# facebookresearch/habitat-lab

Hardware: AMD Instinct MI355X
Metric: env-steps/sec (SPS) PointNav RGB-D 256x256, 64 envs x 128 rollout (higher is better)
Workload: dtype f32; 1 GPU; PointNav SimpleCNN+GRU, 64 envs x 128 steps, 256x256 RGB-D synthetic; envs_per_gpu=64, rollout_steps=128, ppo_epoch=4, num_mini_batch=4, parallelism=dp1

## Files before the change

habitat-lab_amd/csrc/conv2_dgrad_strip.h:

```cpp
#pragma once
#include "igemm_bf3.h"
#include "ops.h"

namespace hab {

struct C2dArgs {
    const float* dy;
    const float* wd;
    const float* mask;
    float* dx;
    int B;
    int strips, items;
    int sign_schedule;
    int H, W, Ho, Wo;
};

template <int R2>
struct C2dCfg {
    static constexpr int H = 63, Ho = 30, Wo = 30, NT = 512, CELLS = 32;
    static constexpr int YRS = R2 + 1, YCOLS = 33, YPIX = YRS * YCOLS;
    static constexpr int YU = YRS * Wo * 16, YPT = (YU + NT - 1) / NT;
    static constexpr int Y_PLANE = YPIX * 64;
    static constexpr int RED_LD = 68;
    static constexpr size_t Y_BYTES = ((size_t)3 * Y_PLANE * 2 + 15) / 16 * 16, RED_BYTES = (size_t)8 * 32 * RED_LD * 4;
    static constexpr size_t LDS_BYTES = Y_BYTES + RED_BYTES;
    static_assert(CELLS % R2 == 0, "");
};

template <int R2, bool RT>
__global__ void __launch_bounds__(512) conv2_dgrad_strip_kernel(const C2dArgs a) {
    using Cfg = C2dCfg<R2>;
    constexpr int NT = Cfg::NT;
    const int H = RT ? a.H : Cfg::H, W = RT ? a.W : Cfg::H, Ho = RT ? a.Ho : Cfg::Ho, Wo = RT ? a.Wo : Cfg::Wo;
    const int YU = Cfg::YRS * Wo * 16;
    extern __shared__ __attribute__((aligned(16))) unsigned short smem16[];
    unsigned short* ys = smem16;
    float* red = reinterpret_cast<float*>(reinterpret_cast<char*>(smem16) + Cfg::Y_BYTES);
    const int t = threadIdx.x, lane = t & 63;
    const int wave = __builtin_amdgcn_readfirstlane(t >> 6);
    const int tap = wave >> 1, ph = wave & 1, ta = tap >> 1, tb = tap & 1;
    const int li = lane & 31, hi = lane >> 5;

    const int xcd = blockIdx.x & 7, jw = blockIdx.x >> 3, wg_per_xcd = gridDim.x >> 3;
    const int per_xcd = (a.items + 7) >> 3, per_wg = (per_xcd + wg_per_xcd - 1) / wg_per_xcd;
    const int xcd_end = min(a.items, (xcd + 1) * per_xcd);
    const int first = min(xcd_end, xcd * per_xcd + jw * per_wg), last = min(xcd_end, first + per_wg);
    if (first >= last) return;

    for (int i = t; i < (int)(Cfg::Y_BYTES / 16); i += NT) reinterpret_cast<u32x4*>(smem16)[i] = u32x4{0u, 0u, 0u, 0u};

    const bool flip = a.sign_schedule && (blockIdx.x & 1);
    const unsigned sgn2 = flip ? 0x80008000u : 0u;

    bf16x8 bw[4][2][3];
#pragma unroll
    for (int j = 0; j < 4; ++j)
#pragma unroll
        for (int pw = 0; pw < 2; ++pw) {
            const int kh = ph + 2 * ta, kw = pw + 2 * tb, co = j * 16 + hi * 8;
            const float* src = a.wd + ((size_t)(li * 4 + kh) * 4 + kw) * 64 + co;
            const f32x4 v0 = *reinterpret_cast<const f32x4*>(src), v1 = *reinterpret_cast<const f32x4*>(src + 4);
            unsigned p[3][4];
            bf3_split2(v0[0], v0[1], p[0][0], p[1][0], p[2][0]);
            bf3_split2(v0[2], v0[3], p[0][1], p[1][1], p[2][1]);
            bf3_split2(v1[0], v1[1], p[0][2], p[1][2], p[2][2]);
            bf3_split2(v1[2], v1[3], p[0][3], p[1][3], p[2][3]);
#pragma unroll
            for (int pl = 0; pl < 3; ++pl)
                bw[j][pw][pl] = __builtin_bit_cast(bf16x8, u32x4{p[pl][0] ^ sgn2, p[pl][1] ^ sgn2, p[pl][2] ^ sgn2, p[pl][3] ^ sgn2});
        }

    f32x4 yr[Cfg::YPT];
    int pf_h20 = 0;
    auto fetch = [&](int item) {
        const int img = item / a.strips, h20 = (item - img * a.strips) * R2;
        pf_h20 = h20;
#pragma unroll
        for (int j = 0; j < Cfg::YPT; ++j) {
            const int u = t + j * NT;
            const int r = u / (Wo * 16), row = h20 - 1 + r;
            const bool ok = (RT ? u < YU : (Cfg::YU % NT == 0 || u < Cfg::YU)) && (unsigned)row < (unsigned)Ho;
            const size_t off = ok ? ((size_t)img * Ho + row) * (size_t)(Wo * 64) + (size_t)(u - r * (Wo * 16)) * 4 : 0;
            yr[j] = *reinterpret_cast<const f32x4*>(a.dy + off);
        }
    };
    auto stage = [&]() {
#pragma unroll
        for (int j = 0; j < Cfg::YPT; ++j) {
            const int u = t + j * NT;
            if (RT ? u >= YU : (Cfg::YU % NT != 0 && u >= Cfg::YU)) continue;
            const int r = u / (Wo * 16), rem = u - r * (Wo * 16), w = rem >> 4, c4 = rem & 15;
            const int pixidx = r * Cfg::YCOLS + w + 1;
            unsigned short* dst = ys + pixidx * 64 + (((c4 >> 1) ^ ((pixidx >> 1) & 7)) << 3) + (c4 & 1) * 4;
            const bool in_image = (unsigned)(pf_h20 - 1 + r) < (unsigned)Ho;
            bf3_store4(in_image ? yr[j] : f32x4{0.f, 0.f, 0.f, 0.f}, dst, dst + Cfg::Y_PLANE, dst + 2 * Cfg::Y_PLANE);
        }
    };

    __syncthreads();
    fetch(first);
    for (int item = first; item < last; ++item) {
        stage();
        __syncthreads();
        if (item + 1 < last) fetch(item + 1);
        const int img = item / a.strips, h20 = (item - img * a.strips) * R2;
#pragma unroll 1
        for (int tr = 0; tr < R2; ++tr) {
            const int pixidx = (tr + 1 - ta) * Cfg::YCOLS + li + 1 - tb;
            const int swz = (pixidx >> 1) & 7;
            f32x4 mk[2];
            if (a.mask) {
#pragma unroll
                for (int q = 0; q < 2; ++q) {
                    const int idx = t + q * NT, rph = idx >> 9, cell = (idx >> 4) & 31, cq = idx & 15;
                    const int h = 2 * (h20 + tr) + rph, w = 2 * cell + (cq >> 3);
                    const bool ok = h < H && w < W;
                    mk[q] = *reinterpret_cast<const f32x4*>(a.mask + (ok ? (((size_t)img * H + h) * W + w) * 32 + (cq & 7) * 4 : (size_t)0));
                }
            }
            f32x16 acc[2];
#pragma unroll
            for (int pw = 0; pw < 2; ++pw)
#pragma unroll
                for (int v = 0; v < 16; ++v) acc[pw][v] = 0.f;
#pragma unroll
            for (int j = 0; j < 4; ++j) {
                const unsigned short* src = ys + pixidx * 64 + (((2 * j + hi) ^ swz) << 3);
                bf16x8 yf[3];
#pragma unroll
                for (int pl = 0; pl < 3; ++pl) yf[pl] = *reinterpret_cast<const bf16x8*>(src + pl * Cfg::Y_PLANE);
                constexpr int PA[6] = {2, 0, 1, 1, 0, 0}, PB[6] = {0, 2, 1, 0, 1, 0};
#pragma unroll
                for (int q = 0; q < 6; ++q)
#pragma unroll
                    for (int pw = 0; pw < 2; ++pw)
                        acc[pw] = __builtin_amdgcn_mfma_f32_32x32x16_bf16(bw[j][pw][PB[q]], yf[PA[q]], acc[pw], 0, 0, 0);
            }
            if (tr > 0) __syncthreads();
            float* mine = red + (size_t)(wave * 32 + li) * Cfg::RED_LD;
#pragma unroll
            for (int pw = 0; pw < 2; ++pw)
#pragma unroll
                for (int g = 0; g < 4; ++g)
                    *reinterpret_cast<f32x4*>(mine + pw * 32 + 8 * g + 4 * hi) =
                        f32x4{acc[pw][4 * g], acc[pw][4 * g + 1], acc[pw][4 * g + 2], acc[pw][4 * g + 3]};
            __syncthreads();
            const int h2 = h20 + tr;
#pragma unroll
            for (int q = 0; q < 2; ++q) {
                const int idx = t + q * NT, rph = idx >> 9, cell = (idx >> 4) & 31, cq = idx & 15;
                f32x4 s = *reinterpret_cast<const f32x4*>(red + (size_t)(rph * 32 + cell) * Cfg::RED_LD + cq * 4);
#pragma unroll
                for (int t4 = 1; t4 < 4; ++t4)
                    s += *reinterpret_cast<const f32x4*>(red + (size_t)((2 * t4 + rph) * 32 + cell) * Cfg::RED_LD + cq * 4);
                if (flip) s = -s;
                const int h = 2 * h2 + rph, w = 2 * cell + (cq >> 3);
                if (h < H && w < W) {
                    const size_t off = (((size_t)img * H + h) * W + w) * 32 + (cq & 7) * 4;
                    if (a.mask) {
                        const f32x4 m = mk[q];
#pragma unroll
                        for (int e = 0; e < 4; ++e) s[e] = m[e] > 0.f ? s[e] : 0.f;
                    }
                    *reinterpret_cast<f32x4*>(a.dx + off) = s;
                }
            }
        }
        __syncthreads();
    }
}

inline bool conv2_dgrad_strip_covers(const ConvDesc& d) {
    return d.KH == 4 && d.KW == 4 && d.stride == 2 && d.pad == 0 && d.C == 32 && d.Cout == 64 && d.H >= 4 && d.W >= 4 && d.H <= 63 && d.W <= 63;
}

inline int conv2_dgrad_strip(const ConvDesc& d, const float* dy, const float* wd, const float* mask, const float* add, float* dx,
                             hipStream_t stream) {
    if (!conv2_dgrad_strip_covers(d)) return 1;
    if (add || d.B < 16 || !dy || !wd || !dx) return 1;
    if ((reinterpret_cast<uintptr_t>(dy) | reinterpret_cast<uintptr_t>(wd) | reinterpret_cast<uintptr_t>(dx) | reinterpret_cast<uintptr_t>(mask)) & 15) return 1;
    constexpr int R2 = 2;
    using Cfg = C2dCfg<R2>;
    C2dArgs a;
    a.dy = dy; a.wd = wd; a.mask = mask; a.dx = dx; a.B = d.B;
    a.H = d.H; a.W = d.W; a.Ho = (d.H - 4) / 2 + 1; a.Wo = (d.W - 4) / 2 + 1;
    a.strips = ((d.H + 1) / 2 + R2 - 1) / R2;
    if ((long long)d.B * a.strips > 0x7fffffffLL) return 1;
    a.items = d.B * a.strips;
    static const int sign_schedule = !hab_env_flag("HAB_BF3_NOSIGN");
    a.sign_schedule = sign_schedule;
    static const hipError_t attr_err = [] {
        const hipError_t e0 = hipFuncSetAttribute(reinterpret_cast<const void*>(conv2_dgrad_strip_kernel<R2, false>),
                                                  hipFuncAttributeMaxDynamicSharedMemorySize, (int)Cfg::LDS_BYTES);
        const hipError_t e1 = hipFuncSetAttribute(reinterpret_cast<const void*>(conv2_dgrad_strip_kernel<R2, true>),
                                                  hipFuncAttributeMaxDynamicSharedMemorySize, (int)Cfg::LDS_BYTES);
        return e0 != hipSuccess ? e0 : e1;
    }();
    if (attr_err != hipSuccess) return (int)attr_err;
    int grid = 256;
    while (grid > 8 && grid > a.items) grid -= 8;
    if (d.H == 63 && d.W == 63) conv2_dgrad_strip_kernel<R2, false><<<grid, Cfg::NT, Cfg::LDS_BYTES, stream>>>(a);
    else conv2_dgrad_strip_kernel<R2, true><<<grid, Cfg::NT, Cfg::LDS_BYTES, stream>>>(a);
    HAB_LAUNCH_CHECK();
    return HAB_OK;
}

}
```

habitat-lab_amd/csrc/conv2_fwd_strip.h:

```cpp
#pragma once
#include "igemm_bf3.h"

namespace hab {

struct C2fArgs {
    const float* x;
    const float* wf;
    const float* bias;
    float* y;
    int B;
    int strips, items;
    int relu, sign_schedule;
    int H, W, Ho, Wo;
};

template <int R>
struct C2fCfg {
    static constexpr int W = 63, C = 32, N = 64, Wo = 30, Ho = 30, NT = 512;
    static constexpr int XRS = 2 * (R - 1) + 4, XROWS = XRS * W, NPIX = R * Wo, NPT = (NPIX + 31) / 32;
    static constexpr int XU = XRS * W * C / 4, XPT = (XU + NT - 1) / NT;
    static constexpr int WH = (W + 1) / 2;
    static constexpr int X_PLANE = XROWS * 32;
    static constexpr int RED_LD = N + 4;
    static constexpr size_t X_BYTES = (size_t)3 * X_PLANE * 2, RED_BYTES = (size_t)8 * 32 * RED_LD * 4;
    static constexpr size_t LDS_BYTES = X_BYTES + RED_BYTES;
    static_assert(X_BYTES % 16 == 0 && Ho % R == 0, "");
    __host__ __device__ static constexpr int xcol(int w) { return (w & 1) * WH + (w >> 1); }
};

template <int R, bool RT>
__global__ void __launch_bounds__(512) conv2_fwd_strip_kernel(const C2fArgs a) {
    using Cfg = C2fCfg<R>;
    constexpr int NT = Cfg::NT;
    const int W = RT ? a.W : Cfg::W, H = RT ? a.H : Cfg::W, Wo = RT ? a.Wo : Cfg::Wo, Ho = RT ? a.Ho : Cfg::Ho;
    const int WH = (W + 1) / 2, X_PLANE = Cfg::XRS * W * 32, XU = Cfg::XRS * W * 8, NPIX = R * Wo, NPT = (NPIX + 31) / 32;
    auto xcol = [&](int w) { return (w & 1) * WH + (w >> 1); };
    extern __shared__ __attribute__((aligned(16))) unsigned short smem16[];
    unsigned short* xs = smem16;
    float* red = reinterpret_cast<float*>(reinterpret_cast<char*>(smem16) + (size_t)3 * X_PLANE * 2);
    const int t = threadIdx.x, lane = t & 63;
    const int wave = __builtin_amdgcn_readfirstlane(t >> 6);
    const int kh = wave >> 1, kwp = wave & 1;
    const int li = lane & 31, hi = lane >> 5;

    const int xcd = blockIdx.x & 7, jw = blockIdx.x >> 3, wg_per_xcd = gridDim.x >> 3;
    const int per_xcd = (a.items + 7) >> 3, per_wg = (per_xcd + wg_per_xcd - 1) / wg_per_xcd;
    const int xcd_end = min(a.items, (xcd + 1) * per_xcd);
    const int first = min(xcd_end, xcd * per_xcd + jw * per_wg), last = min(xcd_end, first + per_wg);
    if (first >= last) return;

    const bool flip = a.sign_schedule && (blockIdx.x & 1);
    const unsigned sgn2 = flip ? 0x80008000u : 0u;

    bf16x8 bw[4][2][3];
#pragma unroll
    for (int j = 0; j < 4; ++j)
#pragma unroll
        for (int ct = 0; ct < 2; ++ct) {
            const int co = ct * 32 + li, kw = 2 * kwp + (j >> 1), ci = (j & 1) * 16 + hi * 8;
            const float* src = a.wf + ((size_t)(co * 4 + kh) * 4 + kw) * 32 + ci;
            const f32x4 v0 = *reinterpret_cast<const f32x4*>(src), v1 = *reinterpret_cast<const f32x4*>(src + 4);
            unsigned p[3][4];
            bf3_split2(v0[0], v0[1], p[0][0], p[1][0], p[2][0]);
            bf3_split2(v0[2], v0[3], p[0][1], p[1][1], p[2][1]);
            bf3_split2(v1[0], v1[1], p[0][2], p[1][2], p[2][2]);
            bf3_split2(v1[2], v1[3], p[0][3], p[1][3], p[2][3]);
#pragma unroll
            for (int pl = 0; pl < 3; ++pl)
                bw[j][ct][pl] = __builtin_bit_cast(bf16x8, u32x4{p[pl][0] ^ sgn2, p[pl][1] ^ sgn2, p[pl][2] ^ sgn2, p[pl][3] ^ sgn2});
        }

    f32x4 xr[Cfg::XPT];
    int pf_units = XU;
    auto fetch = [&](int item) {
        const int img = item / a.strips, ho0 = (item - img * a.strips) * R;
        const float* xb = a.x + ((size_t)img * H + ho0 * 2) * (size_t)(W * 32);
        if (RT) pf_units = min(Cfg::XRS, H - 2 * ho0) * W * 8;
#pragma unroll
        for (int j = 0; j < Cfg::XPT; ++j) {
            const int u = t + j * NT;
            const bool in = RT ? u < pf_units : (Cfg::XU % NT == 0 || u < Cfg::XU);
            xr[j] = *reinterpret_cast<const f32x4*>(xb + (in ? (size_t)u * 4 : 0));
        }
    };
    auto stage = [&]() {
#pragma unroll
        for (int j = 0; j < Cfg::XPT; ++j) {
            const int u = t + j * NT;
            if (RT ? u >= XU : (Cfg::XU % NT != 0 && u >= Cfg::XU)) continue;
            const int c4 = u & 7, pix = u >> 3, w = pix % W, hh = pix / W;
            const int row = hh * W + xcol(w);
            unsigned short* dst = xs + row * 32 + (((c4 >> 1) ^ ((row >> 2) & 3)) << 3) + (c4 & 1) * 4;
            bf3_store4((!RT || u < pf_units) ? xr[j] : f32x4{0.f, 0.f, 0.f, 0.f}, dst, dst + X_PLANE, dst + 2 * X_PLANE);
        }
    };

    const int rpix = t >> 4, rco = (t & 15) * 4;
    f32x4 bias4 = {0.f, 0.f, 0.f, 0.f};
    if (a.bias) bias4 = *reinterpret_cast<const f32x4*>(a.bias + rco);

    fetch(first);
    for (int item = first; item < last; ++item) {
        stage();
        __syncthreads();
        if (item + 1 < last) fetch(item + 1);
        const int img = item / a.strips, ho0 = (item - img * a.strips) * R;
        float* yb = a.y + ((size_t)img * Ho + ho0) * (size_t)(Wo * 64);
        const int npix_here = RT ? min(R, Ho - ho0) * Wo : NPIX;
#pragma unroll 1
        for (int pt = 0; pt < NPT; ++pt) {
            const int p = pt * 32 + li;
            const int pc = (!RT && Cfg::NPIX % 32 == 0) || p < NPIX ? p : 0;
            const int hol = pc / Wo, wo = pc - hol * Wo;
            const int row0 = (hol * 2 + kh) * W + wo;
            f32x16 acc[2];
#pragma unroll
            for (int ct = 0; ct < 2; ++ct)
#pragma unroll
                for (int v = 0; v < 16; ++v) acc[ct][v] = 0.f;
#pragma unroll
            for (int j = 0; j < 4; ++j) {
                const int kw = 2 * kwp + (j >> 1);
                const int row = row0 + (kw & 1) * WH + (kw >> 1);
                const int chunk = (j & 1) * 2 + hi;
                const unsigned short* src = xs + row * 32 + ((chunk ^ ((row >> 2) & 3)) << 3);
                bf16x8 af[3];
#pragma unroll
                for (int pl = 0; pl < 3; ++pl) af[pl] = *reinterpret_cast<const bf16x8*>(src + pl * X_PLANE);
                constexpr int PA[6] = {2, 0, 1, 1, 0, 0}, PB[6] = {0, 2, 1, 0, 1, 0};
#pragma unroll
                for (int q = 0; q < 6; ++q)
#pragma unroll
                    for (int ct = 0; ct < 2; ++ct)
                        acc[ct] = __builtin_amdgcn_mfma_f32_32x32x16_bf16(bw[j][ct][PB[q]], af[PA[q]], acc[ct], 0, 0, 0);
            }
            if (pt > 0) __syncthreads();
            float* mine = red + (size_t)(wave * 32 + li) * Cfg::RED_LD;
#pragma unroll
            for (int ct = 0; ct < 2; ++ct)
#pragma unroll
                for (int g = 0; g < 4; ++g)
                    *reinterpret_cast<f32x4*>(mine + ct * 32 + 8 * g + 4 * hi) =
                        f32x4{acc[ct][4 * g], acc[ct][4 * g + 1], acc[ct][4 * g + 2], acc[ct][4 * g + 3]};
            __syncthreads();
            f32x4 s = *reinterpret_cast<const f32x4*>(red + (size_t)rpix * Cfg::RED_LD + rco);
#pragma unroll
            for (int w8 = 1; w8 < 8; ++w8) s += *reinterpret_cast<const f32x4*>(red + (size_t)(w8 * 32 + rpix) * Cfg::RED_LD + rco);
            if (flip) s = -s;
            s += bias4;
            if (a.relu) {
#pragma unroll
                for (int e = 0; e < 4; ++e) s[e] = s[e] > 0.f ? s[e] : 0.f;
            }
            const int op = pt * 32 + rpix;
            if (RT ? op < npix_here : (Cfg::NPIX % 32 == 0 || op < Cfg::NPIX)) *reinterpret_cast<f32x4*>(yb + (size_t)op * 64 + rco) = s;
        }
        __syncthreads();
    }
}

inline bool conv2_fwd_strip_covers(const ConvGeom& g) {
    return g.KH == 4 && g.KW == 4 && g.stride == 2 && g.pad == 0 && g.C == 32 && g.Cout == 64 && g.H >= 4 && g.W >= 4 && g.W <= 63;
}

inline int conv2_fwd_strip(const ConvFwdProb& p, float* , size_t , hipStream_t stream) {
    const ConvGeom& g = p.g;
    if (!conv2_fwd_strip_covers(g)) return 1;
    if ((p.ldy != 0 && p.ldy != 64) || g.B < 16) return 1;
    if ((reinterpret_cast<uintptr_t>(p.x) | reinterpret_cast<uintptr_t>(p.w) | reinterpret_cast<uintptr_t>(p.y) | reinterpret_cast<uintptr_t>(p.bias)) & 15) return 1;
    constexpr int R = 2;
    using Cfg = C2fCfg<R>;
    C2fArgs a;
    a.x = p.x; a.wf = p.w; a.bias = p.bias; a.y = p.y; a.B = g.B;
    a.H = g.H; a.W = g.W; a.Ho = (g.H - 4) / 2 + 1; a.Wo = (g.W - 4) / 2 + 1;
    a.strips = (a.Ho + R - 1) / R;
    if ((long long)g.B * a.strips > 0x7fffffffLL) return 1;
    a.items = g.B * a.strips;
    a.relu = p.relu;
    static const int sign_schedule = !hab_env_flag("HAB_BF3_NOSIGN");
    a.sign_schedule = sign_schedule;
    const bool bench_geom = g.H == 63 && g.W == 63;
    static const hipError_t attr_err = [] {
        const hipError_t e0 = hipFuncSetAttribute(reinterpret_cast<const void*>(conv2_fwd_strip_kernel<R, false>),
                                                  hipFuncAttributeMaxDynamicSharedMemorySize, (int)Cfg::LDS_BYTES);
        const hipError_t e1 = hipFuncSetAttribute(reinterpret_cast<const void*>(conv2_fwd_strip_kernel<R, true>),
                                                  hipFuncAttributeMaxDynamicSharedMemorySize, (int)Cfg::LDS_BYTES);
        return e0 != hipSuccess ? e0 : e1;
    }();
    if (attr_err != hipSuccess) return (int)attr_err;
    int grid = 256;
    while (grid > 8 && grid > a.items) grid -= 8;
    if (bench_geom) conv2_fwd_strip_kernel<R, false><<<grid, Cfg::NT, Cfg::LDS_BYTES, stream>>>(a);
    else conv2_fwd_strip_kernel<R, true><<<grid, Cfg::NT, (size_t)3 * Cfg::XRS * g.W * 32 * 2 + Cfg::RED_BYTES, stream>>>(a);
    HAB_LAUNCH_CHECK();
    return HAB_OK;
}

}
```

habitat-lab_amd/csrc/engine.h:

```cpp
#pragma once
#include <string.h>

#include <algorithm>
#include <string>
#include <vector>

#include "heads.h"
#include "ops.h"
#include "problems.h"
#include "resnet_ops.h"
#include "../../include/habitat_amd.h"

struct ParamSpec {
    std::string name;
    int64_t shape[4];
    int ndim;
    int64_t offset;
    int64_t numel;
    int is_buffer = 0;
};

struct Arena {
    int64_t used = 0;
    int64_t take(int64_t n) {
        const int64_t o = used;
        used += (n + 63) & ~(int64_t)63;
        return o;
    }
};

struct RnnForm {
    int chunks = 0;
    bool wave = false;
};

struct hab_policy {
    hab_policy_desc d;
    std::vector<ParamSpec> params;
    int64_t param_floats = 0, packed_floats = 0, work_floats = 0;
    float *P = nullptr, *G = nullptr, *PK = nullptr, *WK = nullptr;
    int64_t work_bound = 0;
    int Cin = 0;
    hab::ConvDesc c1, c2, c3;
    int fc_in = 0, rnn_in = 0, rnn_ld = 0, G_ = 3, L = 1;
    int i_c1w = -1, i_c1b = -1, i_c2w = -1, i_c2b = -1, i_c3w = -1, i_c3b = -1, i_fcw = -1, i_fcb = -1, i_aw = -1, i_ab = -1, i_cw = -1, i_cb = -1;
    int i_astd = -1;
    int head_K = 0;
    int64_t w_gsaved = -1;
    std::vector<int> i_wih, i_whh, i_bih, i_bhh;
    int64_t pk_c1f = -1, pk_c2f = -1, pk_c2d = -1, pk_c3f = -1, pk_c3d = -1, pk_fc = -1;
    int64_t pk_c1img = -1;
    std::vector<int64_t> pk_whht;
    std::vector<int64_t> pk_wiht;
    int64_t pk_wih0 = -1;
    int64_t w_a1 = -1, w_a2 = -1, w_a3 = -1, w_da1 = -1, w_da2 = -1, w_da3 = -1;
    int64_t w_rnnin = -1, w_drnnin = -1, w_hinit = -1, w_cinit = -1, w_probs = -1, w_logitsn = -1, w_dzv = -1, w_dv = -1, w_dfeat = -1,
            w_scratch = -1, w_value = -1, w_logp = -1, w_ent = -1, w_hmask = -1, w_gistep = -1, w_step_h = -1, w_ws = -1;
    std::vector<int64_t> w_gi, w_gates, w_hn, w_hprev, w_cprev, w_c, w_out, w_dgi, w_dgh, w_dlayer;
    int64_t ws_floats = 0;
    int last_B = 0, last_n = 0;
    const uint8_t* last_masks = nullptr;
    hipStream_t s2 = nullptr;
    std::vector<hipEvent_t> evs;
    int64_t w_ws2 = -1, ws2_floats = 0, w_fmask = -1, w_iota = -1;
    RnnForm form;
    struct ResNetPlan* rn = nullptr;
    int save_acts = 1;
    int training = 1;
    hab_allreduce_fn allreduce_cb = nullptr;
    void* allreduce_ctx = nullptr;
    int world_size = 1;
    hab_grad_ready_fn grad_ready_cb = nullptr;
    void* grad_ready_ctx = nullptr;
    struct hab_comm* comm = nullptr;
    const float* xg_feat = nullptr; const float* xg_perc = nullptr;
    int comm_err = 0;
    int64_t comm_first = -1;
    hipStream_t cur_stream = nullptr;
    uint64_t probe_mask = 0;
    struct ProbeEv { int tag; hipEvent_t first, second; };
    std::vector<ProbeEv> probe_events;
    size_t probe_used = 0;
    double probe_flops[64] = {0}, probe_bytes[64] = {0};

    float* p(int i) const { return P + params[i].offset; }
    float* g(int i) const { return G + params[i].offset; }
};

inline int add_param(hab_policy* e, const std::string& name, std::initializer_list<int64_t> shape) {
    ParamSpec s;
    s.name = name;
    s.ndim = (int)shape.size();
    s.numel = 1;
    int k = 0;
    for (auto v : shape) { s.shape[k++] = v; s.numel *= v; }
    for (; k < 4; ++k) s.shape[k] = 1;
    s.offset = e->param_floats;
    e->param_floats += (s.numel + 3) & ~(int64_t)3;
    e->params.push_back(s);
    return (int)e->params.size() - 1;
}
inline int conv_out(int x, int k, int s, int p) { return (x + 2 * p - k) / s + 1; }

void add_tail_params(hab_policy* e);
void pack_tail(hab_policy* e, Arena& pk);
void plan_tail_workspace(hab_policy* e, Arena& wk, int64_t ws_floats);
int repack_tail(hab_policy* e, hipStream_t s);
int build_resnet(hab_policy* e);
void destroy_resnet(hab_policy* e);
int resnet_repack(hab_policy* e, hipStream_t s);
void grad_tail_ready(hab_policy* e, int first_param);
int comm_exchange_async(struct hab_comm* c, float* buf, int64_t first, int64_t count, hipStream_t compute);
extern "C" int hab_comm_allreduce_sum(struct hab_comm* c, float* buf, int64_t count, hipStream_t stream);
int resnet_feature_shape(const hab_policy* e, int* c, int* hf, int* wf);
int resnet_encode(hab_policy* e, const hab_obs* obs, int n, float* out, hipStream_t s);
int resnet_encoder_forward(hab_policy* e, const hab_obs* obs, const uint8_t* masks, const int* rows, int B, hipStream_t s, int f0 = 0, int nB = -1);
int resnet_encoder_backward(hab_policy* e, const hab_obs* obs, const uint8_t* masks, const int* rows, int B, hipStream_t s);
int resnet_tap(hab_policy* e, int which, const float** ptr, int64_t* floats);

struct Probe {
    hab_policy* e; hipStream_t s; bool on;
    Probe(hab_policy* e_, int tag, hipStream_t s_, double flops = 0.0, double bytes = 0.0) : e(e_), s(s_), on((e_->probe_mask >> tag) & 1) {
        if (!on) return;
        e->probe_flops[tag] += flops; e->probe_bytes[tag] += bytes;
        if (e->probe_used == e->probe_events.size()) {
            hipEvent_t a, b;
            (void)hipEventCreate(&a); (void)hipEventCreate(&b);
            e->probe_events.push_back({tag, a, b});
        }
        e->probe_events[e->probe_used].tag = tag;
        (void)hipEventRecord(e->probe_events[e->probe_used].first, s);
    }
    ~Probe() {
        if (!on) return;
        (void)hipEventRecord(e->probe_events[e->probe_used].second, s);
        e->probe_used++;
    }
};
// ... 2 lines not shown
```

habitat-lab_amd/csrc/engine.hip:

```cpp
#include <string.h>

#include <algorithm>

#include <string>
#include <vector>

#include "engine.h"

using namespace hab;

static void plan_tm_workspace(hab_policy* e, Arena& wk);
void add_tail_params(hab_policy* e) {
    const hab_policy_desc& d = e->d;
    const int H = d.hidden;
    const std::string rn = "net.state_encoder.rnn.";
    for (int l = 0; l < d.rnn_layers; ++l) {
        const int in = l == 0 ? e->rnn_in : H;
        const std::string sfx = "_l" + std::to_string(l);
        e->i_wih.push_back(add_param(e, rn + "weight_ih" + sfx, {e->G_ * H, in}));
        e->i_whh.push_back(add_param(e, rn + "weight_hh" + sfx, {e->G_ * H, H}));
        e->i_bih.push_back(add_param(e, rn + "bias_ih" + sfx, {e->G_ * H}));
        e->i_bhh.push_back(add_param(e, rn + "bias_hh" + sfx, {e->G_ * H}));
    }
    if (d.action_dist == HAB_DIST_GAUSSIAN) {
// ... 11 lines not shown
void pack_tail(hab_policy* e, Arena& pk) {
    const int64_t GH = (int64_t)e->G_ * e->d.hidden;
    for (int l = 0; l < e->L; ++l) e->pk_whht.push_back(pk.take(GH * e->d.hidden));
    for (int l = 0; l < e->L; ++l) e->pk_wiht.push_back(l == 0 ? -1 : pk.take(GH * e->d.hidden));
    e->pk_wih0 = pk.take(GH * e->rnn_ld);
}
int repack_tail(hab_policy* e, hipStream_t s) {
    const int H = e->d.hidden;
    for (int l = 0; l < e->L; ++l) HAB_TRY(transpose2d(e->p(e->i_whh[l]), e->PK + e->pk_whht[l], e->G_ * H, H, s));
    for (int l = 1; l < e->L; ++l) HAB_TRY(transpose2d(e->p(e->i_wih[l]), e->PK + e->pk_wiht[l], e->G_ * H, H, s));
    return pad_rows(e->p(e->i_wih[0]), e->PK + e->pk_wih0, e->G_ * H, e->rnn_in, e->rnn_ld, s);
}
void plan_tail_workspace(hab_policy* e, Arena& wk, int64_t ws_floats) {
    const hab_policy_desc& d = e->d;
    const int64_t B = d.max_frames, F = d.max_frames;
    const int64_t H = d.hidden, GH = e->G_ * H;
    e->w_rnnin = wk.take(B * e->rnn_ld); e->w_drnnin = wk.take(B * e->rnn_ld);
    e->w_hinit = wk.take(e->L * F * H); e->w_cinit = wk.take(e->L * F * H);
    for (int l = 0; l < e->L; ++l) {
        e->w_gi.push_back(wk.take(B * GH)); e->w_gates.push_back(wk.take(B * GH));
        e->w_hn.push_back(wk.take(B * H)); e->w_hprev.push_back(wk.take(B * H));
        e->w_cprev.push_back(wk.take(B * H)); e->w_c.push_back(wk.take(B * H)); e->w_out.push_back(wk.take(B * H));
        e->w_dgi.push_back(wk.take(B * GH)); e->w_dgh.push_back(wk.take(B * GH));
        e->w_dlayer.push_back(wk.take(B * H));
    }
    e->w_probs = wk.take(B * 8); e->w_logitsn = wk.take(B * 8); e->w_dzv = wk.take(B * 8); e->w_dv = wk.take(B);
    e->w_dfeat = wk.take(B * H); e->w_scratch = wk.take((int64_t)std::max(3, 2 * e->L) * F * H);
    e->w_value = wk.take(B); e->w_logp = wk.take(B); e->w_ent = wk.take(B);
    if (d.action_dist == HAB_DIST_GAUSSIAN) e->w_gsaved = wk.take(B * 16);
    e->w_hmask = wk.take(2 * H * e->L * d.max_envs);
    e->w_gistep = wk.take(d.max_envs * GH);
    e->w_step_h = wk.take(d.max_envs * H * 2);
    e->ws_floats = ws_floats;
    e->w_ws = wk.take(ws_floats);
    plan_tm_workspace(e, wk);
}

static int build_baseline(hab_policy* e) {
    const hab_policy_desc& d = e->d;
    e->Cin = (d.has_rgb ? 3 : 0) + (d.has_depth ? 1 : 0);
    const bool blind = e->Cin == 0;
    if (blind && d.goal_dim <= 0) return HAB_ERR_ARG;
    if (d.rnn_type != HAB_RNN_GRU && d.rnn_type != HAB_RNN_LSTM) return HAB_ERR_ARG;
    const int H = d.hidden;
    e->G_ = d.rnn_type == HAB_RNN_GRU ? 3 : 4;
    e->L = d.rnn_layers;
    e->c1 = ConvDesc{0, d.H, d.W, blind ? 4 : e->Cin, 32, 8, 8, 4, 0};
    e->c2 = ConvDesc{0, conv_out(d.H, 8, 4, 0), conv_out(d.W, 8, 4, 0), 32, 64, 4, 4, 2, 0};
    e->c3 = ConvDesc{0, e->c2.Ho(), e->c2.Wo(), 64, 32, 3, 3, 1, 0};
    const int h3 = e->c3.Ho(), w3 = e->c3.Wo();
    if (!blind && (h3 <= 0 || w3 <= 0)) return HAB_ERR_ARG;
    e->fc_in = blind ? 0 : 32 * h3 * w3;
    e->rnn_in = (blind ? 0 : H) + d.goal_dim;
    e->rnn_ld = (e->rnn_in + 15) & ~15;
    const std::string ve = "net.visual_encoder.cnn.";
    if (!blind) {
        e->i_c1w = add_param(e, ve + "0.weight", {32, e->Cin, 8, 8});
        e->i_c1b = add_param(e, ve + "0.bias", {32});
        e->i_c2w = add_param(e, ve + "2.weight", {64, 32, 4, 4});
        e->i_c2b = add_param(e, ve + "2.bias", {64});
        e->i_c3w = add_param(e, ve + "4.weight", {32, 64, 3, 3});
        e->i_c3b = add_param(e, ve + "4.bias", {32});
        e->i_fcw = add_param(e, ve + "6.weight", {H, e->fc_in});
        e->i_fcb = add_param(e, ve + "6.bias", {H});
    }
    add_tail_params(e);

    Arena pk;
    e->pk_c1f = pk.take(32 * 64 * (blind ? 4 : e->Cin));
    e->pk_c1img = (!blind && e->Cin == 4) ? pk.take(obs_conv_weight_image_floats()) : -1;
    e->pk_c2f = pk.take(64 * 16 * 32);
    e->pk_c2d = pk.take(64 * 16 * 32);
    e->pk_c3f = pk.take(32 * 9 * 64);
    e->pk_c3d = pk.take(32 * 9 * 64);
    e->pk_fc = pk.take((int64_t)H * std::max(e->fc_in, 4));
    pack_tail(e, pk);
    e->packed_floats = pk.used;

    Arena wk;
    const int64_t B = d.max_frames;
    const int64_t m1 = blind ? 0 : (int64_t)e->c1.Ho() * e->c1.Wo() * 32, m2 = blind ? 0 : (int64_t)e->c2.Ho() * e->c2.Wo() * 64, m3 = e->fc_in;
    e->w_a1 = wk.take(B * m1); e->w_a2 = wk.take(B * m2); e->w_a3 = wk.take(B * m3);
    e->w_da1 = wk.take(B * m1); e->w_da2 = wk.take(B * m2); e->w_da3 = wk.take(B * m3);
    plan_tail_workspace(e, wk, std::max<int64_t>((int64_t)16 << 20, (int64_t)8 * H * e->fc_in / 4));
    e->work_floats = wk.used;
    return HAB_OK;
}

extern "C" int hab_policy_create(const hab_policy_desc* desc, hab_policy** out) {
    if (!desc || !out) return HAB_ERR_ARG;
    if (desc->hidden <= 0 || desc->hidden % 64 || desc->num_actions <= 0 || desc->num_actions > 8 || desc->max_frames <= 0 ||
        desc->max_envs <= 0 || desc->rnn_layers <= 0 || desc->goal_dim < 0 ||
        ((desc->has_rgb || desc->has_depth || desc->has_semantic || desc->num_visual > 0) && (desc->H <= 0 || desc->W <= 0)))
        return HAB_ERR_ARG;
    if (desc->arch != HAB_ARCH_RESNET && (desc->num_visual != 0 || desc->num_fused != 0)) return HAB_ERR_UNSUPPORTED;
    if (desc->action_dist != HAB_DIST_CATEGORICAL && (desc->action_dist != HAB_DIST_GAUSSIAN || desc->arch != HAB_ARCH_RESNET))
        return HAB_ERR_UNSUPPORTED;
    if (desc->action_dist == HAB_DIST_GAUSSIAN && desc->num_actions > 4) return HAB_ERR_UNSUPPORTED;
    hab_policy* e = new hab_policy();
    e->d = *desc;
    int rc = HAB_ERR_UNSUPPORTED;
    if (desc->arch == HAB_ARCH_SIMPLE_CNN) rc = build_baseline(e);
    else if (desc->arch == HAB_ARCH_RESNET) rc = build_resnet(e);
    if (rc != HAB_OK) { destroy_resnet(e); delete e; return rc; }
    *out = e;
    return HAB_OK;
}
extern "C" void hab_policy_destroy(hab_policy* e) {
    if (!e) return;
    for (auto& ev : e->probe_events) { (void)hipEventDestroy(ev.first); (void)hipEventDestroy(ev.second); }
    for (auto& ev : e->evs) (void)hipEventDestroy(ev);
    if (e->s2) (void)hipStreamDestroy(e->s2);
    destroy_resnet(e);
    delete e;
}
extern "C" int hab_policy_num_params(const hab_policy* e) { return e ? (int)e->params.size() : HAB_ERR_ARG; }
extern "C" int hab_policy_param_info(const hab_policy* e, int i, char* name, int name_cap, int64_t* shape4, int* ndim,
                                     int64_t* offset_floats) {
    if (!e || i < 0 || i >= (int)e->params.size() || !name || name_cap <= 0) return HAB_ERR_ARG;
    const ParamSpec& s = e->params[i];
    strncpy(name, s.name.c_str(), name_cap - 1);
    name[name_cap - 1] = 0;
    if (shape4) for (int k = 0; k < 4; ++k) shape4[k] = s.shape[k];
    if (ndim) *ndim = s.ndim;
    if (offset_floats) *offset_floats = s.offset;
    return HAB_OK;
}
extern "C" int hab_policy_param_is_buffer(const hab_policy* e, int i) {
    if (!e || i < 0 || i >= (int)e->params.size()) return HAB_ERR_ARG;
    return e->params[i].is_buffer;
}
extern "C" int hab_policy_set_training(hab_policy* e, int training) {
    if (!e) return HAB_ERR_ARG;
    e->training = training ? 1 : 0;
    return HAB_OK;
}
extern "C" int hab_policy_set_grad_ready(hab_policy* e, hab_grad_ready_fn fn, void* ctx) {
    if (!e) return HAB_ERR_ARG;
    e->grad_ready_cb = fn; e->grad_ready_ctx = ctx;
    return HAB_OK;
}
void grad_tail_ready(hab_policy* e, int first_param) {
    if (e->comm) {
        static const bool no_overlap = hab_env_flag("HAB_NO_GRAD_OVERLAP");
        if (no_overlap || e->comm_err != HAB_OK) return;
        const int64_t first = e->g(first_param) - e->G;
        const int64_t end = e->comm_first < 0 ? (int64_t)e->param_floats : e->comm_first;
        if (first >= end) return;
        const int rc = comm_exchange_async(e->comm, e->G, first, end - first, e->cur_stream);
        if (rc == HAB_OK) e->comm_first = first;
        else e->comm_err = rc;
        return;
    }
    if (!e->grad_ready_cb) return;
    const int64_t first = e->g(first_param) - e->G;
    e->grad_ready_cb(first, (int64_t)e->param_floats - first, e->grad_ready_ctx);
}
extern "C" int hab_policy_set_allreduce(hab_policy* e, hab_allreduce_fn fn, void* ctx, int world_size) {
    if (!e || world_size < 1) return HAB_ERR_ARG;
    e->allreduce_cb = fn; e->allreduce_ctx = ctx; e->world_size = world_size;
    return HAB_OK;
}
extern "C" int64_t hab_policy_param_floats(const hab_policy* e) { return e ? e->param_floats : -1; }
extern "C" int64_t hab_policy_packed_floats(const hab_policy* e) { return e ? e->packed_floats : -1; }
extern "C" int64_t hab_policy_work_floats(const hab_policy* e) { return e ? e->work_floats : -1; }

// ... 8 lines not shown
extern "C" int hab_policy_repack(hab_policy* e, hipStream_t stream) {
    if (!e || !e->P) return HAB_ERR_ARG;
    if (e->rn) return resnet_repack(e, stream);
    if (e->Cin == 0) return repack_tail(e, stream);
    HAB_TRY(repack_conv(e->p(e->i_c1w), e->PK + e->pk_c1f, nullptr, 32, e->Cin, 8, 8, e->Cin, stream));
    if (e->pk_c1img >= 0) {
        const int rc = obs_conv_weight_image(e->PK + e->pk_c1f, 32, 8, 8, e->Cin, e->PK + e->pk_c1img, stream);
        if (rc != HAB_OK) return rc == 1 ? HAB_ERR_UNSUPPORTED : rc;
    }
    HAB_TRY(repack_conv(e->p(e->i_c2w), e->PK + e->pk_c2f, e->PK + e->pk_c2d, 64, 32, 4, 4, 32, stream));
    HAB_TRY(repack_conv(e->p(e->i_c3w), e->PK + e->pk_c3f, e->PK + e->pk_c3d, 32, 64, 3, 3, 64, stream));
    HAB_TRY(repack_flatten(e->p(e->i_fcw), e->PK + e->pk_fc, e->d.hidden, 32, e->fc_in / 32, stream));
    return repack_tail(e, stream);
}

extern "C" int hab_policy_probe_enable(hab_policy* e, int tag) {
    if (!e || tag >= 64) return HAB_ERR_ARG;
    e->probe_mask = tag < 0 ? 0 : (uint64_t)1 << tag;
    e->probe_used = 0;
    for (int i = 0; i < 64; ++i) { e->probe_flops[i] = 0.0; e->probe_bytes[i] = 0.0; }
    return HAB_OK;
}
extern "C" int hab_policy_probe_enable_mask(hab_policy* e, uint64_t mask) {
    if (!e) return HAB_ERR_ARG;
    e->probe_mask = mask;
    e->probe_used = 0;
    for (int i = 0; i < 64; ++i) { e->probe_flops[i] = 0.0; e->probe_bytes[i] = 0.0; }
    return HAB_OK;
}
static int probe_sum(hab_policy* e, int tag, double* total_ms, int* count) {
    double t = 0;
    int n = 0;
    for (size_t i = 0; i < e->probe_used; ++i) {
        if (tag >= 0 && e->probe_events[i].tag != tag) continue;
        hipError_t err = hipEventSynchronize(e->probe_events[i].second);
        if (err != hipSuccess) return (int)err;
        float ms = 0;
        err = hipEventElapsedTime(&ms, e->probe_events[i].first, e->probe_events[i].second);
        if (err != hipSuccess) return (int)err;
        t += ms;
        ++n;
    }
    *total_ms = t;
    *count = n;
    return HAB_OK;
}
extern "C" int hab_policy_probe_work(hab_policy* e, int tag, double* flops, double* bytes) {
    if (!e || tag < 0 || tag >= 64 || !flops || !bytes) return HAB_ERR_ARG;
    *flops = e->probe_flops[tag]; *bytes = e->probe_bytes[tag];
    return HAB_OK;
}
extern "C" int hab_policy_probe_read(hab_policy* e, double* total_ms, int* count) {
    if (!e || !total_ms || !count) return HAB_ERR_ARG;
    HAB_TRY(probe_sum(e, -1, total_ms, count));
    e->probe_used = 0;
    return HAB_OK;
}
extern "C" int hab_policy_probe_read_tag(hab_policy* e, int tag, double* total_ms, int* count) {
    if (!e || !total_ms || !count || tag < 0 || tag >= 64) return HAB_ERR_ARG;
    return probe_sum(e, tag, total_ms, count);
}


static int encoder_forward(hab_policy* e, const hab_obs* obs, const uint8_t* masks, const int* rows, int B, hipStream_t s, int f0 = 0, int nB = -1) {
    if (e->rn) { Probe pr(e, HAB_PROBE_ENC_FWD, s); return resnet_encoder_forward(e, obs, masks, rows, B, s, f0, nB); }
    if (nB < 0) nB = B;
    float* W = e->WK;
    float* ws = W + e->w_ws;
    const int H = e->d.hidden;
    if (e->Cin == 0) {
        if (!rows && f0) return HAB_ERR_ARG;
        return gather_cols(obs->goal, e->d.goal_dim, rows ? rows + f0 : nullptr, W + e->w_rnnin + (int64_t)f0 * e->rnn_ld, e->rnn_ld, 0, e->d.goal_dim,
                           e->rnn_ld - e->rnn_in, nB, s);
    }
    const int64_t m1 = (int64_t)e->c1.Ho() * e->c1.Wo() * 32, m2 = (int64_t)e->c2.Ho() * e->c2.Wo() * 64, m3 = e->fc_in;
    float *a1 = W + e->w_a1 + f0 * m1, *a2 = W + e->w_a2 + f0 * m2, *a3 = W + e->w_a3 + f0 * m3, *rin = W + e->w_rnnin + (int64_t)f0 * e->rnn_ld;
    const int* rws = rows ? rows + f0 : nullptr;
    if (!rows && f0) return HAB_ERR_ARG;
    ObsView ov;
    ov.rgb = e->d.has_rgb ? obs->rgb : nullptr; ov.depth = e->d.has_depth ? obs->depth : nullptr; ov.rows = rws;
    ov.H = e->d.H; ov.W = e->d.W; ov.C = e->Cin;
    ConvDesc c1 = e->c1, c2 = e->c2, c3 = e->c3;
    c1.B = c2.B = c3.B = nB;
    { Probe pr(e, HAB_PROBE_CONV1_FWD, s);
      HAB_TRY(obs_conv_fwd(c1, ov, e->PK + e->pk_c1f, e->p(e->i_c1b), a1, 1, ws, e->ws_floats, s, e->pk_c1img >= 0 ? e->PK + e->pk_c1img : nullptr)); }
    { Probe pr(e, HAB_PROBE_CONV2_FWD, s);
      HAB_TRY(conv_fwd(c2, a1, e->PK + e->pk_c2f, e->p(e->i_c2b), a2, 1, ws, e->ws_floats, s)); }
    { Probe pr(e, HAB_PROBE_CONV3_FWD, s);
      HAB_TRY(conv_fwd(c3, a2, e->PK + e->pk_c3f, e->p(e->i_c3b), a3, 0, ws, e->ws_floats, s)); }
    { Probe pr(e, HAB_PROBE_FC_FWD, s);
      HAB_TRY(linear_fwd(a3, e->fc_in, e->PK + e->pk_fc, e->fc_in, e->p(e->i_fcb), rin, e->rnn_ld, nB, H, e->fc_in, 1, 0, ws, e->ws_floats, s)); }
    if (e->d.goal_dim > 0)
        HAB_TRY(gather_cols(obs->goal, e->d.goal_dim, rws, rin, e->rnn_ld, H, e->d.goal_dim, e->rnn_ld - e->rnn_in, nB, s));
    return HAB_OK;
}

static RnnForm rnn_form_cfg(const hab_policy* e, int frames, int n, bool tm_shape) {
    static const int chunks = hab_env_int("HAB_RNN_CHUNKS", 4), chunks_resnet = hab_env_int("HAB_RNN_CHUNKS_RESNET", -1);
    static const int wave = hab_env_int("HAB_RNN_WAVE", 1);
    RnnForm f;
    if (tm_shape) {
        int nc = chunks;
        if (e->rn && chunks > 1) nc = chunks_resnet >= 0 ? chunks_resnet : frames >= 4096 ? 2 : 0;
        f.chunks = std::max(0, std::min(nc, frames / n));
    }
    if (f.chunks == 0) f.wave = wave && e->L >= 2 && e->L <= 4;
    return f;
}
static RnnForm rnn_form(const hab_policy* e, const int* rows, const hab_pack_info* pack, int B, int n) {
    const bool tm_shape = e->Cin > 0 && rows && !pack->env_first_frame && (B % n) == 0 && B / n >= 2 && e->w_ws2 >= 0 &&
                          (int64_t)e->L * 2 * n <= 3 * (int64_t)e->d.max_frames;
    return rnn_form_cfg(e, B, n, tm_shape);
}
static void plan_tm_workspace(hab_policy* e, Arena& wk) {
    const int64_t B = e->d.max_frames;
    if (rnn_form_cfg(e, (int)B, 1, true).chunks == 0) return;
    e->ws2_floats = e->ws_floats;
    e->w_ws2 = wk.take(e->ws2_floats);
    e->w_fmask = wk.take((B + 3) / 4 + 64);
    e->w_iota = wk.take(B + 64);
}
static int tm_setup(hab_policy* e, int nev) {
    if (!e->s2) {
        int lo = 0, hi = 0;
        (void)hipDeviceGetStreamPriorityRange(&lo, &hi);
        hipError_t err = hipStreamCreateWithPriority(&e->s2, hipStreamNonBlocking, hi);
        if (err != hipSuccess) return (int)err;
    }
    while ((int)e->evs.size() < nev) {
        hipEvent_t ev;
        hipError_t err = hipEventCreateWithFlags(&ev, hipEventDisableTiming);
        if (err != hipSuccess) return (int)err;
        e->evs.push_back(ev);
    }
    return HAB_OK;
}
static int tm_order(hab_policy* e, int ev, hipStream_t from, hipStream_t to) {
    hipError_t err = hipEventRecord(e->evs[ev], from);
    if (err != hipSuccess) return (int)err;
    err = hipStreamWaitEvent(to, e->evs[ev], 0);
    return err == hipSuccess ? HAB_OK : (int)err;
}

static RnnLayerParams layer_params(hab_policy* e, int l) {
    RnnLayerParams lp;
    lp.w_ih = e->p(e->i_wih[l]); lp.w_hh = e->p(e->i_whh[l]); lp.b_ih = e->p(e->i_bih[l]); lp.b_hh = e->p(e->i_bhh[l]);
    lp.w_hh_t = e->PK + e->pk_whht[l];
    if (e->G) { lp.dw_ih = e->g(e->i_wih[l]); lp.dw_hh = e->g(e->i_whh[l]); lp.db_ih = e->g(e->i_bih[l]); lp.db_hh = e->g(e->i_bhh[l]); }
    else { lp.dw_ih = lp.dw_hh = lp.db_ih = lp.db_hh = nullptr; }
    lp.in_dim = l == 0 ? e->rnn_in : e->d.hidden;
    if (l == 0 && e->pk_wih0 >= 0) { lp.w_ih_pad = e->PK + e->pk_wih0; lp.w_ih_ld = e->rnn_ld; }
    else if (l > 0 && (e->d.hidden & 15) == 0) { lp.w_ih_pad = lp.w_ih; lp.w_ih_ld = e->d.hidden; }
    return lp;
}
static RnnWork layer_work(hab_policy* e, int l) {
    float* W = e->WK;
    RnnWork wk;
    wk.gi = W + e->w_gi[l]; wk.gates = W + e->w_gates[l]; wk.hn = W + e->w_hn[l]; wk.hprev = W + e->w_hprev[l];
    wk.cprev = W + e->w_cprev[l]; wk.c = W + e->w_c[l]; wk.out = W + e->w_out[l]; wk.dgi = W + e->w_dgi[l];
    wk.dgh = W + e->w_dgh[l];
    return wk;
}
static const float* layer_x(const hab_policy* e, int l) { return e->WK + (l == 0 ? e->w_rnnin : e->w_out[l - 1]); }
static int layer_ld(const hab_policy* e, int l) { return l == 0 ? e->rnn_ld : e->d.hidden; }
static float* layer_dx(const hab_policy* e, int l) { return e->WK + (l == 0 ? e->w_drnnin : e->w_dlayer[l]); }
static const float* layer_dout(const hab_policy* e, int l) { return l == e->L - 1 ? e->WK + e->w_dfeat : layer_dx(e, l + 1); }
static PackInfo pack_info(const hab_pack_info* pack, int n) {
    PackInfo pk;
    pk.select_inds = pack->select_inds; pk.step_offsets = pack->step_offsets_host; pk.num_seqs_at_step = pack->num_seqs_at_step_host;
    pk.frag_env = pack->frag_env; pk.frag_start = pack->frag_start; pk.P = pack->P; pk.F = pack->F; pk.max_len = pack->max_len;
// ... 64 lines not shown
    ha.mode = actions ? (deterministic ? 2 : 1) : 2;
    ha.feats = x; ha.feats_ld = ldx; ha.w_actor = e->p(e->i_aw); ha.b_actor = e->p(e->i_ab); ha.w_critic = e->p(e->i_cw); ha.b_critic = e->p(e->i_cb);
    ha.actions_in = nullptr; ha.rows = nullptr; ha.noise = exp_noise;
    ha.actions_out = actions ? actions : reinterpret_cast<int64_t*>(W + e->w_dzv);
    ha.value = values; ha.logp = action_log_probs ? action_log_probs : W + e->w_logp; ha.entropy = nullptr;
    ha.probs = probs_out ? W + e->w_probs : nullptr; ha.logits_n = W + e->w_logitsn;
    if (ha.mode == 1 && !exp_noise) return HAB_ERR_ARG;
    HAB_TRY(heads_forward(ha, stream));
    if (probs_out) HAB_TRY(copy_rows(W + e->w_probs, nullptr, 8, probs_out, 8, n, 8, stream));
    return HAB_OK;
}

static int rnn_state_init(hab_policy* e, const float* hidden0, int hidden_env_stride, const int* rows, const uint8_t* masks,
                          const int* frag_env, const int* frag_start, int F, const int* env_first_frame, hipStream_t s) {
    const int H = e->d.hidden, L = e->L;
    for (int l = 0; l < L; ++l) {
        HAB_TRY(rnn_frag_init(hidden0 + (size_t)l * H, rows, hidden_env_stride, masks, rows, frag_env, frag_start, F, H,
                              e->WK + e->w_hinit + (size_t)l * F * H, s, env_first_frame));
        if (e->d.rnn_type == HAB_RNN_LSTM)
            HAB_TRY(rnn_frag_init(hidden0 + (size_t)(L + l) * H, rows, hidden_env_stride, masks, rows, frag_env, frag_start, F, H,
                                  e->WK + e->w_cinit + (size_t)l * F * H, s, env_first_frame));
    }
    return HAB_OK;
}
static int rnn_tm_forward(hab_policy* e, const hab_obs* obs, const int* rows, const float* hidden0, int hidden_env_stride,
                          const uint8_t* masks, int B, int n, hipStream_t stream) {
    float* W = e->WK;
    const int H = e->d.hidden, L = e->L, NC = e->form.chunks, T = B / n, Tc = (T + NC - 1) / NC;
    HAB_TRY(tm_setup(e, 2 * NC + 4));
    hipStream_t sB = e->s2;
    uint8_t* fmask = reinterpret_cast<uint8_t*>(W + e->w_fmask);
    HAB_TRY(rnn_tm_prepare(masks, rows, B, fmask, reinterpret_cast<int*>(W + e->w_iota), stream));
    HAB_TRY(rnn_state_init(e, hidden0, hidden_env_stride, rows, masks, nullptr, nullptr, n, nullptr, stream));
    for (int c = 0; c < NC; ++c) {
        const int t0 = c * Tc, t1 = std::min(T, t0 + Tc);
        if (t0 >= t1) break;
        HAB_TRY(encoder_forward(e, obs, masks, rows, B, stream, t0 * n, (t1 - t0) * n));
        HAB_TRY(tm_order(e, c, stream, sB));
        for (int l = 0; l < L; ++l) {
            Probe pr(e, HAB_PROBE_RNN_FWD, sB);
            HAB_TRY(rnn_tm_layer_forward(e->d.rnn_type, H, layer_params(e, l), layer_work(e, l), layer_x(e, l), layer_ld(e, l),
                                         W + e->w_hinit + (size_t)l * n * H, W + e->w_cinit + (size_t)l * n * H, fmask, n, T, t0, t1,
                                         W + e->w_ws2, e->ws2_floats, sB));
        }
    }
    return tm_order(e, NC, sB, stream);
}
static int rnn_packed_forward(hab_policy* e, const int* rows, const float* hidden0, int hidden_env_stride, const uint8_t* masks,
                              const hab_pack_info* pack, int n, hipStream_t stream) {
    float* W = e->WK;
    const int H = e->d.hidden, L = e->L;
    const PackInfo pk = pack_info(pack, n);
    HAB_TRY(rnn_state_init(e, hidden0, hidden_env_stride, rows, masks, pk.frag_env, pk.frag_start, pk.F, pack->env_first_frame, stream));
    if (e->form.wave) {
        RnnLayerParams lps[4]; RnnWork wks[4]; const float* hin[4]; const float* cin[4];
        for (int l = 0; l < L; ++l) {
            lps[l] = layer_params(e, l); wks[l] = layer_work(e, l);
            hin[l] = W + e->w_hinit + (size_t)l * pk.F * H; cin[l] = W + e->w_cinit + (size_t)l * pk.F * H;
        }
        Probe pr(e, HAB_PROBE_RNN_FWD, stream);
        const int rc = rnn_seq_wave_forward(e->d.rnn_type, H, L, lps, wks, layer_x(e, 0), layer_ld(e, 0), hin, cin, pk, W + e->w_ws,
                                            e->ws_floats, stream);
        return rc == 1 ? HAB_ERR_UNSUPPORTED : rc;
    }
    for (int l = 0; l < L; ++l) {
        Probe pr(e, HAB_PROBE_RNN_FWD, stream);
        HAB_TRY(rnn_seq_layer_forward(e->d.rnn_type, H, layer_params(e, l), layer_work(e, l), layer_x(e, l), layer_ld(e, l),
                                      W + e->w_hinit + (size_t)l * pk.F * H, W + e->w_cinit + (size_t)l * pk.F * H, pk, W + e->w_ws,
                                      e->ws_floats, stream));
    }
    return HAB_OK;
}

extern "C" int hab_policy_evaluate(hab_policy* e, const hab_obs* obs, const int* rows, const float* hidden0,
                                   int hidden_env_stride, const uint8_t* masks, const int64_t* actions,
                                   const hab_pack_info* pack, int B, int n, float* value, float* log_prob, float* entropy,
                                   hipStream_t stream) {
    if (!e || !e->P || !obs || !hidden0 || !masks || !actions || !pack || B <= 0 || n <= 0 || B > e->d.max_frames) return HAB_ERR_ARG;
    if (!pack->env_first_frame && (B % n)) return HAB_ERR_ARG;
    if (pack->P != B || pack->F <= 0 || pack->F > B || pack->max_len <= 0) return HAB_ERR_ARG;
    float* W = e->WK;
    const int H = e->d.hidden, L = e->L;
    e->form = rnn_form(e, rows, pack, B, n);
    if (e->form.chunks > 0) {
        HAB_TRY(rnn_tm_forward(e, obs, rows, hidden0, hidden_env_stride, masks, B, n, stream));
    } else {
        HAB_TRY(encoder_forward(e, obs, masks, rows, B, stream));
        HAB_TRY(rnn_packed_forward(e, rows, hidden0, hidden_env_stride, masks, pack, n, stream));
    }
    const float* feats = W + e->w_out[L - 1];
    if (e->d.action_dist == HAB_DIST_GAUSSIAN) {
        GaussHeadsArgs ga;
        ga.B = B; ga.H = H; ga.A = e->d.num_actions; ga.K = e->head_K; ga.flags = e->d.gauss_flags; ga.mode = 0;
        ga.min_std = e->d.gauss_min_std; ga.max_std = e->d.gauss_max_std;
        ga.feats = feats; ga.feats_ld = H; ga.w = e->p(e->i_aw); ga.b = e->p(e->i_ab);
        ga.std_param = e->i_astd >= 0 ? e->p(e->i_astd) : nullptr; ga.w_critic = e->p(e->i_cw); ga.b_critic = e->p(e->i_cb);
        ga.actions_in = reinterpret_cast<const float*>(actions); ga.rows = rows; ga.noise = nullptr; ga.actions_out = nullptr;
        ga.value = value ? value : W + e->w_value; ga.logp = log_prob ? log_prob : W + e->w_logp;
        ga.entropy = entropy ? entropy : W + e->w_ent; ga.saved = W + e->w_gsaved;
        HAB_TRY(gauss_heads_forward(ga, stream));
    } else {
    HeadsArgs ha;
        ha.B = B; ha.H = H; ha.A = e->d.num_actions; ha.mode = 0;
        ha.feats = feats; ha.feats_ld = H; ha.w_actor = e->p(e->i_aw); ha.b_actor = e->p(e->i_ab); ha.w_critic = e->p(e->i_cw); ha.b_critic = e->p(e->i_cb);
        ha.actions_in = actions; ha.rows = rows; ha.noise = nullptr; ha.actions_out = nullptr;
        ha.value = value ? value : W + e->w_value; ha.logp = log_prob ? log_prob : W + e->w_logp;
        ha.entropy = entropy ? entropy : W + e->w_ent;
        ha.probs = W + e->w_probs; ha.logits_n = W + e->w_logitsn;
        HAB_TRY(heads_forward(ha, stream));
    }
    e->last_B = B;
    e->last_n = pack->env_first_frame ? 0 : n;
    e->last_masks = masks;
    return HAB_OK;
}

extern "C" int hab_policy_final_hidden(hab_policy* e, float* hidden_out, hipStream_t stream) {
    if (!e || !hidden_out || e->last_B <= 0 || e->last_n <= 0) return HAB_ERR_ARG;
    const int H = e->d.hidden, L = e->L, n = e->last_n, B = e->last_B;
    const int Lh = e->d.rnn_type == HAB_RNN_LSTM ? 2 * L : L;
    for (int l = 0; l < L; ++l) {
        HAB_TRY(copy_rows(e->WK + e->w_out[l] + (size_t)(B - n) * H, nullptr, H, hidden_out + (size_t)l * H, Lh * H, n, H, stream));
        if (e->d.rnn_type == HAB_RNN_LSTM)
            HAB_TRY(copy_rows(e->WK + e->w_c[l] + (size_t)(B - n) * H, nullptr, H, hidden_out + (size_t)(L + l) * H, Lh * H, n, H, stream));
    }
    return HAB_OK;
}

__global__ void add_rows_kernel(float* __restrict__ dst, const float* __restrict__ src, long long n) {
    for (long long i = (long long)blockIdx.x * blockDim.x + threadIdx.x; i < n; i += (long long)gridDim.x * blockDim.x) dst[i] += src[i];
}
__global__ void add_masked_cols_kernel(float* __restrict__ dst, int ldd, const float* __restrict__ src, const float* __restrict__ x, int ldx,
                                       int B, int H) {
    const long long n = (long long)B * H;
    for (long long i = (long long)blockIdx.x * blockDim.x + threadIdx.x; i < n; i += (long long)gridDim.x * blockDim.x) {
        const int f = (int)(i / H), c = (int)(i % H);
        if (x[(size_t)f * ldx + c] > 0.f) dst[(size_t)f * ldd + c] += src[i];
    }
}
extern "C" int hab_policy_set_extra_grads(hab_policy* e, const float* d_rnn_output, const float* d_perception_embed) {
    if (!e) return HAB_ERR_ARG;
    if (d_perception_embed && e->Cin == 0) return HAB_ERR_ARG;
    e->xg_feat = d_rnn_output; e->xg_perc = d_perception_embed;
    return HAB_OK;
}

static int cnn_dgrad(hab_policy* e, int64_t f0, int nB, hipStream_t s) {
    float* W = e->WK;
    float* ws = W + e->w_ws;
    const int64_t m1 = (int64_t)e->c1.Ho() * e->c1.Wo() * 32, m2 = (int64_t)e->c2.Ho() * e->c2.Wo() * 64, m3 = e->fc_in;
    ConvDesc c2 = e->c2, c3 = e->c3;
    c2.B = c3.B = nB;
    { Probe pr(e, HAB_PROBE_FC_DGRAD, s);
      HAB_TRY(linear_dgrad(W + e->w_drnnin + f0 * e->rnn_ld, e->rnn_ld, e->PK + e->pk_fc, e->fc_in, nullptr, 0, 0, W + e->w_da3 + f0 * m3,
                           e->fc_in, nB, e->fc_in, e->d.hidden, 0, ws, e->ws_floats, s)); }
    { Probe pr(e, HAB_PROBE_CONV3_DGRAD, s);
      HAB_TRY(conv_dgrad(c3, W + e->w_da3 + f0 * m3, e->PK + e->pk_c3d, W + e->w_a2 + f0 * m2, nullptr, W + e->w_da2 + f0 * m2, ws,
                         e->ws_floats, s)); }
    { Probe pr(e, HAB_PROBE_CONV2_DGRAD, s);
      HAB_TRY(conv_dgrad(c2, W + e->w_da2 + f0 * m2, e->PK + e->pk_c2d, W + e->w_a1 + f0 * m1, nullptr, W + e->w_da1 + f0 * m1, ws,
                         e->ws_floats, s)); }
    return HAB_OK;
}
static int rnn_tm_backward(hab_policy* e, int B, hipStream_t stream) {
    float* W = e->WK;
    const int H = e->d.hidden, L = e->L, n = e->last_n, T = B / n, NC = e->form.chunks, Tc = (T + NC - 1) / NC;
    hipStream_t sB = e->s2;
    const uint8_t* fmask = reinterpret_cast<const uint8_t*>(W + e->w_fmask);
    const int* iota = reinterpret_cast<const int*>(W + e->w_iota);
    HAB_TRY(tm_order(e, NC + 1, stream, sB));
    for (int c = NC - 1; c >= 0; --c) {
        const int t0 = c * Tc, t1 = std::min(T, t0 + Tc);
        if (t0 >= t1) continue;
        for (int l = L - 1; l >= 0; --l) {
            Probe pr(e, HAB_PROBE_RNN_BWD, sB);
            HAB_TRY(rnn_tm_layer_backward(e->d.rnn_type, H, layer_params(e, l), layer_work(e, l), layer_dout(e, l), layer_dx(e, l), layer_ld(e, l),
                                          l == 0 ? layer_x(e, 0) : nullptr, layer_ld(e, l), H, fmask, iota, n, T, t0, t1,
                                          W + e->w_scratch + (size_t)l * 2 * n * H, W + e->w_ws2, e->ws2_floats, sB));
        }
        if (!e->rn) {
            HAB_TRY(tm_order(e, NC + 2 + c, sB, stream));
            HAB_TRY(cnn_dgrad(e, (int64_t)t0 * n, (t1 - t0) * n, stream));
        }
    }
    for (int l = L - 1; l >= 0; --l)
        HAB_TRY(rnn_tm_layer_param_grads(e->d.rnn_type, H, layer_params(e, l), layer_work(e, l), layer_x(e, l), layer_ld(e, l), B, W + e->w_ws2,
                                         e->ws2_floats, sB));
    return HAB_OK;
}
static int rnn_packed_backward(hab_policy* e, const hab_pack_info* pack, hipStream_t stream) {
    float* W = e->WK;
    const int H = e->d.hidden, L = e->L;
    const PackInfo pk = pack_info(pack, e->last_n);
    const bool blind0 = !e->rn && e->Cin == 0, nofc = e->Cin == 0;
    const float* x0 = layer_x(e, 0);
    if (e->form.wave) {
        RnnLayerParams lps[4]; RnnWork wks[4]; const float* wiht[4];
        for (int l = 0; l < L; ++l) { lps[l] = layer_params(e, l); wks[l] = layer_work(e, l); wiht[l] = l ? e->PK + e->pk_wiht[l] : nullptr; }
        Probe pr(e, HAB_PROBE_RNN_BWD, stream);
        const int rc = rnn_seq_wave_backward(e->d.rnn_type, H, L, lps, wiht, wks, x0, e->rnn_ld, layer_dout(e, L - 1), blind0 ? nullptr : layer_dx(e, 0),
                                             e->rnn_ld, nofc ? nullptr : x0, e->rnn_ld, nofc ? 0 : H, pk, W + e->w_scratch, W + e->w_ws, e->ws_floats,
                                             stream);
        return rc == 1 ? HAB_ERR_UNSUPPORTED : rc;
    }
    for (int l = L - 1; l >= 0; --l) {
        Probe pr(e, HAB_PROBE_RNN_BWD, stream);
        HAB_TRY(rnn_seq_layer_backward(e->d.rnn_type, H, layer_params(e, l), layer_work(e, l), layer_x(e, l), layer_ld(e, l), layer_dout(e, l),
                                       (blind0 && l == 0) ? nullptr : layer_dx(e, l), layer_ld(e, l), (l == 0 && !nofc) ? x0 : nullptr,
                                       layer_ld(e, l), nofc ? 0 : H, pk, W + e->w_scratch, W + e->w_ws, e->ws_floats, stream));
    }
    return HAB_OK;
}

static int policy_backward_impl(hab_policy* e, const hab_obs* obs, const int* rows, const int64_t* actions,
                                const hab_pack_info* pack, const float* d_value, const float* d_log_prob,
                                const float* d_entropy, hipStream_t stream) {
    if (!e || !e->P || !e->G || !obs || !actions || !pack || !d_value || !d_log_prob || !d_entropy || e->last_B <= 0)
        return HAB_ERR_ARG;
    e->comm_err = HAB_OK;
    float* W = e->WK;
    float* ws = W + e->w_ws;
    const int H = e->d.hidden, L = e->L, B = e->last_B, A = e->d.num_actions;
    e->cur_stream = stream;
    e->comm_first = -1;
    const float* feats = W + e->w_out[L - 1];
    if (e->d.action_dist == HAB_DIST_GAUSSIAN) {
        const int K = e->head_K;
        GaussHeadsBwdArgs gb;
        gb.B = B; gb.H = H; gb.A = A; gb.K = K; gb.d_value = d_value; gb.d_logp = d_log_prob; gb.d_entropy = d_entropy;
        gb.actions = reinterpret_cast<const float*>(actions); gb.rows = rows; gb.saved = W + e->w_gsaved;
        gb.w = e->p(e->i_aw); gb.w_critic = e->p(e->i_cw); gb.dfeat = W + e->w_dfeat; gb.dz = W + e->w_dzv; gb.dv_out = W + e->w_dv;
        HAB_TRY(gauss_heads_backward(gb, stream));
        HAB_TRY(linear_wgrad(W + e->w_dzv, 8, feats, H, e->g(e->i_aw), H, B, K, H, 0, 0, 0, ws, e->ws_floats, stream));
        HAB_TRY(colsum(W + e->w_dzv, 8, B, K, e->g(e->i_ab), 0, ws, e->ws_floats, stream));
        if (e->i_astd >= 0) HAB_TRY(colsum(W + e->w_dzv + A, 8, B, A, e->g(e->i_astd), 0, ws, e->ws_floats, stream));
        HAB_TRY(linear_wgrad(W + e->w_dv, 1, feats, H, e->g(e->i_cw), H, B, 1, H, 0, 0, 0, ws, e->ws_floats, stream));
        HAB_TRY(colsum(W + e->w_dv, 1, B, 1, e->g(e->i_cb), 0, ws, e->ws_floats, stream));
    } else {
    HeadsBwdArgs hb;
        hb.B = B; hb.H = H; hb.A = A; hb.d_value = d_value; hb.d_logp = d_log_prob; hb.d_entropy = d_entropy;
        hb.actions = actions; hb.rows = rows; hb.probs = W + e->w_probs; hb.logits_n = W + e->w_logitsn;
        hb.w_actor = e->p(e->i_aw); hb.w_critic = e->p(e->i_cw); hb.dfeat = W + e->w_dfeat; hb.dzv = W + e->w_dzv; hb.dv_out = W + e->w_dv;
        HAB_TRY(heads_backward(hb, stream));
        HAB_TRY(linear_wgrad(W + e->w_dzv, 8, feats, H, e->g(e->i_aw), H, B, A, H, 0, 0, 0, ws, e->ws_floats, stream));
        HAB_TRY(linear_wgrad(W + e->w_dv, 1, feats, H, e->g(e->i_cw), H, B, 1, H, 0, 0, 0, ws, e->ws_floats, stream));
        HAB_TRY(colsum(W + e->w_dzv, 8, B, A, e->g(e->i_ab), 0, ws, e->ws_floats, stream));
        HAB_TRY(colsum(W + e->w_dv, 1, B, 1, e->g(e->i_cb), 0, ws, e->ws_floats, stream));
    }
    const int NC = e->form.chunks;
    if (e->xg_feat || e->xg_perc) {
        if (NC > 0) return HAB_ERR_UNSUPPORTED;
        if (e->xg_feat) {
            add_rows_kernel<<<(int)std::min<long long>(1024, cdivl((long long)B * H, 256)), 256, 0, stream>>>(W + e->w_dfeat, e->xg_feat, (long long)B * H);
            HAB_LAUNCH_CHECK();
        }
    }
    if (NC > 0) {
        HAB_TRY(rnn_tm_backward(e, B, stream));
    } else {
        HAB_TRY(rnn_packed_backward(e, pack, stream));
        if (e->xg_perc) {
            add_masked_cols_kernel<<<(int)std::min<long long>(1024, cdivl((long long)B * H, 256)), 256, 0, stream>>>(
                W + e->w_drnnin, e->rnn_ld, e->xg_perc, W + e->w_rnnin, e->rnn_ld, B, H);
            HAB_LAUNCH_CHECK();
        }
        if (!e->rn && e->Cin == 0) {
            grad_tail_ready(e, e->i_wih[0]);
            return HAB_OK;
        }
    }
    if (e->rn) {
        if (NC > 0) HAB_TRY(tm_order(e, 2 * NC + 3, e->s2, stream));
        Probe pr(e, HAB_PROBE_ENC_BWD, stream);
        return resnet_encoder_backward(e, obs, e->last_masks, rows, B, stream);
    }
    const float* dfc = W + e->w_drnnin;
    { Probe pr(e, HAB_PROBE_FC_WGRAD, stream);
      HAB_TRY(linear_wgrad(dfc, e->rnn_ld, W + e->w_a3, e->fc_in, e->g(e->i_fcw), e->fc_in, B, H, e->fc_in, 32, e->fc_in / 32, 0,
                           ws, e->ws_floats, stream)); }
    HAB_TRY(colsum(dfc, e->rnn_ld, B, H, e->g(e->i_fcb), 0, ws, e->ws_floats, stream));
    if (NC > 0) HAB_TRY(tm_order(e, 2 * NC + 3, e->s2, stream));
    grad_tail_ready(e, e->i_fcw);
    if (NC == 0) HAB_TRY(cnn_dgrad(e, 0, B, stream));
    ConvDesc c1 = e->c1, c2 = e->c2, c3 = e->c3;
    c1.B = c2.B = c3.B = B;
    { Probe pr(e, HAB_PROBE_CONV3_WGRAD, stream);
      HAB_TRY(conv_wgrad(c3, W + e->w_a2, W + e->w_da3, e->g(e->i_c3w), e->g(e->i_c3b), ws, e->ws_floats, stream)); }
    { Probe pr(e, HAB_PROBE_CONV2_WGRAD, stream);
      HAB_TRY(conv_wgrad(c2, W + e->w_a1, W + e->w_da2, e->g(e->i_c2w), e->g(e->i_c2b), ws, e->ws_floats, stream)); }
    ObsView ov;
    ov.rgb = e->d.has_rgb ? obs->rgb : nullptr; ov.depth = e->d.has_depth ? obs->depth : nullptr; ov.rows = rows;
    ov.H = e->d.H; ov.W = e->d.W; ov.C = e->Cin;
    { Probe pr(e, HAB_PROBE_CONV1_WGRAD, stream);
      HAB_TRY(obs_conv_wgrad(c1, ov, W + e->w_da1, e->g(e->i_c1w), e->g(e->i_c1b), ws, e->ws_floats, stream)); }
    return HAB_OK;
}
extern "C" int hab_policy_backward(hab_policy* e, const hab_obs* obs, const int* rows, const int64_t* actions,
                                   const hab_pack_info* pack, const float* d_value, const float* d_log_prob,
                                   const float* d_entropy, hipStream_t stream) {
    const int rc = policy_backward_impl(e, obs, rows, actions, pack, d_value, d_log_prob, d_entropy, stream);
    if (e) e->xg_feat = e->xg_perc = nullptr;
    return (rc == HAB_OK && e && e->comm_err != HAB_OK) ? e->comm_err : rc;
}

extern "C" int hab_policy_tap(hab_policy* e, int which, const float** ptr, int64_t* floats) {
    if (!e || !ptr || !floats || e->last_B <= 0) return HAB_ERR_ARG;
    const int64_t B = e->last_B;
    float* W = e->WK;
    if (e->rn && which != HAB_TAP_RNN_IN && which != HAB_TAP_RNN_OUT) return resnet_tap(e, which, ptr, floats);
    if (!e->rn && e->Cin == 0 && (which == HAB_TAP_CONV1 || which == HAB_TAP_CONV2 || which == HAB_TAP_CONV3)) return HAB_ERR_ARG;
    switch (which) {
        case HAB_TAP_CONV1: *ptr = W + e->w_a1; *floats = B * e->c1.Ho() * e->c1.Wo() * 32; break;
        case HAB_TAP_CONV2: *ptr = W + e->w_a2; *floats = B * e->c2.Ho() * e->c2.Wo() * 64; break;
        case HAB_TAP_CONV3: *ptr = W + e->w_a3; *floats = B * e->fc_in; break;
        case HAB_TAP_RNN_IN: *ptr = W + e->w_rnnin; *floats = B * e->rnn_ld; break;
        case HAB_TAP_RNN_OUT: *ptr = W + e->w_out[e->L - 1]; *floats = B * e->d.hidden; break;
        default: return HAB_ERR_ARG;
    }
    return HAB_OK;
}
```

habitat-lab_amd/csrc/gemm_ops.hip:

```cpp
#include "igemm.h"
#include "igemm_dma.h"
#include "igemm_dma_wgrad.h"
#include "igemm_bf3.h"
#include "igemm_bf3_ws.h"
#include "dense_bf3.h"
#include "obs_conv_bf3.h"
#include "obs_conv_bf3_ws.h"
#include "obs_conv_patch.h"
#include "wgrad3x3_bf3.h"
#include "conv2_fwd_strip.h"
#include "conv2_dgrad_strip.h"
#include "obs_wgrad_bf3.h"
#include "conv_patch_bf3.h"
#include "wgrad3x3_patch.h"
#include "prob_build.h"
#include <stdlib.h>

#include <atomic>

#include "../../include/habitat_amd.h"

namespace hab {

static bool no_dma() { static const bool v = hab_env_flag("HAB_NO_DMA"); return v; }
static bool no_merged_dgrad() { static const bool v = hab_env_flag("HAB_NO_MERGED_DGRAD"); return v; }
static bool no_patch() { static const bool v = hab_env_flag("HAB_NO_PATCH"); return v; }
static std::atomic<int> g_bf3_mode{-1};
static int bf3_mode() {
    int m = g_bf3_mode.load(std::memory_order_relaxed);
    if (m < 0) {
        static const int from_env = hab_env_int("HAB_BF3", 2047);
        int expected = -1;
        g_bf3_mode.compare_exchange_strong(expected, from_env, std::memory_order_relaxed);
        m = g_bf3_mode.load(std::memory_order_relaxed);
    }
    return m;
}
int matrix_path_bits() { return bf3_mode(); }
extern "C" int hab_set_matrix_path(int mode) {
    const int prev = bf3_mode();
    if (mode >= 0) g_bf3_mode.store(mode, std::memory_order_relaxed);
    return prev;
}


template <class P, int TM, int TN, int WM, int WN>
static int bf3_launch(const P& p, float* ws, size_t ws_floats, int target_blocks, hipStream_t stream) {
    constexpr bool WS_SHAPE = P::A_RC && P::B_RC && TM == 2 && TN == 2 && WM == 2 && WN == 2;
    if constexpr (WS_SHAPE) {
        constexpr int ws_min_k = 2048;
        if ((bf3_mode() & 32) && p.K >= ws_min_k) return igemm_bf3_ws_launch<P, TM, TN, WM, WN, 4>(p, ws, ws_floats, target_blocks, stream);
    }
    return igemm_bf3_launch<P, TM, TN, WM, WN>(p, ws, ws_floats, target_blocks, stream);
}

template <class P>
static int run_igemm(const P& p, float* ws, size_t ws_floats, hipStream_t stream, int target_blocks = 1024) {
    if (P::A_RC || P::B_RC) target_blocks = 256;
    constexpr bool WG = !P::A_RC && !P::B_RC && AKv<P>::value == 4;
    if constexpr (P::A_RC && P::B_RC) {
        if ((bf3_mode() & 1) && p.M > 64) {
            if (p.N <= 32) return bf3_launch<P, 2, 1, 4, 1>(p, ws, ws_floats, target_blocks, stream);
            if (p.N <= 64) {
                if (p.M >= 256 * 512 && p.K >= 576) return bf3_launch<P, 2, 2, 4, 1>(p, ws, ws_floats, target_blocks, stream);
                return bf3_launch<P, 1, 2, 4, 1>(p, ws, ws_floats, target_blocks, stream);
            }
            return bf3_launch<P, 2, 2, 2, 2>(p, ws, ws_floats, target_blocks, stream);
        }
    } else if constexpr (AKv<P>::value == 4) {
        if ((bf3_mode() & 4) && p.M > 64) {
            if (p.N <= 32) {
                if constexpr (WG) {
                    if (p.M % 96 == 0 || cdiv(p.M, 96) * 96 < cdiv(p.M, 256) * 256)
                        return bf3_launch<P, 1, 1, 3, 1>(p, ws, ws_floats, target_blocks, stream);
                }
                return bf3_launch<P, 2, 1, 4, 1>(p, ws, ws_floats, target_blocks, stream);
            }
            if (p.N <= 64) {
                if constexpr (WG) {
                    if (p.M % 96 == 0 || cdiv(p.M, 96) * 96 < cdiv(p.M, 128) * 128)
                        return bf3_launch<P, 1, 2, 3, 1>(p, ws, ws_floats, target_blocks, stream);
                }
                return bf3_launch<P, 1, 2, 4, 1>(p, ws, ws_floats, target_blocks, stream);
            }
            return bf3_launch<P, 2, 2, 2, 2>(p, ws, ws_floats, target_blocks, stream);
        }
    }
    if constexpr (std::is_same_v<P, ConvFwdProb> || std::is_same_v<P, ConvDgradProb>) {
        if (p.dma_ok() && p.M > 64 && !no_dma()) {
            if (p.N <= 32) return igemm_dma_launch<P, 2, 1, 4, 1, false>(p, ws, ws_floats, target_blocks, stream);
            if (p.N <= 64) return igemm_dma_launch<P, 1, 2, 4, 1, false>(p, ws, ws_floats, target_blocks, stream);
            if (p.N <= 128) return igemm_dma_launch<P, 2, 2, 2, 2, true>(p, ws, ws_floats, target_blocks, stream);
        }
    }
    if (p.N <= 32) {
        if (p.M <= 64) return igemm_launch<P, 1, 1, 2, 1>(p, ws, ws_floats, target_blocks, stream);
        if constexpr (WG) {
            if (p.M % 96 == 0 || cdiv(p.M, 96) * 96 < cdiv(p.M, 256) * 256)
                return igemm_launch<P, 1, 1, 3, 1>(p, ws, ws_floats, target_blocks, stream);
        }
        return igemm_launch<P, 2, 1, 4, 1>(p, ws, ws_floats, target_blocks, stream);
    } else if (p.N <= 64) {
        if (p.M <= 64) return igemm_launch<P, 1, 1, 2, 2>(p, ws, ws_floats, target_blocks, stream);
        if constexpr (WG) {
            if (p.M % 96 == 0 || cdiv(p.M, 96) * 96 < cdiv(p.M, 128) * 128)
                return igemm_launch<P, 1, 2, 3, 1>(p, ws, ws_floats, target_blocks, stream);
        }
        return igemm_launch<P, 1, 2, 4, 1>(p, ws, ws_floats, target_blocks, stream);
    } else {
        if (p.M <= 64) return igemm_launch<P, 1, 2, 2, 2>(p, ws, ws_floats, target_blocks, stream);
        return igemm_launch<P, 2, 2, 2, 2>(p, ws, ws_floats, target_blocks, stream);
    }
}

int conv_fwd(const ConvDesc& d, const float* x, const float* wf, const float* bias, float* y, int relu, float* ws,
             size_t ws_floats, hipStream_t stream) {
    ConvFwdProb p;
    HAB_TRY(build(p, d, x, wf, bias, y, relu));
    if ((bf3_mode() & 256) && (bf3_mode() & 1)) {
        const int rc = conv2_fwd_strip(p, ws, ws_floats, stream);
        if (rc != 1) return rc;
    }
    if ((bf3_mode() & 16) && d.stride == 1 && d.KH == 3 && d.KW == 3 && p.M > 64) {
        PatchGeom gq{};
        gq.in = x; gq.Hi = d.H; gq.Wi = d.W; gq.Ci = d.C; gq.Ho = p.g.Ho; gq.Wo = p.g.Wo; gq.KH = 3; gq.KW = 3;
        gq.off_h = -d.pad; gq.off_w = -d.pad; gq.flip = 0;
        const int rc = conv_patch_bf3_dispatch(p, gq, ws, ws_floats, stream);
        if (rc != 1) return rc;
    }
    return run_igemm(p, ws, ws_floats, stream);
}
int64_t obs_conv_weight_image_floats() { return ((int64_t)OCP_W_ELEMS + 1) / 2 + 4; }
int obs_conv_weight_image(const float* wf, int Cout, int KH, int KW, int C, void* img, hipStream_t stream) {
    return obs_conv_patch_weight_image(wf, Cout, KH, KW, C, reinterpret_cast<unsigned short*>(img), stream);
}
int obs_conv_fwd(const ConvDesc& d, const ObsView& obs, const float* wf, const float* bias, float* y, int relu, float* ws,
                 size_t ws_floats, hipStream_t stream, const void* wimg) {
    ObsConvFwdProb p;
    HAB_TRY(build(p, d, obs, wf, bias, y, relu));
    if ((bf3_mode() & 64) && (bf3_mode() & 2) && p.quad) {
        const int rc = obs_conv_patch_launch(p, ws, ws_floats, stream, reinterpret_cast<const unsigned short*>(wimg));
        if (rc != 1) return rc;
    }
    if ((bf3_mode() & 32) && (bf3_mode() & 2) && p.quad && p.M > 64) {
        const int rc = obs_conv_bf3_ws_launch(p, ws, ws_floats, stream);
        if (rc != 1) return rc;
    }
    if ((bf3_mode() & 2) && p.quad && p.M > 64) {
        const int rc = obs_conv_bf3_launch<2>(p, ws, ws_floats, stream);
        if (rc != 1) return rc;
    }
    return run_igemm(p, ws, ws_floats, stream);
}
__global__ void dgrad_empty_class_kernel(ConvDgradProb p) {
    const long long total = (long long)p.g.B * p.Hc * p.Wc * p.N;
    for (long long e = (long long)blockIdx.x * blockDim.x + threadIdx.x; e < total; e += (long long)gridDim.x * blockDim.x)
        p.store((int)(e / p.N), (int)(e % p.N), 0.f);
}

int conv_dgrad(const ConvDesc& d, const float* dy, const float* wd, const float* mask, const float* add, float* dx,
               float* ws, size_t ws_floats, hipStream_t stream) {
    if ((bf3_mode() & 512) && (bf3_mode() & 1)) {
        const int rc = conv2_dgrad_strip(d, dy, wd, mask, add, dx, stream);
        if (rc != 1) return rc;
    }
    if (d.stride > 1 && !no_dma() && !no_merged_dgrad()) {
        ConvDgradMergedProb q;
        HAB_TRY(check_conv(d));
        q.g = make_geom(d);
        if (ConvDgradMergedProb::applicable(q.g)) {
            q.dy = dy; q.w = wd; q.mask = mask; q.add = add; q.dx = dx;
            q.finish();
            if ((bf3_mode() & 1) && q.M > 64) {
                if (q.N <= 32) return bf3_launch<ConvDgradMergedProb, 2, 1, 4, 1>(q, ws, ws_floats, 256, stream);
                if (q.N <= 64) return bf3_launch<ConvDgradMergedProb, 1, 2, 4, 1>(q, ws, ws_floats, 256, stream);
                return bf3_launch<ConvDgradMergedProb, 2, 2, 2, 2>(q, ws, ws_floats, 256, stream);
            }
            if (q.dma_ok()) {
                if (q.N <= 32) return igemm_dma_launch<ConvDgradMergedProb, 2, 1, 4, 1, false>(q, ws, ws_floats, 1024, stream);
                if (q.N <= 64) return igemm_dma_launch<ConvDgradMergedProb, 1, 2, 4, 1, false>(q, ws, ws_floats, 1024, stream);
                return igemm_dma_launch<ConvDgradMergedProb, 2, 2, 2, 2, false>(q, ws, ws_floats, 1024, stream);
            }
        }
    }
    for (int ph = 0; ph < d.stride; ++ph)
        for (int pw = 0; pw < d.stride; ++pw) {
            ConvDgradProb p;
            HAB_TRY(build(p, d, dy, wd, mask, add, dx, ph, pw));
            if (p.Hc <= 0 || p.Wc <= 0) continue;
            if ((bf3_mode() & 16) && d.stride == 1 && d.KH == 3 && d.KW == 3 && p.M > 64 && p.K > 0) {
                PatchGeom gq{};
                gq.in = dy; gq.Hi = p.g.Ho; gq.Wi = p.g.Wo; gq.Ci = d.Cout; gq.Ho = d.H; gq.Wo = d.W; gq.KH = 3; gq.KW = 3;
                gq.off_h = d.pad - 2; gq.off_w = d.pad - 2; gq.flip = 1;
                const int rc = conv_patch_bf3_dispatch(p, gq, ws, ws_floats, stream);
                if (rc == HAB_OK) continue;
                if (rc != 1) return rc;
            }
            if (p.K <= 0) {
                p.M = d.B * p.Hc * p.Wc;
                dgrad_empty_class_kernel<<<1024, 256, 0, stream>>>(p);
                HAB_LAUNCH_CHECK();
                continue;
            }
            HAB_TRY(run_igemm(p, ws, ws_floats, stream));
        }
    return HAB_OK;
}
int conv_wgrad(const ConvDesc& d, const float* x, const float* dy, float* dw_oihw, float* dbias, float* ws, size_t ws_floats,
               hipStream_t stream) {
    ConvWgradProb p;
    HAB_TRY(build(p, d, x, dy, dw_oihw, dbias));
    if (ws && (bf3_mode() & 8) && (bf3_mode() & 128) && wgrad3x3_bf3_shape(p)) {
        const int rc = wgrad3x3_bf3(p, ws, ws_floats, stream);
        if (rc != 1) return rc;
    }
    if (ws && wgrad3x3_patch_ok(p) && !no_patch() && !(bf3_mode() & 8)) {
        ConvWgradProb q = p;
        q.colsum = nullptr;
        if (dbias) HAB_TRY(colsum(dy, p.N, p.K, p.N, dbias, 0, ws, ws_floats, stream));
        return wgrad3x3_patch(q, ws, ws_floats, stream);
    }
    if (ws && d.pad == 0 && p.N <= 32 && !no_dma() && !(bf3_mode() & 8)) {
        ConvWgradProb q = p;
        q.colsum = nullptr;
        if (wgrad_dma_ok(q)) {
            if (dbias) HAB_TRY(colsum(dy, p.N, p.K, p.N, dbias, 0, ws, ws_floats, stream));
            if ((q.M % 288 == 0) || (cdiv(q.M, 288) * 288 < cdiv(q.M, 256) * 256)) return igemm_dma_wgrad_launch<3, 3, 1>(q, ws, ws_floats, 1024, stream);
            return igemm_dma_wgrad_launch<2, 4, 1>(q, ws, ws_floats, 1024, stream);
        }
    }
    return run_igemm(p, ws, ws_floats, stream);
}
int obs_conv_wgrad(const ConvDesc& d, const ObsView& obs, const float* dy, float* dw_oihw, float* dbias, float* ws,
                   size_t ws_floats, hipStream_t stream) {
    ObsConvWgradProb p;
    HAB_TRY(build(p, d, obs, dy, dw_oihw, dbias));
    if ((bf3_mode() & 2) && p.quad && p.K > 4096) {
        const int rc = obs_wgrad_bf3_launch(p, ws, ws_floats, stream);
        if (rc != 1) return rc;
    }
    return run_igemm(p, ws, ws_floats, stream);
}
static bool dense_on() { return (bf3_mode() & 1024) && (bf3_mode() & 1); }
static bool dense_worth(long long M, long long N, long long K) {
    if (bf3_mode() & 2048) return true;
    static const long long min_flop = (long long)hab_env_int("HAB_DENSE_MIN_MFLOP", 4000) * 1000000LL;
    return 2 * M * N * K >= min_flop;
}
int linear_fwd(const float* x, int ldx, const float* w, int ldw, const float* bias, float* y, int ldy, int M, int N, int K,
               int relu, int accumulate, float* ws, size_t ws_floats, hipStream_t stream) {
    LinearFwdProb p;
    HAB_TRY(build(p, x, ldx, w, ldw, bias, y, ldy, M, N, K, relu, accumulate));
    if (dense_on() && dense_worth(M, N, K)) {
        DenseArgs g{};
        g.M = M; g.N = N; g.K = K; g.a = x; g.lda = ldx; g.b = w; g.ldb = ldw; g.c = y; g.ldc = ldy; g.bias = bias; g.relu = relu;
        g.accumulate = accumulate; g.partial = ws;
        g.a_bytes = ((long long)(M - 1) * ldx + K) * 4; g.b_bytes = ((long long)(N - 1) * ldw + K) * 4;
        if (dense_bf3_ok(g, false, false)) {
            g.nsplit = ws ? dense_bf3_splits(g, ws_floats) : 1;
            HAB_TRY((dense_bf3_launch<0, 0>(g, stream)));
            if (g.nsplit > 1) {
                igemm_splitk_reduce<LinearFwdProb>(p, ws, g.nsplit, stream);
                HAB_LAUNCH_CHECK();
            }
            return HAB_OK;
        }
    }
    return run_igemm(p, ws, ws_floats, stream);
}
int linear_dgrad(const float* dy, int lddy, const float* w, int ldw, const float* mask, int ldmask, int mask_cols, float* dx,
                 int lddx, int M, int Nin, int Kout, int accumulate, float* ws, size_t ws_floats, hipStream_t stream) {
// ... 136 lines not shown
        const size_t t = e / C;
        const int hw = (int)(t % HW);
        const size_t n = t / HW;
        wp[e] = w[(n * C + c) * HW + hw];
    }
}
int repack_flatten(const float* w, float* wp, int N, int C, int HW, hipStream_t stream) {
    if (!w || !wp || N <= 0 || C <= 0 || HW <= 0) return HAB_ERR_ARG;
    const size_t total = (size_t)N * C * HW;
    repack_flatten_kernel<<<(int)fmin(4096.0, (double)cdivl((long long)total, 256)), 256, 0, stream>>>(w, wp, N, C, HW);
    HAB_LAUNCH_CHECK();
    return HAB_OK;
}

__global__ void transpose_kernel(const float* __restrict__ w, float* __restrict__ wt, int R, int C) {
    __shared__ float tile[32][33];
    const int bx = blockIdx.x * 32, by = blockIdx.y * 32;
    for (int j = threadIdx.y; j < 32; j += blockDim.y) {
        const int r = by + j, c = bx + threadIdx.x;
        tile[j][threadIdx.x] = (r < R && c < C) ? w[(size_t)r * C + c] : 0.f;
    }
    __syncthreads();
    for (int j = threadIdx.y; j < 32; j += blockDim.y) {
        const int c = bx + j, r = by + threadIdx.x;
        if (c < C && r < R) wt[(size_t)c * R + r] = tile[threadIdx.x][j];
    }
}
__global__ void pad_rows_kernel(const float* __restrict__ w, float* __restrict__ wp, int R, int C, int ld) {
    const long long total = (long long)R * ld;
    for (long long e = (long long)blockIdx.x * blockDim.x + threadIdx.x; e < total; e += (long long)gridDim.x * blockDim.x) {
        const int c = (int)(e % ld);
        const long long r = e / ld;
        wp[e] = c < C ? w[r * C + c] : 0.f;
    }
}
int pad_rows(const float* w, float* wp, int R, int C, int ld, hipStream_t stream) {
    if (!w || !wp || R <= 0 || C <= 0 || ld < C) return HAB_ERR_ARG;
    const long long total = (long long)R * ld;
    pad_rows_kernel<<<(int)fmin(2048.0, (double)cdivl(total, 256)), 256, 0, stream>>>(w, wp, R, C, ld);
    HAB_LAUNCH_CHECK();
    return HAB_OK;
}
int transpose2d(const float* w, float* wt, int R, int C, hipStream_t stream) {
    if (!w || !wt || R <= 0 || C <= 0) return HAB_ERR_ARG;
    transpose_kernel<<<dim3(cdiv(C, 32), cdiv(R, 32)), dim3(32, 8), 0, stream>>>(w, wt, R, C);
    HAB_LAUNCH_CHECK();
    return HAB_OK;
}

}

using namespace hab;

static ConvDesc mk(int B, int H, int W, int C, int Cout, int KH, int KW, int stride, int pad) {
    ConvDesc d;
    d.B = B; d.H = H; d.W = W; d.C = C; d.Cout = Cout; d.KH = KH; d.KW = KW; d.stride = stride; d.pad = pad;
    return d;
}
static ObsView mkobs(const uint8_t* rgb, const float* depth, const int* rows, int H, int W) {
    ObsView o;
    o.rgb = rgb; o.depth = depth; o.rows = rows; o.H = H; o.W = W; o.C = (rgb ? 3 : 0) + (depth ? 1 : 0);
    return o;
}

extern "C" int hab_conv2d_fwd(const float* x, const float* w_fwd, const float* bias, float* y, int B, int H, int W, int C,
                              int Cout, int KH, int KW, int stride, int pad, int relu, float* ws, size_t ws_floats,
                              hipStream_t stream) {
    if (!x || !w_fwd || !y) return HAB_ERR_ARG;
    return conv_fwd(mk(B, H, W, C, Cout, KH, KW, stride, pad), x, w_fwd, bias, y, relu, ws, ws_floats, stream);
}
extern "C" int hab_obs_conv2d_fwd(const uint8_t* rgb, const float* depth, const int* rows, const float* w_fwd,
                                  const float* bias, float* y, int B, int H, int W, int Cout, int KH, int KW, int stride,
                                  int pad, int relu, float* ws, size_t ws_floats, hipStream_t stream) {
    if ((!rgb && !depth) || !w_fwd || !y) return HAB_ERR_ARG;
    ObsView o = mkobs(rgb, depth, rows, H, W);
    return obs_conv_fwd(mk(B, H, W, o.C, Cout, KH, KW, stride, pad), o, w_fwd, bias, y, relu, ws, ws_floats, stream);
}
extern "C" int hab_conv2d_dgrad(const float* dy, const float* w_dgrad, const float* relu_mask, const float* add, float* dx,
                                int B, int H, int W, int C, int Cout, int KH, int KW, int stride, int pad, float* ws,
                                size_t ws_floats, hipStream_t stream) {
    if (!dy || !w_dgrad || !dx) return HAB_ERR_ARG;
    return conv_dgrad(mk(B, H, W, C, Cout, KH, KW, stride, pad), dy, w_dgrad, relu_mask, add, dx, ws, ws_floats, stream);
}
extern "C" int hab_conv2d_wgrad(const float* x, const float* dy, float* dw_oihw, float* dbias, int B, int H, int W, int C, int Cout,
                                int KH, int KW, int stride, int pad, float* ws, size_t ws_floats, hipStream_t stream) {
    if (!x || !dy || !dw_oihw) return HAB_ERR_ARG;
    return conv_wgrad(mk(B, H, W, C, Cout, KH, KW, stride, pad), x, dy, dw_oihw, dbias, ws, ws_floats, stream);
}
extern "C" int hab_obs_conv2d_wgrad(const uint8_t* rgb, const float* depth, const int* rows, const float* dy, float* dw_oihw,
                                    float* dbias, int B, int H, int W, int Cout, int KH, int KW, int stride, int pad, float* ws,
                                    size_t ws_floats, hipStream_t stream) {
    if ((!rgb && !depth) || !dy || !dw_oihw) return HAB_ERR_ARG;
    ObsView o = mkobs(rgb, depth, rows, H, W);
    return obs_conv_wgrad(mk(B, H, W, o.C, Cout, KH, KW, stride, pad), o, dy, dw_oihw, dbias, ws, ws_floats, stream);
}
extern "C" int hab_linear_fwd(const float* x, int ldx, const float* w, int ldw, const float* bias, float* y, int ldy, int M,
                              int N, int K, int relu, int accumulate, float* ws, size_t ws_floats, hipStream_t stream) {
    return linear_fwd(x, ldx, w, ldw, bias, y, ldy, M, N, K, relu, accumulate, ws, ws_floats, stream);
}
extern "C" int hab_linear_dgrad(const float* dy, int lddy, const float* w, int ldw, const float* relu_mask, int ldmask,
                                float* dx, int lddx, int M, int n_in, int n_out, int accumulate, float* ws, size_t ws_floats,
                                hipStream_t stream) {
    return linear_dgrad(dy, lddy, w, ldw, relu_mask, ldmask, n_in, dx, lddx, M, n_in, n_out, accumulate, ws, ws_floats, stream);
}
extern "C" int hab_linear_wgrad(const float* dy, int lddy, const float* x, int ldx, float* dw, int lddw, int M, int n_out,
                                int n_in, int perm_c, int perm_hw, int accumulate, float* ws, size_t ws_floats,
                                hipStream_t stream) {
    return linear_wgrad(dy, lddy, x, ldx, dw, lddw, M, n_out, n_in, perm_c, perm_hw, accumulate, ws, ws_floats, stream);
}
extern "C" int hab_debug_dense_trace(long long* out320) {
    return (int)hipMemcpyFromSymbol(out320, HIP_SYMBOL(hab::dn_trace), sizeof(long long) * 8 * 8 * 5);
}
extern "C" int hab_colsum(const float* a, int lda, int M, int N, float* out, int accumulate, float* ws, size_t ws_floats,
                          hipStream_t stream) {
    return colsum(a, lda, M, N, out, accumulate, ws, ws_floats, stream);
}
extern "C" int hab_repack_conv_weight(const float* w_oihw, float* w_fwd, float* w_dgrad, int Cout, int Cin, int KH, int KW,
                                      int cin_padded, hipStream_t stream) {
    return repack_conv(w_oihw, w_fwd, w_dgrad, Cout, Cin, KH, KW, cin_padded, stream);
}
extern "C" int hab_repack_flatten_weight(const float* w, float* w_packed, int N, int C, int HW, hipStream_t stream) {
    return repack_flatten(w, w_packed, N, C, HW, stream);
}
extern "C" int hab_transpose2d(const float* w, float* wt, int R, int C, hipStream_t stream) {
    return transpose2d(w, wt, R, C, stream);
}
```

habitat-lab_amd/csrc/obs_conv_patch.h:

```cpp
#pragma once
#include <utility>

#include "igemm_bf3.h"

namespace hab {

constexpr int OCP_TH = 4;
constexpr int OCP_R = 4 * OCP_TH + 4;
constexpr int OCP_KP = 256 + 8;
constexpr int OCP_DP = 64 + 8;

constexpr int OCP_W_ELEMS = 3 * 32 * OCP_KP + 2 * 32 * OCP_DP;
__global__ void obs_patch_split_weights(const float* __restrict__ w, int N, unsigned short* __restrict__ img) {
    const int e = blockIdx.x * blockDim.x + threadIdx.x;
    if (e >= 32 * 256) return;
    const int n = e >> 8, k = e & 255, c = k & 3;
    float v = n < N ? w[(size_t)n * 256 + k] : 0.f;
    if (c < 3) v *= HAB_RCP255;
    unsigned h1, h2, h3;
    bf3_split(v, h1, h2, h3);
    img[(0 * 32 + n) * OCP_KP + k] = (unsigned short)h1;
    img[(1 * 32 + n) * OCP_KP + k] = (unsigned short)h2;
    img[(2 * 32 + n) * OCP_KP + k] = (unsigned short)h3;
    if (c == 3) {
        unsigned short* d = img + 3 * 32 * OCP_KP;
        const int kd = k >> 2;
        d[(0 * 32 + n) * OCP_DP + kd] = (unsigned short)h1;
        d[(1 * 32 + n) * OCP_DP + kd] = (unsigned short)h2;
    }
    if (k < 8) {
        img[(0 * 32 + n) * OCP_KP + 256 + k] = 0; img[(1 * 32 + n) * OCP_KP + 256 + k] = 0; img[(2 * 32 + n) * OCP_KP + 256 + k] = 0;
        unsigned short* d = img + 3 * 32 * OCP_KP;
        d[(0 * 32 + n) * OCP_DP + 64 + k] = 0; d[(1 * 32 + n) * OCP_DP + 64 + k] = 0;
    }
}

template <class F, int... Is>
__device__ __forceinline__ void ocp_static_for_impl(F& f, std::integer_sequence<int, Is...>) { (f(std::integral_constant<int, Is>()), ...); }
template <int N, class F>
__device__ __forceinline__ void ocp_static_for(F& f) { ocp_static_for_impl(f, std::make_integer_sequence<int, N>()); }

struct ObsPatchGeom {
    int W, H, Ho, Wo, tiles_per_img, ntiles;
    int units;
    int patch_elems;
};

template <int UPT>
__global__ void __launch_bounds__(512) obs_conv_patch_kernel(const ObsConvFwdProb p, const ObsPatchGeom gq, const unsigned short* __restrict__ wimg,
                                                              const int sign_schedule, const int ablate) {
    using P = ObsConvFwdProb;
    static_assert(EpiV4<P>::value, "transposed-accumulator epilogue");
    extern __shared__ __attribute__((aligned(16))) unsigned short smem16[];
    const int W = gq.W;
    const int t = threadIdx.x;
    const int lane = t & 63, wave = __builtin_amdgcn_readfirstlane(t >> 6), group = wave >> 2, gw = wave & 3, tg = t & 255;
    const int li = lane & 31, hi = lane >> 5;
    unsigned short* W12 = smem16;
    unsigned short* WD1 = W12 + 2 * 32 * OCP_KP;
    float* biasL = reinterpret_cast<float*>(WD1 + 32 * OCP_DP);
    unsigned short* P0 = WD1 + 32 * OCP_DP + 64 + group * gq.patch_elems;
    unsigned short* P1 = P0 + OCP_R * W * 4;
    unsigned short* P2 = P1 + OCP_R * W;

    for (int i = t; i < 2 * 32 * OCP_KP / 8; i += 512) reinterpret_cast<u32x4*>(W12)[i] = reinterpret_cast<const u32x4*>(wimg)[i];
    for (int i = t; i < 32 * OCP_DP / 8; i += 512) reinterpret_cast<u32x4*>(WD1)[i] = reinterpret_cast<const u32x4*>(wimg + 3 * 32 * OCP_KP)[i];
    if (t < 32) biasL[t] = (p.bias && t < p.N) ? p.bias[t] : 0.f;
    bf16x8 w3f[8][2], wd2f[4];
    {
        const unsigned short* w3 = wimg + 2 * 32 * OCP_KP + li * OCP_KP + hi * 8;
        const unsigned short* wd = wimg + 3 * 32 * OCP_KP + li * OCP_DP + hi * 8;
#pragma unroll
        for (int kh = 0; kh < 8; ++kh)
#pragma unroll
            for (int s = 0; s < 2; ++s) w3f[kh][s] = *reinterpret_cast<const bf16x8*>(w3 + kh * 32 + s * 16);
#pragma unroll
        for (int j = 0; j < 4; ++j) wd2f[j] = *reinterpret_cast<const bf16x8*>(wd + 32 * OCP_DP + j * 16);
    }

    auto tile_of = [&](int vb) {
        const int q = gq.ntiles >> 3, r = gq.ntiles & 7, xcd = vb & 7, idx = vb >> 3;
        return (xcd < r ? xcd * (q + 1) : r * (q + 1) + (xcd - r) * q) + idx;
    };

    struct Rgb12 { uint32_t d0, d1, d2; };
    Rgb12 rg[UPT];
    f32x4 dp[UPT];
    const int qpr = W >> 2;
    auto tile_base = [&](int tile, int& y0) {
        const int img = tile / gq.tiles_per_img;
        y0 = 4 * (tile - img * gq.tiles_per_img) * OCP_TH;
        return (size_t)p.obs.srow(img) * gq.H;
    };
    auto unit_pix = [&](size_t frame, int y0, int j, bool& ok) {
        const int u = tg + 256 * j;
        const int r = u / qpr, x4 = u - r * qpr;
        const int y = y0 + r;
        ok = (u < gq.units) & (y < gq.H);
        return (frame + (ok ? y : 0)) * W + 4 * (ok ? x4 : 0);
    };
    auto fetch_depth = [&](int tile) {
        if (ablate & 1) return;
        int y0;
        const size_t frame = tile_base(tile, y0);
#pragma unroll
        for (int j = 0; j < UPT; ++j) {
            bool ok;
            const size_t pix = unit_pix(frame, y0, j, ok);
            dp[j] = ld4(p.obs.depth + pix);
            if (!ok) dp[j] = zero4();
        }
    };
    auto fetch_rgb = [&](int tile) {
        if (ablate & 1) return;
        int y0;
        const size_t frame = tile_base(tile, y0);
#pragma unroll
        for (int j = 0; j < UPT; ++j) {
            bool ok;
            const size_t pix = unit_pix(frame, y0, j, ok);
            rg[j] = *reinterpret_cast<const Rgb12*>(p.obs.rgb + pix * 3);
            if (!ok) { rg[j].d0 = 0; rg[j].d1 = 0; rg[j].d2 = 0; }
        }
    };
    auto stage = [&]() {
        if (ablate & 8) return;
#pragma unroll
        for (int j = 0; j < UPT; ++j) {
            const int u = tg + 256 * j;
            if (u >= gq.units) continue;
            const unsigned d[3] = {rg[j].d0, rg[j].d1, rg[j].d2};
            unsigned f[12];
#pragma unroll
// ... 14 lines not shown
            *reinterpret_cast<u32x2*>(P1 + (size_t)u * 4) = r1;
            *reinterpret_cast<u32x2*>(P2 + (size_t)u * 4) = r2;
        }
    };

    const int a_px0 = (4 * gw) * W + 4 * li;
    f32x16 acc[2];
    bf16x8 fr[2][5];
    auto load_step = [&](auto stc) {
        constexpr int st = decltype(stc)::value, set = st & 1;
        if constexpr (st < 4) {
#pragma unroll
            for (int i = 0; i < 2; ++i) {
                const int px = a_px0 + (2 * st + hi) * W + 128 * i;
                u32x4 v1, v2;
                const u32x2 l1 = *reinterpret_cast<const u32x2*>(P1 + px), h1 = *reinterpret_cast<const u32x2*>(P1 + px + 4);
                const u32x2 l2 = *reinterpret_cast<const u32x2*>(P2 + px), h2 = *reinterpret_cast<const u32x2*>(P2 + px + 4);
                v1[0] = l1[0]; v1[1] = l1[1]; v1[2] = h1[0]; v1[3] = h1[1];
                v2[0] = l2[0]; v2[1] = l2[1]; v2[2] = h2[0]; v2[3] = h2[1];
                fr[set][i] = __builtin_bit_cast(bf16x8, v1);
                fr[set][2 + i] = __builtin_bit_cast(bf16x8, v2);
            }
            fr[set][4] = *reinterpret_cast<const bf16x8*>(WD1 + li * OCP_DP + (2 * st + hi) * 8);
        } else {
            constexpr int kh = (st - 4) >> 1, s_ = (st - 4) & 1;
#pragma unroll
            for (int i = 0; i < 2; ++i)
                fr[set][i] = *reinterpret_cast<const bf16x8*>(P0 + (size_t)(a_px0 + kh * W + 128 * i) * 4 + (2 * s_ + hi) * 8);
#pragma unroll
            for (int pl = 0; pl < 2; ++pl)
                fr[set][2 + pl] = *reinterpret_cast<const bf16x8*>(W12 + (pl * 32 + li) * OCP_KP + kh * 32 + s_ * 16 + hi * 8);
        }
    };
    auto flip = [&](bf16x8 f, const unsigned sgn) {
        u32x4 v = __builtin_bit_cast(u32x4, f);
        v[0] ^= sgn; v[1] ^= sgn; v[2] ^= sgn; v[3] ^= sgn;
        return __builtin_bit_cast(bf16x8, v);
    };
    auto mma_step = [&](auto stc, const unsigned sgn) {
        constexpr int st = decltype(stc)::value, set = st & 1;
        if constexpr (st < 4) {
            const bf16x8 a1[2] = {flip(fr[set][0], sgn), flip(fr[set][1], sgn)}, a2[2] = {flip(fr[set][2], sgn), flip(fr[set][3], sgn)};
            const bf16x8 wd1 = fr[set][4];
#pragma unroll
            for (int i = 0; i < 2; ++i) acc[i] = __builtin_amdgcn_mfma_f32_32x32x16_bf16(wd1, a2[i], acc[i], 0, 0, 0);
#pragma unroll
            for (int i = 0; i < 2; ++i) acc[i] = __builtin_amdgcn_mfma_f32_32x32x16_bf16(wd2f[st], a1[i], acc[i], 0, 0, 0);
#pragma unroll
            for (int i = 0; i < 2; ++i) acc[i] = __builtin_amdgcn_mfma_f32_32x32x16_bf16(wd1, a1[i], acc[i], 0, 0, 0);
        } else {
            constexpr int kh = (st - 4) >> 1, s_ = (st - 4) & 1;
            const bf16x8 a[2] = {flip(fr[set][0], sgn), flip(fr[set][1], sgn)};
#pragma unroll
            for (int i = 0; i < 2; ++i) acc[i] = __builtin_amdgcn_mfma_f32_32x32x16_bf16(w3f[kh][s_], a[i], acc[i], 0, 0, 0);
#pragma unroll
            for (int i = 0; i < 2; ++i) acc[i] = __builtin_amdgcn_mfma_f32_32x32x16_bf16(fr[set][3], a[i], acc[i], 0, 0, 0);
#pragma unroll
            for (int i = 0; i < 2; ++i) acc[i] = __builtin_amdgcn_mfma_f32_32x32x16_bf16(fr[set][2], a[i], acc[i], 0, 0, 0);
        }
    };
    auto matrix_phase = [&](const unsigned sgn) {
#pragma unroll
        for (int i = 0; i < 2; ++i)
#pragma unroll
            for (int v = 0; v < 16; ++v) acc[i][v] = 0.0f;
        if (ablate & 2) return;
        load_step(std::integral_constant<int, 0>());
        auto body = [&](auto stc) {
            constexpr int st = decltype(stc)::value;
            if constexpr (st + 1 < 20) load_step(std::integral_constant<int, st + 1>());
            mma_step(stc, sgn);
        };
        ocp_static_for<20>(body);
    };
    auto store_tile = [&](int tile, bool neg) {
        if ((ablate & 4) && acc[0][0] != 12345.f) return;
        const int img = tile / gq.tiles_per_img, ho = (tile - img * gq.tiles_per_img) * OCP_TH + gw;
        if (ho >= gq.Ho) return;
#pragma unroll
        for (int i = 0; i < 2; ++i) {
            const int wo = 32 * i + li;
            if (wo >= gq.Wo) continue;
            const size_t base = ((size_t)(img * gq.Ho + ho) * gq.Wo + wo) * p.N;
#pragma unroll
            for (int g = 0; g < 4; ++g) {
                const int n = 8 * g + 4 * hi;
                if (n + 3 >= p.N) continue;
                f32x4 v;
                v[0] = acc[i][4 * g]; v[1] = acc[i][4 * g + 1]; v[2] = acc[i][4 * g + 2]; v[3] = acc[i][4 * g + 3];
                if (neg) { v[0] = -v[0]; v[1] = -v[1]; v[2] = -v[2]; v[3] = -v[3]; }
                v += *reinterpret_cast<const f32x4*>(biasL + n);
                if (p.relu) { v[0] = fmaxf(v[0], 0.f); v[1] = fmaxf(v[1], 0.f); v[2] = fmaxf(v[2], 0.f); v[3] = fmaxf(v[3], 0.f); }
                if (p.y) *reinterpret_cast<f32x4*>(p.y + base + n) = v;
            }
        }
    };

    const int vstep = 2 * gridDim.x;
    const int vb0 = blockIdx.x + group * gridDim.x;
    const int n_mine = vb0 < gq.ntiles ? (gq.ntiles - vb0 + vstep - 1) / vstep : 0;
    const int n_first = (int)blockIdx.x < gq.ntiles ? (gq.ntiles - (int)blockIdx.x + vstep - 1) / vstep : 0;
    if (n_first == 0) return;
    if (n_mine > 0) { fetch_depth(tile_of(vb0)); if (group == 0) fetch_rgb(tile_of(vb0)); }
    if (group == 0) stage();
    __syncthreads();
    for (int pI = 0; pI <= 2 * n_first; ++pI) {
        if ((pI & 1) == group) {
            const int k = pI >> 1;
            if (k < n_mine) {
                if (k + 1 < n_mine) fetch_depth(tile_of(vb0 + (k + 1) * vstep));
                const int tile = tile_of(vb0 + k * vstep);
                matrix_phase((sign_schedule && (tile & 1)) ? 0x80008000u : 0u);
            }
        } else {
            const int kd = (pI - 1 - group) / 2;
            const int ks = (pI + 1 - group) / 2;
            if (ks < n_mine) {
                fetch_rgb(tile_of(vb0 + ks * vstep));
                stage();
            }
            if (pI >= 1 + group && kd < n_mine) {
                const int tile_d = tile_of(vb0 + kd * vstep);
                store_tile(tile_d, sign_schedule && (tile_d & 1));
            }
        }
        __syncthreads();
    }
}

inline int obs_conv_patch_weight_image(const float* w_packed, int N, int KH, int KW, int C, unsigned short* img, hipStream_t stream) {
    if (KH != 8 || KW != 8 || C != 4 || N > 32 || (N & 3) || !w_packed || !img || (reinterpret_cast<uintptr_t>(img) & 15)) return 1;
    obs_patch_split_weights<<<32, 256, 0, stream>>>(w_packed, N, img);
    HAB_LAUNCH_CHECK();
    return HAB_OK;
}

inline int obs_conv_patch_launch(const ObsConvFwdProb& p, float* ws, size_t ws_floats, hipStream_t stream, const unsigned short* wimg_cached = nullptr) {
    const ConvGeom& g = p.g;
    if (!p.quad || g.KH != 8 || g.KW != 8 || g.stride != 4 || g.pad != 0 || p.N > 32 || (p.N & 3) || p.K != 256 || g.W > 256 || (g.W & 3) || g.Wo > 64 ||
        g.Wo < 1 || p.M <= 0)
        return 1;
    if (!wimg_cached && (!ws || ws_floats * 4 < (size_t)OCP_W_ELEMS * 2 || (reinterpret_cast<uintptr_t>(ws) & 15))) return 1;
    if (reinterpret_cast<uintptr_t>(wimg_cached) & 15) return 1;
    ObsPatchGeom gq;
    gq.W = g.W; gq.H = g.H; gq.Ho = g.Ho; gq.Wo = g.Wo;
    gq.tiles_per_img = cdiv(g.Ho, OCP_TH);
    gq.ntiles = g.B * gq.tiles_per_img;
    gq.units = OCP_R * (g.W >> 2);
    if (cdiv(gq.units, 256) > 5) return 1;
    gq.patch_elems = OCP_R * g.W * 6 + 64;
    const size_t lds = ((size_t)2 * 32 * OCP_KP + 32 * OCP_DP + 64 + (size_t)2 * gq.patch_elems) * 2;
    if (lds > 160 * 1024) return 1;
    const unsigned short* wimg = wimg_cached;
    if (!wimg) {
        unsigned short* built = reinterpret_cast<unsigned short*>(ws);
        obs_patch_split_weights<<<32, 256, 0, stream>>>(p.w, p.N, built);
        HAB_LAUNCH_CHECK();
        wimg = built;
    }
    auto kern = obs_conv_patch_kernel<5>;
    static const hipError_t attr_err = hipFuncSetAttribute(reinterpret_cast<const void*>(kern), hipFuncAttributeMaxDynamicSharedMemorySize, 160 * 1024);
    if (attr_err != hipSuccess) return (int)attr_err;
    static const int sign_schedule = !hab_env_flag("HAB_BF3_NOSIGN");
    static const int ablate = hab_env_int("HAB_OCP_ABLATE", 0);
    const int pairs = (gq.ntiles + 1) / 2;
    const int grid = pairs < 256 ? (pairs + 7) / 8 * 8 : 256;
    kern<<<grid, 512, lds, stream>>>(p, gq, wimg, sign_schedule, ablate);
    HAB_LAUNCH_CHECK();
    return HAB_OK;
}

}
```

habitat-lab_amd/csrc/ops.h:

```cpp
#pragma once
#include "hab_common.h"

namespace hab {

struct ConvDesc {
    int B, H, W, C, Cout, KH, KW, stride, pad;
    int Creal = 0;
    int Ho() const { return (H + 2 * pad - KH) / stride + 1; }
    int Wo() const { return (W + 2 * pad - KW) / stride + 1; }
};
struct ObsView;

int conv_fwd(const ConvDesc& d, const float* x, const float* wf, const float* bias, float* y, int relu, float* ws,
             size_t ws_floats, hipStream_t stream);
int obs_conv_fwd(const ConvDesc& d, const ObsView& obs, const float* wf, const float* bias, float* y, int relu, float* ws,
                 size_t ws_floats, hipStream_t stream, const void* wimg = nullptr);
int64_t obs_conv_weight_image_floats();
int obs_conv_weight_image(const float* wf, int Cout, int KH, int KW, int C, void* img, hipStream_t stream);
int conv_dgrad(const ConvDesc& d, const float* dy, const float* wd, const float* mask, const float* add, float* dx,
               float* ws, size_t ws_floats, hipStream_t stream);
int conv_wgrad(const ConvDesc& d, const float* x, const float* dy, float* dw_oihw, float* dbias, float* ws, size_t ws_floats,
               hipStream_t stream);
int obs_conv_wgrad(const ConvDesc& d, const ObsView& obs, const float* dy, float* dw_oihw, float* dbias, float* ws,
                   size_t ws_floats, hipStream_t stream);
int linear_fwd(const float* x, int ldx, const float* w, int ldw, const float* bias, float* y, int ldy, int M, int N, int K,
               int relu, int accumulate, float* ws, size_t ws_floats, hipStream_t stream);
int linear_dgrad(const float* dy, int lddy, const float* w, int ldw, const float* mask, int ldmask, int mask_cols, float* dx,
                 int lddx, int M, int Nin, int Kout, int accumulate, float* ws, size_t ws_floats, hipStream_t stream);
int linear_wgrad(const float* dy, int lddy, const float* x, int ldx, float* dw, int lddw, int Mrows, int Nout, int Kin,
                 int perm_c, int perm_hw, int accumulate, float* ws, size_t ws_floats, hipStream_t stream);
int colsum(const float* a, int lda, int M, int N, float* out, int accumulate, float* ws, size_t ws_floats, hipStream_t stream);
int repack_conv(const float* w_oihw, float* wf, float* wd, int Cout, int Cin, int KH, int KW, int cpad, hipStream_t stream);
int repack_flatten(const float* w, float* wp, int N, int C, int HW, hipStream_t stream);
int transpose2d(const float* w, float* wt, int R, int C, hipStream_t stream);
int pad_rows(const float* w, float* wp, int R, int C, int ld, hipStream_t stream);

struct PackInfo {
    const int* select_inds;
    const int* step_offsets;
    const int* num_seqs_at_step;
    const int* frag_env;
    const int* frag_start;
    int P, F, max_len, n_envs;
};

struct RnnLayerParams {
    const float* w_ih; const float* w_hh; const float* b_ih; const float* b_hh;
    const float* w_hh_t;
    float* dw_ih; float* dw_hh; float* db_ih; float* db_hh;
    int in_dim;
    const float* w_ih_pad = nullptr;
    int w_ih_ld = 0;
};

struct RnnWork {
    float* gi;
    float* gates;
    float* hn;
    float* hprev;
    float* cprev;
    float* c;
    float* out;
    float* dgi;
    float* dgh;
};

int rnn_frag_init(const float* h0, const int* env_rows, int env_stride, const uint8_t* masks, const int* mask_rows,
                  const int* frag_env, const int* frag_start, int F, int H, float* hinit, hipStream_t stream,
                  const int* env_first = nullptr);
int rnn_seq_layer_forward(int rnn_type, int H, const RnnLayerParams& lp, const RnnWork& wk, const float* x, int ldx,
                          const float* hinit, const float* cinit, const PackInfo& pk, float* ws, size_t ws_floats,
                          hipStream_t stream);
int rnn_seq_wave_forward(int rnn_type, int H, int L, const RnnLayerParams* lp, const RnnWork* wk, const float* x, int ldx,
                         const float* const* hinit, const float* const* cinit, const PackInfo& pk, float* ws, size_t ws_floats,
                         hipStream_t stream);
int rnn_seq_wave_backward(int rnn_type, int H, int L, const RnnLayerParams* lp, const float* const* w_ih_t, const RnnWork* wk, const float* x0,
                          int ldx0, const float* dout, float* dx0, int lddx0, const float* dx_mask, int ldmask, int mask_cols,
                          const PackInfo& pk, float* scratch , float* ws, size_t ws_floats, hipStream_t stream);
int rnn_step_layer_forward(int rnn_type, int H, const RnnLayerParams& lp, const float* x, int ldx, const float* h_in, int h_in_stride,
                           const float* c_in, int c_in_stride, const uint8_t* masks, int n, float* gi_scratch, float* h_out,
                           int h_out_stride, float* c_out, int c_out_stride, float* ws, size_t ws_floats, hipStream_t stream);
int rnn_seq_layer_backward(int rnn_type, int H, const RnnLayerParams& lp, const RnnWork& wk, const float* x, int ldx,
                           const float* dout, float* dx, int lddx, const float* dx_mask, int ldmask, int mask_cols,
                           const PackInfo& pk, float* scratch , float* ws, size_t ws_floats,
                           hipStream_t stream);
int matrix_path_bits();
int rnn_tm_prepare(const uint8_t* masks, const int* rows, int B, uint8_t* frame_mask, int* iota, hipStream_t stream);
int rnn_tm_layer_forward(int rnn_type, int H, const RnnLayerParams& lp, const RnnWork& wk, const float* x, int ldx, const float* hinit,
                         const float* cinit, const uint8_t* frame_mask, int n, int T_total, int t0, int t1, float* ws, size_t ws_floats,
                         hipStream_t stream);
int rnn_tm_layer_backward(int rnn_type, int H, const RnnLayerParams& lp, const RnnWork& wk, const float* dout, float* dx, int lddx,
                          const float* dx_mask, int ldmask, int mask_cols, const uint8_t* frame_mask, const int* iota, int n, int T, int t0,
                          int t1, float* scratch, float* ws, size_t ws_floats, hipStream_t stream);
int rnn_tm_layer_param_grads(int rnn_type, int H, const RnnLayerParams& lp, const RnnWork& wk, const float* x, int ldx, int P, float* ws,
                             size_t ws_floats, hipStream_t stream);

}
```

habitat-lab_amd/csrc/problems.h:

```cpp
#pragma once
#include <math.h>

#include "hab_common.h"
#include "bf3_split.h"

namespace hab {

#define HAB_HD __host__ __device__ inline

HAB_HD f32x4 zero4() {
    f32x4 z;
    z[0] = 0.f; z[1] = 0.f; z[2] = 0.f; z[3] = 0.f;
    return z;
}
HAB_HD f32x4 ld4(const float* p) { return *reinterpret_cast<const f32x4*>(p); }

struct Raw4 { f32x4 v; int ok; };
struct KKey { int k, ok; };
HAB_HD KKey kkey(int k, int k_end) { KKey q; q.k = k; q.ok = k < k_end; return q; }
HAB_HD f32x4 sel4(const Raw4& r) { return r.ok ? r.v : zero4(); }
struct NoCtx {};
struct NoAux {};

constexpr int HAB_FAR = -(1 << 28);
// ... 265 lines not shown
    }
    HAB_HD AKey a_key(const KCtx&, int k, int k_end) const {
        AKey q;
        g.dKW.divmod(k >> 2, q.kh, q.kw);
        q.ok = k < k_end;
        return q;
    }
    HAB_HD ARaw a_fetch(const ACtx& c, const KCtx&, const AKey& q) const {
        if (quad) {
            const int h = c.h0 + q.kh, w_ = c.w0 + q.kw;
            const int ok = q.ok & ((unsigned)h < (unsigned)g.H) & ((unsigned)w_ < (unsigned)g.W);
            return obs_quad_fetch(obs, c.srow, h, w_, ok);
        }
        ARaw r;
        r.d0 = r.d1 = r.d2 = 0; r.dep = zero4(); r.ok = -1;
        return r;
    }
    HAB_HD void a_cvt(const ACtx& c, const ARaw& r, int k, int k_end, f32x4* out) const {
        if (r.ok >= 0) { obs_quad_cvt_raw(r, out); return; }
        for (int e = 0; e < 16; ++e) {
            const int kk = k + e;
            float v = 0.f;
            if (kk < k_end && c.h0 != HAB_FAR) {
                int tap, ci, kh, kw;
                g.dC.divmod(kk, tap, ci);
                g.dKW.divmod(tap, kh, kw);
                const int h = c.h0 + kh, w_ = c.w0 + kw;
                if ((unsigned)h < (unsigned)g.H && (unsigned)w_ < (unsigned)g.W) v = obs.get(c.srow, h, w_, ci);
            }
            out[e >> 2][e & 3] = v;
        }
    }
    HAB_HD BCtx b_ctx(int n) const { BCtx c; c.ok = n < N; c.row = c.ok ? w + (size_t)n * K : w; return c; }
    HAB_HD BKey b_key(const KCtx&, int k, int k_end) const { return kkey(k, k_end); }
    HAB_HD BRaw b_fetch(const BCtx& c, const KCtx&, const BKey& q) const {
        BRaw r;
        if ((K & 3) == 0) {
            r.ok = c.ok & q.ok;
            r.v = ld4(c.row + (q.k & -r.ok));
        } else {
            r.ok = 1;
            r.v = zero4();
            for (int e = 0; e < 4; ++e)
                if (c.ok && q.ok && q.k + e < K) r.v[e] = c.row[q.k + e];
        }
        return r;
    }
    HAB_HD f32x4 b_cvt(const BRaw& r) const {
        f32x4 v = sel4(r);
        if (quad) { v[0] *= HAB_RCP255; v[1] *= HAB_RCP255; v[2] *= HAB_RCP255; }
        return v;
    }
    using EpiCol = ColN;
    using EpiRow = RowBase;
    using EpiAux = NoAux;
    HAB_HD EpiCol epi_col(int n) const { EpiCol c; c.n = n; c.ok = n < N; c.bias = (bias && c.ok) ? bias[n] : 0.f; return c; }
    HAB_HD EpiRow epi_row(int m) const { EpiRow r; r.ok = m < M; r.base = (size_t)m * N; return r; }
    HAB_HD EpiAux epi_fetch(const EpiRow&, const EpiCol&) const { return EpiAux(); }
    HAB_HD void epi_store(const EpiRow& r, const EpiCol& c, const EpiAux&, float v) const {
        if (!(r.ok & c.ok)) return;
        v += c.bias;
        if (relu) v = v > 0.f ? v : 0.f;
        if (y) y[r.base + c.n] = v;
    }
    HAB_BIAS_RELU_VEC4
    HAB_GENERIC_STORE
};

struct ConvDgradProb {
    static constexpr bool A_RC = true, B_RC = true;
    int M, N, K;
    ConvGeom g;
    int ph, pw;
    int h_first, w_first;
    int Hc, Wc;
    int KHs, KWs;
    int Kfull;
    FastDiv dHcWc, dWc, dKWs;
    const float* dy;
    const float* w;
    const float* mask;
    const float* add;
    float* dx;
    HAB_HD const float* dma_a_origin() const { return dy; }
    HAB_HD const float* dma_b_origin() const { return w; }
    void set_class(int ph_, int pw_) {
        const int s = g.stride;
        ph = ph_; pw = pw_;
        h_first = ((ph - g.pad) % s + s) % s;
        w_first = ((pw - g.pad) % s + s) % s;
        Hc = h_first < g.H ? (g.H - h_first + s - 1) / s : 0;
        Wc = w_first < g.W ? (g.W - w_first + s - 1) / s : 0;
        KHs = ph < g.KH ? (g.KH - ph + s - 1) / s : 0;
        KWs = pw < g.KW ? (g.KW - pw + s - 1) / s : 0;
        Kfull = g.KH * g.KW * g.Cout;
        M = g.B * Hc * Wc; N = g.C; K = KHs * KWs * g.Cout;
        dHcWc = FastDiv(Hc * Wc > 0 ? Hc * Wc : 1); dWc = FastDiv(Wc > 0 ? Wc : 1); dKWs = FastDiv(KWs > 0 ? KWs : 1);
    }
    HAB_NO_KCTX
    struct ACtx { const float* base; int hq, wq, off0; };
    struct AKey { int a, b, koff, ok; };
    using BCtx = WRowCtx;
    struct BKey { int off, ok; };
    using ARaw = Raw4;
    using BRaw = Raw4;
    HAB_HD ACtx a_ctx(int m) const {
        ACtx c;
        if (m >= M) { c.base = dy; c.hq = HAB_FAR; c.wq = 0; c.off0 = 0; return c; }
        int img, rem, hc, wc;
        dHcWc.divmod(m, img, rem);
        dWc.divmod(rem, hc, wc);
        c.base = dy + (size_t)img * g.Ho * g.Wo * g.Cout;
        c.hq = (h_first + hc * g.stride + g.pad - ph) / g.stride;
        c.wq = (w_first + wc * g.stride + g.pad - pw) / g.stride;
        c.off0 = (c.hq * g.Wo + c.wq) * g.Cout;
        return c;
    }
    HAB_HD AKey a_key(const KCtx&, int k, int k_end) const {
        AKey q;
        int tap, co;
        g.dCout.divmod(k, tap, co);
        dKWs.divmod(tap, q.a, q.b);
        q.koff = co - (q.a * g.Wo + q.b) * g.Cout;
        q.ok = k < k_end;
        return q;
    }
    HAB_HD ARaw a_fetch(const ACtx& c, const KCtx&, const AKey& q) const {
        const int hs = c.hq - q.a, ws = c.wq - q.b;
        ARaw r;
        r.ok = q.ok & ((unsigned)hs < (unsigned)g.Ho) & ((unsigned)ws < (unsigned)g.Wo);
        r.v = ld4(c.base + ((c.off0 + q.koff) & -r.ok));
        return r;
    }
    HAB_HD BCtx b_ctx(int n) const { BCtx c; c.ok = n < N; c.row = c.ok ? w + (size_t)n * Kfull : w; return c; }
    HAB_HD BKey b_key(const KCtx&, int k, int k_end) const {
        BKey q;
        int tap, co, a, b;
        g.dCout.divmod(k, tap, co);
        dKWs.divmod(tap, a, b);
        q.off = ((ph + g.stride * a) * g.KW + (pw + g.stride * b)) * g.Cout + co;
        q.ok = k < k_end;
        return q;
    }
    HAB_HD BRaw b_fetch(const BCtx& c, const KCtx&, const BKey& q) const {
        BRaw r;
        r.ok = c.ok & q.ok;
        r.v = ld4(c.row + (q.off & -r.ok));
        return r;
    }
    HAB_HD bool dma_ok() const {
        return (g.Cout % 32 == 0) && (KHs * KWs <= 32) && (KWs < 32) && (K % 32 == 0) && ((size_t)g.Ho * g.Wo * g.Cout * 4 * 64 < 0x7fffffffull);
    }
    HAB_HD DmaTile dma_a_tile(int m0) const {
        DmaTile t;
        t.origin = dHcWc.div(m0 < M ? m0 : M - 1);
        const size_t shift = (size_t)((KHs - 1) * g.Wo + (KWs - 1)) * g.Cout;
        t.base = dy + (size_t)t.origin * g.Ho * g.Wo * g.Cout - shift;
        t.records = dma_records(((size_t)(g.B - t.origin) * g.Ho * g.Wo * g.Cout + shift) * 4);
        return t;
    }
    HAB_HD uint32_t dma_a_row(const DmaTile& t, int m, uint32_t& mask) const {
        mask = 0;
        if (m >= M) return 0;
        int img, rem, hc, wc;
        dHcWc.divmod(m, img, rem);
        dWc.divmod(rem, hc, wc);
        const int hq = (h_first + hc * g.stride + g.pad - ph) / g.stride, wq = (w_first + wc * g.stride + g.pad - pw) / g.stride;
        mask = tap_rect_mask(hq - g.Ho + 1 > 0 ? hq - g.Ho + 1 : 0, hq + 1 < KHs ? hq + 1 : KHs,
                             wq - g.Wo + 1 > 0 ? wq - g.Wo + 1 : 0, wq + 1 < KWs ? wq + 1 : KWs, KWs);
        return (uint32_t)((((img - t.origin) * g.Ho + hq) * g.Wo + wq) * g.Cout) * 4u;
    }
    HAB_HD void dma_tap(int k0, int& tap, uint32_t& sa, uint32_t& sb) const {
        int co0, a, b;
        g.dCout.divmod(k0, tap, co0);
        dKWs.divmod(tap, a, b);
        sa = (uint32_t)(((KHs - 1 - a) * g.Wo + (KWs - 1 - b)) * g.Cout + co0) * 4u;
        sb = (uint32_t)(((ph + g.stride * a) * g.KW + (pw + g.stride * b)) * g.Cout + co0) * 4u;
    }
    HAB_HD DmaTile dma_b_tile(int n0) const {
        DmaTile t;
        t.origin = n0;
        t.base = w + (size_t)n0 * Kfull;
        t.records = dma_records((size_t)(N - n0) * Kfull * 4);
        return t;
    }
    HAB_HD uint32_t dma_b_row(const DmaTile& t, int n, uint32_t& ok) const { ok = n < N; return (uint32_t)(n - t.origin) * (uint32_t)Kfull * 4u; }
    HAB_PLAIN_CVT
    struct EpiCol { int n, ok; };
    using EpiRow = RowBase;
    struct EpiAux { float add, mask; };
    HAB_HD EpiCol epi_col(int n) const { EpiCol c; c.n = n; c.ok = n < N; return c; }
    HAB_HD EpiRow epi_row(int m) const {
        EpiRow r;
        r.ok = m < M;
        int img, rem, hc, wc;
        dHcWc.divmod(r.ok ? m : 0, img, rem);
        dWc.divmod(rem, hc, wc);
        r.base = ((((size_t)img * g.H) + h_first + hc * g.stride) * g.W + w_first + wc * g.stride) * N;
        return r;
    }
    HAB_HD EpiAux epi_fetch(const EpiRow& r, const EpiCol& c) const {
        EpiAux a;
        const size_t i = (r.ok & c.ok) ? r.base + c.n : 0;
        a.add = add ? add[i] : 0.f;
        a.mask = mask ? mask[i] : 1.f;
        return a;
    }
    HAB_HD void epi_store(const EpiRow& r, const EpiCol& c, const EpiAux& a, float v) const {
        if (!(r.ok & c.ok)) return;
        v += a.add;
        if (!(a.mask > 0.f)) v = 0.f;
        if (dx) dx[r.base + c.n] = v;
    }
    static constexpr bool EPI_VEC4 = true;
    struct EpiCol4 { int n, ok, tail; };
    using EpiAux4 = AddMask4;
    HAB_HD EpiCol4 epi_col4(int n) const { EpiCol4 c; c.n = n; c.ok = ((N & 3) == 0) & (n + 3 < N); c.tail = (n < N) & !c.ok; return c; }
    HAB_HD EpiAux4 epi_fetch4(const EpiRow& r, const EpiCol4& c) const {
        EpiAux4 a;
        const size_t i = (r.ok & c.ok) ? r.base + c.n : 0;
        a.add = add ? ld4(add + i) : zero4();
        a.mask = mask ? ld4(mask + i) : splat4(1.f);
        return a;
    }
    HAB_HD void epi_store4(const EpiRow& r, const EpiCol4& c, const EpiAux4& a, f32x4 v) const {
        if (!r.ok) return;
        if (c.ok) {
            v += a.add;
#pragma unroll
            for (int e = 0; e < 4; ++e)
                if (!(a.mask[e] > 0.f)) v[e] = 0.f;
            if (dx) *reinterpret_cast<f32x4*>(dx + r.base + c.n) = v;
        } else if (c.tail) {
            for (int e = 0; e < 4; ++e) {
                const EpiCol ce = epi_col(c.n + e);
                epi_store(r, ce, epi_fetch(r, ce), v[e]);
            }
        }
    }
    HAB_GENERIC_STORE
};

struct ConvDgradMergedProb {
    int M, N, K;
    ConvGeom g;
    int Hq, Wq, KHs, KWs, Kfull;
    FastDiv dHqWq, dWq, dKWs;
    const float* dy;
    const float* w;
    const float* mask;
    const float* add;
    float* dx;
    HAB_HD const float* dma_a_origin() const { return dy; }
    HAB_HD const float* dma_b_origin() const { return w; }
    static bool applicable(const ConvGeom& g) {
        return g.stride > 1 && g.KH % g.stride == 0 && g.KW % g.stride == 0 && g.Cout % 32 == 0 && g.C % 8 == 0 &&
               g.stride * g.stride * g.C <= 128;
    }
    void finish() {
        const int s = g.stride;
        Hq = (g.H - 1 + g.pad) / s + 1; Wq = (g.W - 1 + g.pad) / s + 1;
        KHs = g.KH / s; KWs = g.KW / s;
        Kfull = g.KH * g.KW * g.Cout;
        M = g.B * Hq * Wq; N = s * s * g.C; K = KHs * KWs * g.Cout;
        dHqWq = FastDiv(Hq * Wq); dWq = FastDiv(Wq); dKWs = FastDiv(KWs);
    }
    static constexpr bool A_RC = true, B_RC = true;
    HAB_NO_KCTX
    struct ACtx { const float* base; int hq, wq; };
    struct AKey { int a, b, co, ok; };
    using BCtx = WRowCtx;
    struct BKey { int koff, ok; };
    using ARaw = Raw4;
    using BRaw = Raw4;
    HAB_HD ACtx a_ctx(int m) const {
        ACtx c;
        if (m >= M) { c.base = dy; c.hq = HAB_FAR; c.wq = 0; return c; }
        int img, rem;
        dHqWq.divmod(m, img, rem);
        dWq.divmod(rem, c.hq, c.wq);
        c.base = dy + (size_t)img * g.Ho * g.Wo * g.Cout;
        return c;
    }
    HAB_HD AKey a_key(const KCtx&, int k, int k_end) const {
        AKey q;
        int tap;
        g.dCout.divmod(k, tap, q.co);
        dKWs.divmod(tap, q.a, q.b);
        q.ok = k < k_end;
        return q;
    }
    HAB_HD ARaw a_fetch(const ACtx& c, const KCtx&, const AKey& q) const {
        const int h = c.hq - q.a, w_ = c.wq - q.b;
        ARaw r;
        r.ok = q.ok & ((unsigned)h < (unsigned)g.Ho) & ((unsigned)w_ < (unsigned)g.Wo);
        r.v = ld4(c.base + (((h * g.Wo + w_) * g.Cout + q.co) & -r.ok));
        return r;
    }
    HAB_HD BCtx b_ctx(int n) const {
        BCtx c;
        c.ok = n < N;
        int pp, ci;
        g.dC.divmod(c.ok ? n : 0, pp, ci);
        const int ph = pp / g.stride, pw = pp - ph * g.stride;
        c.row = w + (size_t)ci * Kfull + (ph * g.KW + pw) * g.Cout;
// ... 477 lines not shown
```

habitat-lab_amd/habitat_amd/_lib.py:

```python
from __future__ import annotations

import ctypes as C
import os
from ctypes import POINTER, c_char_p, c_double, c_float, c_int, c_int32, c_int64, c_size_t, c_uint8, c_uint32, c_void_p

_HERE = os.path.dirname(os.path.abspath(__file__))
LIB_PATH = os.path.join(_HERE, "libhabitat_amd.so")

vp = c_void_p
ALLREDUCE_FN = C.CFUNCTYPE(None, c_void_p, c_int, c_float, c_void_p)
GRAD_READY_FN = C.CFUNCTYPE(None, c_int64, c_int64, c_void_p)


class HabError(RuntimeError):
    pass


class PolicyDesc(C.Structure):
    _fields_ = [(n, c_int32) for n in (
        "arch", "backbone", "baseplanes", "normalize_visual_inputs", "rnn_type", "rnn_layers", "hidden", "num_actions",
        "H", "W", "has_rgb", "has_depth", "goal_dim", "max_frames", "max_envs", "visual_order", "has_semantic",
        "num_object_categories", "has_compass", "has_gps", "action_dist", "gauss_flags")] + [("gauss_min_std", c_float),
                                                                                                ("gauss_max_std", c_float),
                                                                                                ("pointgoal_dim", c_int32),
                                                                                                ("proximity_dim", c_int32),
                                                                                                ("num_visual", c_int32),
                                                                                                ("visual_dtype", c_int32 * 4),
                                                                                                ("visual_channels", c_int32 * 4),
                                                                                                ("visual_scale", c_float * 4),
                                                                                                ("num_fused", c_int32),
                                                                                                ("fused_width", c_int32 * 8)]


MAX_VISUAL, MAX_FUSED = 4, 8
DTYPE_U8, DTYPE_F32, DTYPE_I32 = 0, 1, 2


GAUSS_TANH_MU, GAUSS_USE_LOG_STD, GAUSS_USE_SOFTPLUS, GAUSS_USE_STD_PARAM, GAUSS_CLAMP_STD = 1, 2, 4, 8, 16


class Obs(C.Structure):
    _fields_ = [("rgb", vp), ("depth", vp), ("goal", vp), ("prev_actions", vp), ("semantic", vp), ("objectgoal", vp), ("compass", vp),
                ("gps", vp), ("visual_features", vp), ("pointgoal", vp), ("proximity", vp), ("visual", vp * 4), ("fused", vp * 8)]


class EmbedSlot(C.Structure):
    _fields_ = [("kind", c_int32), ("input", vp), ("weight", vp), ("bias", vp), ("d_weight", vp), ("d_bias", vp), ("num_tokens", c_int32)]


class PackInfo(C.Structure):
    _fields_ = [("select_inds", vp), ("frag_env", vp), ("frag_start", vp), ("step_offsets_host", vp),
                ("num_seqs_at_step_host", vp), ("P", c_int32), ("F", c_int32), ("max_len", c_int32), ("env_first_frame", vp)]


SIGNATURES = {
    "hab_abi_version": (c_int, []),
    "hab_error_string": (c_char_p, [c_int]),
    "hab_synth_step": (c_int, [vp, vp, vp, vp, vp, vp, vp, c_uint32, c_uint32, c_int, c_int, c_int, c_int, vp]),
    "hab_synth_objectnav_sensors": (c_int, [vp, vp, vp, vp, vp, c_uint32, c_uint32, c_int, c_int, c_int, vp]),
    "hab_nav2d_state_bytes": (c_int, []),
    "hab_nav2d_step": (c_int, [vp] * 13 + [c_uint32, c_uint32] + [c_int] * 7 + [vp]),
    "hab_obs_resize_crop": (c_int, [vp, vp, c_int, c_int, c_int, c_int, c_int, c_int, c_int, c_int, c_int, c_int, c_int, c_int, vp]),
    "hab_obs_resize_crop_form": (c_int, [vp, c_int, c_int, c_int, c_int, c_int, c_int, c_int, c_int]),
    "hab_obs_project": (c_int, [vp, c_int, vp, c_int, c_int, c_int, c_int, c_int, vp, vp, c_int, c_int, vp]),
    "hab_rollout_step_stats": (c_int, [vp, vp, vp, vp, vp, vp, vp, c_int, c_int, vp]),
    "hab_compute_returns": (c_int, [vp, vp, vp, vp, vp, c_int, c_int, c_float, c_float, c_int, c_int, vp]),
    "hab_advantages": (c_int, [vp, vp, vp, c_int, c_int, vp, vp, vp]),
    "hab_ppo_loss": (c_int, [vp, vp, vp, vp, vp, vp, vp, vp, c_int, c_float, c_float, c_float, c_int, vp, vp, vp, vp, vp]),
    "hab_ppo_loss_ver": (c_int, [vp, vp, vp, vp, vp, vp, vp, vp, c_int, c_float, c_float, c_float, c_int, vp, vp, vp, c_int64, vp, c_float,
                                 vp, vp, vp, vp, vp]),
    "hab_lagrange_adam_step": (c_int, [vp, vp, vp, vp, c_float, c_float, c_float, c_float, c_float, c_int, c_float, c_float, vp, vp]),
    "hab_ver_compute_returns": (c_int, [vp, vp, vp, vp, vp, vp, vp, vp, c_int, c_double, c_double, vp]),
    "hab_ver_is_coeffs": (c_int, [vp, c_int, c_int, c_int, vp, vp, vp]),
    "hab_clip_adam_step": (c_int, [vp, vp, vp, vp, c_size_t, vp, c_int, c_float, c_float, c_float, c_float, c_float,
                                   c_float, c_int, vp, vp]),
    "hab_sample_actions": (c_int, [vp, vp, vp, c_int, c_int, c_int, vp]),
    "hab_set_matrix_path": (c_int, [c_int]),
    "hab_conv2d_fwd": (c_int, [vp, vp, vp, vp] + [c_int] * 10 + [vp, c_size_t, vp]),
    "hab_obs_conv2d_fwd": (c_int, [vp, vp, vp, vp, vp, vp] + [c_int] * 9 + [vp, c_size_t, vp]),
    "hab_conv2d_dgrad": (c_int, [vp, vp, vp, vp, vp] + [c_int] * 9 + [vp, c_size_t, vp]),
    "hab_conv2d_wgrad": (c_int, [vp, vp, vp, vp] + [c_int] * 9 + [vp, c_size_t, vp]),
    "hab_obs_conv2d_wgrad": (c_int, [vp, vp, vp, vp, vp, vp] + [c_int] * 8 + [vp, c_size_t, vp]),
    "hab_linear_fwd": (c_int, [vp, c_int, vp, c_int, vp, vp, c_int, c_int, c_int, c_int, c_int, c_int, vp, c_size_t, vp]),
    "hab_linear_dgrad": (c_int, [vp, c_int, vp, c_int, vp, c_int, vp, c_int, c_int, c_int, c_int, c_int, vp, c_size_t, vp]),
    "hab_linear_wgrad": (c_int, [vp, c_int, vp, c_int, vp, c_int, c_int, c_int, c_int, c_int, c_int, c_int, vp, c_size_t, vp]),
    "hab_colsum": (c_int, [vp, c_int, c_int, c_int, vp, c_int, vp, c_size_t, vp]),
    "hab_repack_conv_weight": (c_int, [vp, vp, vp, c_int, c_int, c_int, c_int, c_int, vp]),
    "hab_repack_flatten_weight": (c_int, [vp, vp, c_int, c_int, c_int, vp]),
    "hab_transpose2d": (c_int, [vp, vp, c_int, c_int, vp]),
    "hab_obs_ingest_pool": (c_int, [vp, vp, vp, vp, vp, c_int, c_int, c_int, c_int, c_int, c_int, c_int, vp]),
    "hab_obs_ingest_pool_sensors": (c_int, [vp, vp, vp, vp, c_int, vp, vp, c_int, c_int, c_int, c_int, vp, vp, vp, vp, vp, vp]),
    "hab_fused_gather": (c_int, [vp, vp, c_int, vp, vp, c_int, c_int, c_int, c_int, c_int, vp]),
    "hab_channel_moments": (c_int, [vp, c_int64, c_int, c_int, vp, vp, vp, c_int, vp]),
    "hab_running_mean_var_update": (c_int, [vp, vp, vp, vp, vp, c_float, c_int, vp]),
    "hab_running_mean_var_normalize": (c_int, [vp, c_int64, c_int, c_int, vp, vp, vp]),
    "hab_groupnorm_fwd": (c_int, [vp, vp, vp, vp, vp, vp, vp, c_int, c_int, c_int, c_int, c_int, c_float, vp, c_int64, vp]),
    "hab_groupnorm_bwd": (c_int, [vp, vp, vp, vp, vp, vp, vp, vp, vp, c_int, c_int, c_int, c_int, vp, c_int64, vp]),
    "hab_split_weight_planes": (c_int, [vp, c_int, c_int, vp, vp]),
    "hab_stem_split_weights": (c_int, [vp, vp, vp]),
    "hab_stem_conv_wgrad": (c_int, [vp, vp, vp, c_int, c_int, c_int, c_int, vp, c_size_t, vp, vp]),
    "hab_stem_conv_fwd": (c_int, [vp, vp, vp, c_int, c_int, c_int, vp, vp, c_int, vp]),
    "hab_conv_gn_fwd": (c_int, [vp] * 9 + [c_int] * 11 + [c_float, vp]),
    "hab_maxpool3x3s2_fwd": (c_int, [vp, vp, vp, c_int, c_int, c_int, c_int, vp]),
    "hab_maxpool3x3s2_bwd": (c_int, [vp, vp, vp, c_int, c_int, c_int, c_int, vp]),
    "hab_nav_embed_fwd": (c_int, [POINTER(EmbedSlot), c_int, vp, vp, vp, c_int, c_int, c_int, vp, vp]),
    "hab_nav_embed_bwd": (c_int, [POINTER(EmbedSlot), c_int, vp, vp, c_int, c_int, c_int, vp, c_size_t, vp]),
    "hab_build_pack_info": (c_int, [vp, c_int, c_int] + [vp] * 12),
    "hab_build_pack_info_from_ids": (c_int, [vp, vp, vp, c_int] + [vp] * 11),
    "hab_policy_create": (c_int, [POINTER(PolicyDesc), POINTER(vp)]),
    "hab_policy_destroy": (None, [vp]),
    "hab_policy_num_params": (c_int, [vp]),
    "hab_policy_param_info": (c_int, [vp, c_int, c_char_p, c_int, POINTER(c_int64), POINTER(c_int), POINTER(c_int64)]),
    "hab_policy_param_is_buffer": (c_int, [vp, c_int]),
    "hab_policy_set_training": (c_int, [vp, c_int]),
    "hab_comm_available": (c_int, []),
    "hab_comm_unique_id": (c_int, [vp]),
    "hab_comm_create": (c_int, [vp, c_int, c_int, vp]),
    "hab_comm_destroy": (None, [vp]),
    "hab_comm_world_size": (c_int, [vp]),
    "hab_comm_allreduce_sum": (c_int, [vp, vp, c_int64, vp]),
    "hab_policy_set_comm": (c_int, [vp, vp]),
    "hab_policy_grad_sync": (c_int, [vp, vp]),
    "hab_policy_set_grad_ready": (c_int, [vp, GRAD_READY_FN, vp]),
    "hab_policy_set_allreduce": (c_int, [vp, ALLREDUCE_FN, vp, c_int]),
    "hab_policy_param_floats": (c_int64, [vp]),
    "hab_policy_packed_floats": (c_int64, [vp]),
    "hab_policy_work_floats": (c_int64, [vp]),
    "hab_policy_bind": (c_int, [vp, vp, vp, vp, vp, c_int64]),
    "hab_policy_repack": (c_int, [vp, vp]),
    "hab_policy_encode": (c_int, [vp, POINTER(Obs), c_int, vp, vp]),
    "hab_policy_visual_feature_shape": (c_int, [vp, POINTER(c_int), POINTER(c_int), POINTER(c_int)]),
    "hab_policy_act": (c_int, [vp, POINTER(Obs), vp, vp, vp, c_int, c_int, vp, vp, vp, vp, vp, vp]),
    "hab_policy_evaluate": (c_int, [vp, POINTER(Obs), vp, vp, c_int, vp, vp, POINTER(PackInfo), c_int, c_int, vp, vp, vp, vp]),
    "hab_policy_final_hidden": (c_int, [vp, vp, vp]),
    "hab_policy_set_extra_grads": (c_int, [vp, vp, vp]),
    "hab_policy_backward": (c_int, [vp, POINTER(Obs), vp, vp, POINTER(PackInfo), vp, vp, vp, vp]),
    "hab_policy_probe_enable": (c_int, [vp, c_int]),
    "hab_policy_probe_read": (c_int, [vp, POINTER(c_double), POINTER(c_int)]),
    "hab_policy_probe_enable_mask": (c_int, [vp, C.c_uint64]),
    "hab_policy_probe_read_tag": (c_int, [vp, c_int, POINTER(c_double), POINTER(c_int)]),
    "hab_policy_probe_work": (c_int, [vp, c_int, POINTER(c_double), POINTER(c_double)]),
    "hab_policy_tap": (c_int, [vp, c_int, POINTER(vp), POINTER(c_int64)]),
}

_lib = None


def lib():
    global _lib
    if _lib is None:
        if not os.path.exists(LIB_PATH):
            raise HabError(
                f"{LIB_PATH} is missing: build it with `make -C habitat-lab_amd/csrc` (or __graft_entry__.build()). "
                "habitat_amd has no CPU / PyTorch fallback for its kernels.")
        import torch
        L = C.CDLL(LIB_PATH)
        for name, (res, args) in SIGNATURES.items():
            fn = getattr(L, name)
            fn.restype = res
            fn.argtypes = args
        _lib = L
    return _lib

# ... 18 lines not shown
```

include/habitat_amd.h:

```cpp
#ifndef HABITAT_AMD_H
#define HABITAT_AMD_H

#include <stddef.h>
#include <stdint.h>

#ifdef __cplusplus
extern "C" {
#endif

#ifndef __HIP_PLATFORM_AMD__
typedef struct ihipStream_t* hipStream_t;
#endif

#define HAB_ABI_VERSION 1
int hab_abi_version(void);
const char* hab_error_string(int code);

int hab_synth_step(uint8_t* rgb , float* depth , float* goal , float* reward ,
                   uint8_t* not_done , int64_t* env_t , int64_t* since_reset , uint32_t seed,
                   uint32_t env_offset, int N, int H, int W, int advance, hipStream_t stream);
int hab_synth_objectnav_sensors(int32_t* semantic, int64_t* objectgoal, float* compass, float* gps, const int64_t* env_t,
                                uint32_t seed, uint32_t env_offset, int N, int H, int W, hipStream_t stream);

#define HAB_NAV2D_STATE_BYTES 224
// ... 6 lines not shown
#define HAB_NAV2D_W_HEADING 7
#define HAB_NAV2D_W_STEPS 8
#define HAB_NAV2D_W_COLLISIONS 9
#define HAB_NAV2D_W_EPISODE 10
#define HAB_NAV2D_W_ENDED 11
#define HAB_NAV2D_W_LAST_MEASURES 12
int hab_nav2d_state_bytes(void);
int hab_nav2d_step(void* state , const float* dirs, const float* ray, const float* col_cos,
                   const float* tanv, const int64_t* actions , const uint8_t* mask , uint8_t* rgb ,
                   float* depth , float* goal , float* reward , uint8_t* not_done ,
                   float* measure_sums , uint32_t seed, uint32_t env_offset, int N, int H, int W, int num_obstacles,
                   int num_headings, int max_episode_steps, int advance, hipStream_t stream);

#define HAB_DTYPE_U8 0
#define HAB_DTYPE_F32 1
#define HAB_DTYPE_I32 2
#define HAB_RESIZE_AREA 0
#define HAB_RESIZE_NEAREST 1
int hab_obs_resize_crop(const void* src, void* dst, int dtype, int N, int H, int W, int C, int resized_h, int resized_w,
                        int crop_y0, int crop_x0, int out_h, int out_w, int mode, hipStream_t stream);
#define HAB_RESIZE_FORM_GENERIC 0
#define HAB_RESIZE_FORM_TILE 1
#define HAB_RESIZE_FORM_RGB8 2
int hab_obs_resize_crop_form(const void* src, int dtype, int N, int H, int W, int C, int resized_h, int resized_w, int mode);

int hab_obs_project(const void* const* src, int n_src, void* dst, int dtype, int N, int H, int W, int C, const void* table,
                    const float* zfactor, int out_h, int out_w, hipStream_t stream);

int hab_rollout_step_stats(const float* rewards, const uint8_t* not_done, float* current_episode_reward, float* stat_reward,
                           float* stat_count, const int64_t* actions , int64_t* prev_actions_next, int N,
                           int action_dim, hipStream_t stream);

#define HAB_GAE_EXACT 0
#define HAB_GAE_SCAN 1
int hab_compute_returns(const float* rewards, float* value_preds, const uint8_t* masks, float* returns,
                        const float* next_value , int T, int N, float gamma, float tau, int use_gae,
                        int variant, hipStream_t stream);

#define HAB_ADV_RAW 0
#define HAB_ADV_LOCAL_NORMALIZE 1
#define HAB_ADV_STATS_MEAN 2
#define HAB_ADV_EXT_NORMALIZE 3
#define HAB_ADV_STATS_VAR 4
int hab_advantages(const float* returns, const float* value_preds, float* adv, int count, int mode,
                   const float* ext_stats, float* stats_out, hipStream_t stream);

int hab_ppo_loss(const float* values, const float* logp, const float* entropy, const float* old_logp,
                 const float* adv, const float* old_values, const float* returns, const int* rows, int B,
                 float clip_param, float value_loss_coef, float entropy_coef, int use_clipped_value_loss,
                 float* d_value, float* d_logp, float* d_entropy, float* out12, hipStream_t stream);

int hab_ppo_loss_ver(const float* values, const float* logp, const float* entropy, const float* old_logp, const float* adv,
                     const float* old_values, const float* returns, const int* rows, int B, float clip_param, float value_loss_coef,
                     float entropy_coef, int use_clipped_value_loss, const float* is_coeffs, const uint8_t* is_stale,
                     const int64_t* policy_version, int64_t current_policy_version, const float* log_alpha, float entropy_threshold,
                     float* d_value, float* d_logp, float* d_entropy, float* out20, hipStream_t stream);
int hab_lagrange_adam_step(float* log_alpha, float* exp_avg, float* exp_avg_sq, const float* grad, float grad_scale, float lr, float beta1,
                           float beta2, float eps, int step, float log_alpha_min, float log_alpha_max,
                           float* alpha_out , hipStream_t stream);

int hab_ver_compute_returns(const float* rewards, const float* value_preds, const uint8_t* is_stale, float* returns,
                            const int32_t* select_inds, const int32_t* step_offsets, const int32_t* sequence_lengths,
                            const uint8_t* last_sequence_in_batch_mask, int F, double gamma, double tau, hipStream_t stream);
int hab_ver_is_coeffs(const int64_t* environment_ids, int n, int num_envs, int num_steps, int32_t* counts_scratch, float* is_coeffs,
                      hipStream_t stream);

int hab_clip_adam_step(float* params, const float* grads, float* exp_avg, float* exp_avg_sq, size_t n,
                       double* scratch_partials, int scratch_len, float grad_scale, float max_grad_norm, float lr,
                       float beta1, float beta2, float eps, int step, float* grad_norm_out, hipStream_t stream);

int hab_sample_actions(const float* probs, const float* exp_noise, int64_t* actions, int n, int A, int deterministic,
                       hipStream_t stream);

int hab_set_matrix_path(int mode);

int hab_conv2d_fwd(const float* x, const float* w_fwd, const float* bias, float* y, int B, int H, int W, int C, int Cout,
                   int KH, int KW, int stride, int pad, int relu, float* ws, size_t ws_floats, hipStream_t stream);
int hab_obs_conv2d_fwd(const uint8_t* rgb, const float* depth, const int* rows, const float* w_fwd, const float* bias,
                       float* y, int B, int H, int W, int Cout, int KH, int KW, int stride, int pad, int relu, float* ws,
                       size_t ws_floats, hipStream_t stream);
int hab_conv2d_dgrad(const float* dy, const float* w_dgrad, const float* relu_mask, const float* add, float* dx, int B,
                     int H, int W, int C, int Cout, int KH, int KW, int stride, int pad, float* ws, size_t ws_floats,
                     hipStream_t stream);
int hab_conv2d_wgrad(const float* x, const float* dy, float* dw_oihw, float* dbias, int B, int H, int W, int C, int Cout,
                     int KH, int KW, int stride, int pad, float* ws, size_t ws_floats, hipStream_t stream);
int hab_obs_conv2d_wgrad(const uint8_t* rgb, const float* depth, const int* rows, const float* dy, float* dw_oihw,
                         float* dbias, int B, int H, int W, int Cout, int KH, int KW, int stride, int pad, float* ws,
                         size_t ws_floats, hipStream_t stream);
int hab_linear_fwd(const float* x, int ldx, const float* w, int ldw, const float* bias, float* y, int ldy, int M, int N,
                   int K, int relu, int accumulate, float* ws, size_t ws_floats, hipStream_t stream);
int hab_linear_dgrad(const float* dy, int lddy, const float* w, int ldw, const float* relu_mask, int ldmask, float* dx,
                     int lddx, int M, int n_in, int n_out, int accumulate, float* ws, size_t ws_floats,
                     hipStream_t stream);
int hab_linear_wgrad(const float* dy, int lddy, const float* x, int ldx, float* dw, int lddw, int M, int n_out, int n_in,
                     int perm_c, int perm_hw, int accumulate, float* ws, size_t ws_floats, hipStream_t stream);
int hab_colsum(const float* a, int lda, int M, int N, float* out, int accumulate, float* ws, size_t ws_floats,
               hipStream_t stream);
int hab_repack_conv_weight(const float* w_oihw, float* w_fwd, float* w_dgrad, int Cout, int Cin, int KH, int KW,
                           int cin_padded, hipStream_t stream);
int hab_repack_flatten_weight(const float* w, float* w_packed, int N, int C, int HW, hipStream_t stream);
int hab_transpose2d(const float* w, float* wt, int R, int C, hipStream_t stream);

int hab_obs_ingest_pool(const uint8_t* rgb, const float* depth, const int32_t* semantic, const int* rows, float* y, int B, int H, int W,
                        int cpad, int c_rgb, int c_depth, int c_sem ,
                        hipStream_t stream);
int hab_obs_ingest_pool_sensors(const void* const* sensors, const int32_t* dtypes, const int32_t* channels, const float* scales, int n,
                                const int* rows, float* y, int B, int H, int W, int cpad, const float* norm_mean, const float* norm_var,
                                const float* pivot, double* mom_partial, int* mom_blocks, hipStream_t stream);
int hab_fused_gather(const float* const* sensors, const int32_t* widths, int n, const int* rows, float* dst, int ld, int col0, int pad0,
                     int npad, int B, hipStream_t stream);
int hab_channel_moments(const float* x, int64_t npix, int cpad, int mode, const float* mean, float* out, double* scratch,
                        int scratch_len, hipStream_t stream);
int hab_running_mean_var_update(float* r_mean, float* r_var, float* r_count, const float* b_mean, const float* b_var, float n, int C,
                                hipStream_t stream);
int hab_running_mean_var_normalize(float* x, int64_t npix, int cpad, int C, const float* mean, const float* var, hipStream_t stream);
int hab_groupnorm_fwd(const float* x, float* y, const float* gamma, const float* beta, const float* residual, float* mean,
                      float* rstd, int B, int HW, int C, int groups, int relu, float eps, float* ws, int64_t ws_floats,
                      hipStream_t stream);
int hab_groupnorm_bwd(const float* x, const float* dy, const float* relu_out, float* dx, float* dy_masked, const float* gamma,
                      const float* mean, const float* rstd, float* chan_sums, int B, int HW, int C, int groups, float* ws,
                      int64_t ws_floats, hipStream_t stream);
int hab_split_weight_planes(const float* w_fwd, int Cout, int K, uint16_t* planes, hipStream_t stream);
int hab_stem_split_weights(const float* w_fwd, uint16_t* planes, hipStream_t stream);
int hab_stem_conv_fwd(const float* x, const uint16_t* w_planes, float* y, int B, int H, int W, const float* norm, float* gn_part, int gn_groups,
                      hipStream_t stream);
int hab_stem_conv_wgrad(const float* x, const float* dy, float* dw_oihw, int B, int H, int W, int creal, float* ws, size_t ws_floats,
                        const float* norm, hipStream_t stream);
int hab_conv_gn_fwd(const float* x, const uint16_t* w_planes, const float* gamma, const float* beta, const float* residual, float* y,
                    float* raw, float* mean, float* rstd, int B, int H, int W, int C, int Cout, int KH, int KW, int stride, int pad,
                    int groups, int relu, float eps, hipStream_t stream);
int hab_maxpool3x3s2_fwd(const float* x, float* y, uint8_t* idx, int B, int H, int W, int C, hipStream_t stream);
int hab_maxpool3x3s2_bwd(const float* dy, const uint8_t* idx, float* dx, int B, int H, int W, int C, hipStream_t stream);
#define HAB_EMB_POLAR 0
#define HAB_EMB_TOKEN 1
#define HAB_EMB_COSSIN 2
#define HAB_EMB_LIN2 3
#define HAB_EMB_PREV 4
#define HAB_EMB_PREVLIN 5
#define HAB_EMB_LINN 6
typedef struct hab_embed_slot {
    int32_t kind;
    const void* input;
    const float* weight;
    const float* bias;
    float* d_weight;
    float* d_bias;
    int32_t num_tokens;
} hab_embed_slot;
int hab_nav_embed_fwd(const hab_embed_slot* slots, int nslots, const uint8_t* masks, const int* rows, float* out, int ld, int col0, int B,
                      float* saved, hipStream_t stream);
int hab_nav_embed_bwd(const hab_embed_slot* slots, int nslots, const float* saved, const float* dout, int ld, int col0, int B, float* ws,
                      size_t ws_floats, hipStream_t stream);

int hab_build_pack_info(const uint8_t* dones, int T, int N, int64_t* select_inds, int64_t* num_seqs_at_step,
                        int64_t* sequence_starts, int64_t* sequence_lengths, int64_t* rnn_state_batch_inds,
                        uint8_t* last_sequence_in_batch_mask, uint8_t* first_sequence_in_batch_mask,
                        int64_t* last_sequence_in_batch_inds, int64_t* first_episode_in_batch_inds,
                        int64_t* first_step_for_env, int32_t* num_fragments, int32_t* max_len);
int hab_build_pack_info_from_ids(const int64_t* episode_ids, const int64_t* environment_ids, const int64_t* step_ids, int P,
                                 int64_t* select_inds, int64_t* num_seqs_at_step, int64_t* sequence_starts, int64_t* sequence_lengths,
                                 int64_t* rnn_state_batch_inds, uint8_t* last_sequence_in_batch_mask,
                                 uint8_t* first_sequence_in_batch_mask, int64_t* first_step_for_env, int32_t* num_fragments,
                                 int32_t* max_len, int32_t* num_envs);

#define HAB_ARCH_SIMPLE_CNN 0
#define HAB_ARCH_RESNET 1
// ... 66 lines not shown
    const int32_t* frag_env;
    const int32_t* frag_start;
    const int32_t* step_offsets_host;
    const int32_t* num_seqs_at_step_host;
    int32_t P, F, max_len;
    const int32_t* env_first_frame;
} hab_pack_info;

typedef struct hab_policy hab_policy;

int hab_policy_create(const hab_policy_desc* desc, hab_policy** out);
void hab_policy_destroy(hab_policy* p);
int hab_policy_num_params(const hab_policy* p);
int hab_policy_param_info(const hab_policy* p, int i, char* name, int name_cap, int64_t* shape4, int* ndim,
                          int64_t* offset_floats);
int hab_policy_param_is_buffer(const hab_policy* p, int i);
int64_t hab_policy_param_floats(const hab_policy* p);
int64_t hab_policy_packed_floats(const hab_policy* p);
int64_t hab_policy_work_floats(const hab_policy* p);
int hab_policy_bind(hab_policy* p, float* params, float* grads, float* packed, float* work, int64_t work_floats);
int hab_policy_repack(hab_policy* p, hipStream_t stream);
int hab_policy_set_training(hab_policy* p, int training);
typedef void (*hab_allreduce_fn)(float* buf, int n, float scale, void* ctx);
int hab_policy_set_allreduce(hab_policy* p, hab_allreduce_fn fn, void* ctx, int world_size);
typedef void (*hab_grad_ready_fn)(int64_t first, int64_t count, void* ctx);
int hab_policy_set_grad_ready(hab_policy* p, hab_grad_ready_fn fn, void* ctx);
typedef struct hab_comm hab_comm;
int hab_comm_available(void);
int hab_comm_unique_id(uint8_t* out128);
int hab_comm_create(const uint8_t* id128, int world, int rank, hab_comm** out);
void hab_comm_destroy(hab_comm* c);
int hab_comm_world_size(const hab_comm* c);
int hab_comm_allreduce_sum(hab_comm* c, float* buf, int64_t count, hipStream_t stream);
int hab_policy_set_comm(hab_policy* p, hab_comm* c);
int hab_policy_grad_sync(hab_policy* p, hipStream_t stream);
int hab_policy_encode(hab_policy* p, const hab_obs* obs, int n, float* out, hipStream_t stream);
int hab_policy_visual_feature_shape(const hab_policy* p, int* c, int* hf, int* wf);
int hab_policy_act(hab_policy* p, const hab_obs* obs, const float* hidden_in, const uint8_t* masks,
                   const float* exp_noise, int deterministic, int n, float* values, int64_t* actions,
                   float* action_log_probs, float* hidden_out, float* probs_out , hipStream_t stream);
int hab_policy_evaluate(hab_policy* p, const hab_obs* obs, const int* rows, const float* hidden0, int hidden_env_stride,
                        const uint8_t* masks, const int64_t* actions, const hab_pack_info* pack, int B, int n,
                        float* value, float* log_prob, float* entropy, hipStream_t stream);
int hab_policy_final_hidden(hab_policy* p, float* hidden_out, hipStream_t stream);
int hab_policy_backward(hab_policy* p, const hab_obs* obs, const int* rows, const int64_t* actions,
                        const hab_pack_info* pack, const float* d_value, const float* d_log_prob, const float* d_entropy,
                        hipStream_t stream);

int hab_policy_set_extra_grads(hab_policy* p, const float* d_rnn_output, const float* d_perception_embed);

#define HAB_PROBE_CONV1_FWD 0
#define HAB_PROBE_CONV2_FWD 1
#define HAB_PROBE_CONV3_FWD 2
#define HAB_PROBE_FC_FWD 3
#define HAB_PROBE_CONV1_WGRAD 4
#define HAB_PROBE_CONV2_WGRAD 5
#define HAB_PROBE_CONV3_WGRAD 6
#define HAB_PROBE_CONV2_DGRAD 7
#define HAB_PROBE_CONV3_DGRAD 8
#define HAB_PROBE_FC_WGRAD 9
#define HAB_PROBE_FC_DGRAD 10
#define HAB_PROBE_ENC_FWD 11
#define HAB_PROBE_ENC_BWD 12
#define HAB_PROBE_RNN_FWD 13
#define HAB_PROBE_RNN_BWD 14
#define HAB_PROBE_RN_WGRAD_IM2COL 15
int hab_policy_probe_enable(hab_policy* p, int tag );
int hab_policy_probe_enable_mask(hab_policy* p, uint64_t mask);
int hab_policy_probe_read(hab_policy* p, double* total_ms, int* count);
int hab_policy_probe_read_tag(hab_policy* p, int tag, double* total_ms, int* count);
int hab_policy_probe_work(hab_policy* p, int tag, double* flops, double* bytes);

#define HAB_TAP_CONV1 0
#define HAB_TAP_CONV2 1
#define HAB_TAP_CONV3 2
#define HAB_TAP_RNN_IN 3
#define HAB_TAP_RNN_OUT 4
#define HAB_TAP_ENC_IN 5
#define HAB_TAP_STEM 6
#define HAB_TAP_POOL 7
#define HAB_TAP_COMPRESSION 8
#define HAB_TAP_LAYER1 9
#define HAB_TAP_POOL_IDX 13
#define HAB_TAP_CONV_OUT 100
int hab_policy_tap(hab_policy* p, int which, const float** ptr, int64_t* floats);

#ifdef __cplusplus
}
#endif
#endif
```

Before: 62630 env-steps/s.

## Emit packed ReLU bitmasks in conv forward and consume them in dgrad

The conv1 and conv2 forward kernels now also write a 1-bit-per-element ReLU mask, built with DPP lane ORs. The conv dgrad paths (strip kernel and generic epilogue) read these bits instead of the full f32 activation tensor to apply the ReLU gradient mask. This cuts mask read traffic in backward by about 32x and prefetches the mask bits alongside dy. The cost is extra workspace, extra stores in forward, and new template variants. The feature is on by default through the bf3 mode bit.

```diff
diff --git a/habitat-lab_amd/csrc/conv2_dgrad_strip.h b/habitat-lab_amd/csrc/conv2_dgrad_strip.h
--- a/habitat-lab_amd/csrc/conv2_dgrad_strip.h
+++ b/habitat-lab_amd/csrc/conv2_dgrad_strip.h
@@ -1,6 +1,7 @@
 #pragma once
 #include "igemm_bf3.h"
 #include "ops.h"
+#include "relu_bits.h"
 
 namespace hab {
 
@@ -8,6 +9,7 @@
     const float* dy;
     const float* wd;
     const float* mask;
+    const uint32_t* mask_bits;
     float* dx;
     int B;
     int strips, items;
@@ -27,7 +29,7 @@
     static_assert(CELLS % R2 == 0, "");
 };
 
-template <int R2, bool RT>
+template <int R2, bool RT, bool MB>
 __global__ void __launch_bounds__(512) conv2_dgrad_strip_kernel(const C2dArgs a) {
     using Cfg = C2dCfg<R2>;
     constexpr int NT = Cfg::NT;
@@ -71,6 +73,7 @@
         }
 
     f32x4 yr[Cfg::YPT];
+    unsigned mbn[MB ? 2 * R2 : 1], mbc[MB ? 2 * R2 : 1];
     int pf_h20 = 0;
     auto fetch = [&](int item) {
         const int img = item / a.strips, h20 = (item - img * a.strips) * R2;
@@ -82,6 +85,14 @@
             const bool ok = (RT ? u < YU : (Cfg::YU % NT == 0 || u < Cfg::YU)) && (unsigned)row < (unsigned)Ho;
             const size_t off = ok ? ((size_t)img * Ho + row) * (size_t)(Wo * 64) + (size_t)(u - r * (Wo * 16)) * 4 : 0;
             yr[j] = *reinterpret_cast<const f32x4*>(a.dy + off);
+        }
+        if constexpr (MB) {
+#pragma unroll
+            for (int k = 0; k < 2 * R2; ++k) {
+                const int idx = t + (k & 1) * NT, rph = idx >> 9, cell = (idx >> 4) & 31, cq = idx & 15;
+                const int h = 2 * (h20 + (k >> 1)) + rph, w = 2 * cell + (cq >> 3);
+                mbn[k] = a.mask_bits[(h < H && w < W) ? ((size_t)img * H + h) * W + w : (size_t)0];
+            }
         }
     };
     auto stage = [&]() {
@@ -94,6 +105,10 @@
             unsigned short* dst = ys + pixidx * 64 + (((c4 >> 1) ^ ((pixidx >> 1) & 7)) << 3) + (c4 & 1) * 4;
             const bool in_image = (unsigned)(pf_h20 - 1 + r) < (unsigned)Ho;
             bf3_store4(in_image ? yr[j] : f32x4{0.f, 0.f, 0.f, 0.f}, dst, dst + Cfg::Y_PLANE, dst + 2 * Cfg::Y_PLANE);
+        }
+        if constexpr (MB) {
+#pragma unroll
+            for (int k = 0; k < 2 * R2; ++k) mbc[k] = mbn[k];
         }
     };
 
@@ -109,7 +124,7 @@
             const int pixidx = (tr + 1 - ta) * Cfg::YCOLS + li + 1 - tb;
             const int swz = (pixidx >> 1) & 7;
             f32x4 mk[2];
-            if (a.mask) {
+            if (!MB && a.mask) {
 #pragma unroll
                 for (int q = 0; q < 2; ++q) {
                     const int idx = t + q * NT, rph = idx >> 9, cell = (idx >> 4) & 31, cq = idx & 15;
@@ -157,7 +172,14 @@
                 const int h = 2 * h2 + rph, w = 2 * cell + (cq >> 3);
                 if (h < H && w < W) {
                     const size_t off = (((size_t)img * H + h) * W + w) * 32 + (cq & 7) * 4;
-                    if (a.mask) {
+                    if constexpr (MB) {
+                        unsigned m = mbc[q];
+#pragma unroll
+                        for (int r = 1; r < R2; ++r) m = tr == r ? mbc[2 * r + q] : m;
+                        m >>= (cq & 7) * 4;
+#pragma unroll
+                        for (int e = 0; e < 4; ++e) s[e] = ((m >> e) & 1u) ? s[e] : 0.f;
+                    } else if (a.mask) {
                         const f32x4 m = mk[q];
 #pragma unroll
                         for (int e = 0; e < 4; ++e) s[e] = m[e] > 0.f ? s[e] : 0.f;
@@ -174,15 +196,16 @@
     return d.KH == 4 && d.KW == 4 && d.stride == 2 && d.pad == 0 && d.C == 32 && d.Cout == 64 && d.H >= 4 && d.W >= 4 && d.H <= 63 && d.W <= 63;
 }
 
-inline int conv2_dgrad_strip(const ConvDesc& d, const float* dy, const float* wd, const float* mask, const float* add, float* dx,
-                             hipStream_t stream) {
+inline int conv2_dgrad_strip(const ConvDesc& d, const float* dy, const float* wd, const float* mask, const uint32_t* mask_bits, const float* add,
+                             float* dx, hipStream_t stream) {
     if (!conv2_dgrad_strip_covers(d)) return 1;
     if (add || d.B < 16 || !dy || !wd || !dx) return 1;
     if ((reinterpret_cast<uintptr_t>(dy) | reinterpret_cast<uintptr_t>(wd) | reinterpret_cast<uintptr_t>(dx) | reinterpret_cast<uintptr_t>(mask)) & 15) return 1;
+    if (reinterpret_cast<uintptr_t>(mask_bits) & 3) return 1;
     constexpr int R2 = 2;
     using Cfg = C2dCfg<R2>;
     C2dArgs a;
-    a.dy = dy; a.wd = wd; a.mask = mask; a.dx = dx; a.B = d.B;
+    a.dy = dy; a.wd = wd; a.mask = mask; a.mask_bits = mask_bits; a.dx = dx; a.B = d.B;
     a.H = d.H; a.W = d.W; a.Ho = (d.H - 4) / 2 + 1; a.Wo = (d.W - 4) / 2 + 1;
     a.strips = ((d.H + 1) / 2 + R2 - 1) / R2;
     if ((long long)d.B * a.strips > 0x7fffffffLL) return 1;
@@ -190,17 +213,27 @@
     static const int sign_schedule = !hab_env_flag("HAB_BF3_NOSIGN");
     a.sign_schedule = sign_schedule;
     static const hipError_t attr_err = [] {
-        const hipError_t e0 = hipFuncSetAttribute(reinterpret_cast<const void*>(conv2_dgrad_strip_kernel<R2, false>),
-                                                  hipFuncAttributeMaxDynamicSharedMemorySize, (int)Cfg::LDS_BYTES);
-        const hipError_t e1 = hipFuncSetAttribute(reinterpret_cast<const void*>(conv2_dgrad_strip_kernel<R2, true>),
-                                                  hipFuncAttributeMaxDynamicSharedMemorySize, (int)Cfg::LDS_BYTES);
-        return e0 != hipSuccess ? e0 : e1;
+        const void* kerns[4] = {reinterpret_cast<const void*>(conv2_dgrad_strip_kernel<R2, false, false>),
+                                reinterpret_cast<const void*>(conv2_dgrad_strip_kernel<R2, true, false>),
+                                reinterpret_cast<const void*>(conv2_dgrad_strip_kernel<R2, false, true>),
+                                reinterpret_cast<const void*>(conv2_dgrad_strip_kernel<R2, true, true>)};
+        for (const void* k : kerns) {
+            const hipError_t e0 = hipFuncSetAttribute(k, hipFuncAttributeMaxDynamicSharedMemorySize, (int)Cfg::LDS_BYTES);
+            if (e0 != hipSuccess) return e0;
+        }
+        return hipSuccess;
     }();
     if (attr_err != hipSuccess) return (int)attr_err;
     int grid = 256;
     while (grid > 8 && grid > a.items) grid -= 8;
-    if (d.H == 63 && d.W == 63) conv2_dgrad_strip_kernel<R2, false><<<grid, Cfg::NT, Cfg::LDS_BYTES, stream>>>(a);
-    else conv2_dgrad_strip_kernel<R2, true><<<grid, Cfg::NT, Cfg::LDS_BYTES, stream>>>(a);
+    const bool bench_geom = d.H == 63 && d.W == 63;
+    if (mask_bits) {
+        if (bench_geom) conv2_dgrad_strip_kernel<R2, false, true><<<grid, Cfg::NT, Cfg::LDS_BYTES, stream>>>(a);
+        else conv2_dgrad_strip_kernel<R2, true, true><<<grid, Cfg::NT, Cfg::LDS_BYTES, stream>>>(a);
+    } else {
+        if (bench_geom) conv2_dgrad_strip_kernel<R2, false, false><<<grid, Cfg::NT, Cfg::LDS_BYTES, stream>>>(a);
+        else conv2_dgrad_strip_kernel<R2, true, false><<<grid, Cfg::NT, Cfg::LDS_BYTES, stream>>>(a);
+    }
     HAB_LAUNCH_CHECK();
     return HAB_OK;
 }
diff --git a/habitat-lab_amd/csrc/conv2_fwd_strip.h b/habitat-lab_amd/csrc/conv2_fwd_strip.h
--- a/habitat-lab_amd/csrc/conv2_fwd_strip.h
+++ b/habitat-lab_amd/csrc/conv2_fwd_strip.h
@@ -1,5 +1,6 @@
 #pragma once
 #include "igemm_bf3.h"
+#include "relu_bits.h"
 
 namespace hab {
 
@@ -8,6 +9,7 @@
     const float* wf;
     const float* bias;
     float* y;
+    uint32_t* bits;
     int B;
     int strips, items;
     int relu, sign_schedule;
@@ -153,7 +155,12 @@
                 for (int e = 0; e < 4; ++e) s[e] = s[e] > 0.f ? s[e] : 0.f;
             }
             const int op = pt * 32 + rpix;
-            if (RT ? op < npix_here : (Cfg::NPIX % 32 == 0 || op < Cfg::NPIX)) *reinterpret_cast<f32x4*>(yb + (size_t)op * 64 + rco) = s;
+            const bool op_ok = RT ? op < npix_here : (Cfg::NPIX % 32 == 0 || op < Cfg::NPIX);
+            if (op_ok) *reinterpret_cast<f32x4*>(yb + (size_t)op * 64 + rco) = s;
+            if (a.bits) {
+                const unsigned wbits = or_over_8_lanes(relu_bits4(s) << (rco & 31));
+                if (op_ok && (t & 7) == 0) a.bits[(((size_t)img * Ho + ho0) * Wo + op) * 2 + ((t >> 3) & 1)] = wbits;
+            }
         }
         __syncthreads();
     }
@@ -163,15 +170,16 @@
     return g.KH == 4 && g.KW == 4 && g.stride == 2 && g.pad == 0 && g.C == 32 && g.Cout == 64 && g.H >= 4 && g.W >= 4 && g.W <= 63;
 }
 
-inline int conv2_fwd_strip(const ConvFwdProb& p, float* , size_t , hipStream_t stream) {
+inline int conv2_fwd_strip(const ConvFwdProb& p, float* , size_t , hipStream_t stream, uint32_t* relu_bits = nullptr) {
     const ConvGeom& g = p.g;
     if (!conv2_fwd_strip_covers(g)) return 1;
+    if (relu_bits && (!p.relu || (reinterpret_cast<uintptr_t>(relu_bits) & 3))) return HAB_ERR_ARG;
     if ((p.ldy != 0 && p.ldy != 64) || g.B < 16) return 1;
     if ((reinterpret_cast<uintptr_t>(p.x) | reinterpret_cast<uintptr_t>(p.w) | reinterpret_cast<uintptr_t>(p.y) | reinterpret_cast<uintptr_t>(p.bias)) & 15) return 1;
     constexpr int R = 2;
     using Cfg = C2fCfg<R>;
     C2fArgs a;
-    a.x = p.x; a.wf = p.w; a.bias = p.bias; a.y = p.y; a.B = g.B;
+    a.x = p.x; a.wf = p.w; a.bias = p.bias; a.y = p.y; a.bits = relu_bits; a.B = g.B;
     a.H = g.H; a.W = g.W; a.Ho = (g.H - 4) / 2 + 1; a.Wo = (g.W - 4) / 2 + 1;
     a.strips = (a.Ho + R - 1) / R;
     if ((long long)g.B * a.strips > 0x7fffffffLL) return 1;
diff --git a/habitat-lab_amd/csrc/engine.h b/habitat-lab_amd/csrc/engine.h
--- a/habitat-lab_amd/csrc/engine.h
+++ b/habitat-lab_amd/csrc/engine.h
@@ -54,6 +54,8 @@
     std::vector<int64_t> pk_wiht;
     int64_t pk_wih0 = -1;
     int64_t w_a1 = -1, w_a2 = -1, w_a3 = -1, w_da1 = -1, w_da2 = -1, w_da3 = -1;
+    int64_t w_m1 = -1, w_m2 = -1;
+    int bits_a1 = 0, bits_a2 = 0;
     int64_t w_rnnin = -1, w_drnnin = -1, w_hinit = -1, w_cinit = -1, w_probs = -1, w_logitsn = -1, w_dzv = -1, w_dv = -1, w_dfeat = -1,
             w_scratch = -1, w_value = -1, w_logp = -1, w_ent = -1, w_hmask = -1, w_gistep = -1, w_step_h = -1, w_ws = -1;
     std::vector<int64_t> w_gi, w_gates, w_hn, w_hprev, w_cprev, w_c, w_out, w_dgi, w_dgh, w_dlayer;
diff --git a/habitat-lab_amd/csrc/engine.hip b/habitat-lab_amd/csrc/engine.hip
--- a/habitat-lab_amd/csrc/engine.hip
+++ b/habitat-lab_amd/csrc/engine.hip
@@ -117,6 +117,7 @@
     const int64_t m1 = blind ? 0 : (int64_t)e->c1.Ho() * e->c1.Wo() * 32, m2 = blind ? 0 : (int64_t)e->c2.Ho() * e->c2.Wo() * 64, m3 = e->fc_in;
     e->w_a1 = wk.take(B * m1); e->w_a2 = wk.take(B * m2); e->w_a3 = wk.take(B * m3);
     e->w_da1 = wk.take(B * m1); e->w_da2 = wk.take(B * m2); e->w_da3 = wk.take(B * m3);
+    e->w_m1 = wk.take(B * m1 / 32); e->w_m2 = wk.take(B * m2 / 32);
     plan_tail_workspace(e, wk, std::max<int64_t>((int64_t)16 << 20, (int64_t)8 * H * e->fc_in / 4));
     e->work_floats = wk.used;
     return HAB_OK;
@@ -291,10 +292,15 @@
     ov.H = e->d.H; ov.W = e->d.W; ov.C = e->Cin;
     ConvDesc c1 = e->c1, c2 = e->c2, c3 = e->c3;
     c1.B = c2.B = c3.B = nB;
+    uint32_t* mb1 = e->save_acts ? reinterpret_cast<uint32_t*>(W + e->w_m1) + f0 * (m1 / 32) : nullptr;
+    uint32_t* mb2 = e->save_acts ? reinterpret_cast<uint32_t*>(W + e->w_m2) + f0 * (m2 / 32) : nullptr;
+    int made1 = 0, made2 = 0;
     { Probe pr(e, HAB_PROBE_CONV1_FWD, s);
-      HAB_TRY(obs_conv_fwd(c1, ov, e->PK + e->pk_c1f, e->p(e->i_c1b), a1, 1, ws, e->ws_floats, s, e->pk_c1img >= 0 ? e->PK + e->pk_c1img : nullptr)); }
+      HAB_TRY(obs_conv_fwd(c1, ov, e->PK + e->pk_c1f, e->p(e->i_c1b), a1, 1, ws, e->ws_floats, s, e->pk_c1img >= 0 ? e->PK + e->pk_c1img : nullptr,
+                           mb1, &made1)); }
     { Probe pr(e, HAB_PROBE_CONV2_FWD, s);
-      HAB_TRY(conv_fwd(c2, a1, e->PK + e->pk_c2f, e->p(e->i_c2b), a2, 1, ws, e->ws_floats, s)); }
+      HAB_TRY(conv_fwd(c2, a1, e->PK + e->pk_c2f, e->p(e->i_c2b), a2, 1, ws, e->ws_floats, s, mb2, &made2)); }
+    if (e->save_acts) { e->bits_a1 &= made1; e->bits_a2 &= made2; }
     { Probe pr(e, HAB_PROBE_CONV3_FWD, s);
       HAB_TRY(conv_fwd(c3, a2, e->PK + e->pk_c3f, e->p(e->i_c3b), a3, 0, ws, e->ws_floats, s)); }
     { Probe pr(e, HAB_PROBE_FC_FWD, s);
@@ -525,6 +531,7 @@
     float* W = e->WK;
     const int H = e->d.hidden, L = e->L;
     e->form = rnn_form(e, rows, pack, B, n);
+    e->bits_a1 = e->bits_a2 = 1;
     if (e->form.chunks > 0) {
         HAB_TRY(rnn_tm_forward(e, obs, rows, hidden0, hidden_env_stride, masks, B, n, stream));
     } else {
@@ -599,10 +606,10 @@
                            e->fc_in, nB, e->fc_in, e->d.hidden, 0, ws, e->ws_floats, s)); }
     { Probe pr(e, HAB_PROBE_CONV3_DGRAD, s);
       HAB_TRY(conv_dgrad(c3, W + e->w_da3 + f0 * m3, e->PK + e->pk_c3d, W + e->w_a2 + f0 * m2, nullptr, W + e->w_da2 + f0 * m2, ws,
-                         e->ws_floats, s)); }
+                         e->ws_floats, s, e->bits_a2 ? reinterpret_cast<const uint32_t*>(W + e->w_m2) + f0 * (m2 / 32) : nullptr)); }
     { Probe pr(e, HAB_PROBE_CONV2_DGRAD, s);
       HAB_TRY(conv_dgrad(c2, W + e->w_da2 + f0 * m2, e->PK + e->pk_c2d, W + e->w_a1 + f0 * m1, nullptr, W + e->w_da1 + f0 * m1, ws,
-                         e->ws_floats, s)); }
+                         e->ws_floats, s, e->bits_a1 ? reinterpret_cast<const uint32_t*>(W + e->w_m1) + f0 * (m1 / 32) : nullptr)); }
     return HAB_OK;
 }
 static int rnn_tm_backward(hab_policy* e, int B, hipStream_t stream) {
@@ -752,6 +759,13 @@
     float* W = e->WK;
     if (e->rn && which != HAB_TAP_RNN_IN && which != HAB_TAP_RNN_OUT) return resnet_tap(e, which, ptr, floats);
     if (!e->rn && e->Cin == 0 && (which == HAB_TAP_CONV1 || which == HAB_TAP_CONV2 || which == HAB_TAP_CONV3)) return HAB_ERR_ARG;
+    if (!e->rn && (which == HAB_TAP_CONV1_BITS || which == HAB_TAP_CONV2_BITS)) {
+        const bool first = which == HAB_TAP_CONV1_BITS;
+        if (e->Cin == 0 || !(first ? e->bits_a1 : e->bits_a2)) return HAB_ERR_ARG;
+        *ptr = W + (first ? e->w_m1 : e->w_m2);
+        *floats = first ? B * e->c1.Ho() * e->c1.Wo() : B * e->c2.Ho() * e->c2.Wo() * 2;
+        return HAB_OK;
+    }
     switch (which) {
         case HAB_TAP_CONV1: *ptr = W + e->w_a1; *floats = B * e->c1.Ho() * e->c1.Wo() * 32; break;
         case HAB_TAP_CONV2: *ptr = W + e->w_a2; *floats = B * e->c2.Ho() * e->c2.Wo() * 64; break;
diff --git a/habitat-lab_amd/csrc/gemm_ops.hip b/habitat-lab_amd/csrc/gemm_ops.hip
--- a/habitat-lab_amd/csrc/gemm_ops.hip
+++ b/habitat-lab_amd/csrc/gemm_ops.hip
@@ -29,7 +29,7 @@
 static int bf3_mode() {
     int m = g_bf3_mode.load(std::memory_order_relaxed);
     if (m < 0) {
-        static const int from_env = hab_env_int("HAB_BF3", 2047);
+        static const int from_env = hab_env_int("HAB_BF3", 2047 | MATRIX_PATH_RELU_BITS);
         int expected = -1;
         g_bf3_mode.compare_exchange_strong(expected, from_env, std::memory_order_relaxed);
         m = g_bf3_mode.load(std::memory_order_relaxed);
@@ -113,12 +113,16 @@
     }
 }
 
+static bool relu_bits_on() { return (bf3_mode() & MATRIX_PATH_RELU_BITS) != 0; }
 int conv_fwd(const ConvDesc& d, const float* x, const float* wf, const float* bias, float* y, int relu, float* ws,
-             size_t ws_floats, hipStream_t stream) {
+             size_t ws_floats, hipStream_t stream, uint32_t* relu_bits, int* bits_made) {
     ConvFwdProb p;
     HAB_TRY(build(p, d, x, wf, bias, y, relu));
+    if (bits_made) *bits_made = 0;
     if ((bf3_mode() & 256) && (bf3_mode() & 1)) {
-        const int rc = conv2_fwd_strip(p, ws, ws_floats, stream);
+        uint32_t* bits = (relu && relu_bits_on()) ? relu_bits : nullptr;
+        const int rc = conv2_fwd_strip(p, ws, ws_floats, stream, bits);
+        if (rc == HAB_OK && bits && bits_made) *bits_made = 1;
         if (rc != 1) return rc;
     }
     if ((bf3_mode() & 16) && d.stride == 1 && d.KH == 3 && d.KW == 3 && p.M > 64) {
@@ -135,11 +139,14 @@
     return obs_conv_patch_weight_image(wf, Cout, KH, KW, C, reinterpret_cast<unsigned short*>(img), stream);
 }
 int obs_conv_fwd(const ConvDesc& d, const ObsView& obs, const float* wf, const float* bias, float* y, int relu, float* ws,
-                 size_t ws_floats, hipStream_t stream, const void* wimg) {
+                 size_t ws_floats, hipStream_t stream, const void* wimg, uint32_t* relu_bits, int* bits_made) {
     ObsConvFwdProb p;
     HAB_TRY(build(p, d, obs, wf, bias, y, relu));
+    if (bits_made) *bits_made = 0;
     if ((bf3_mode() & 64) && (bf3_mode() & 2) && p.quad) {
-        const int rc = obs_conv_patch_launch(p, ws, ws_floats, stream, reinterpret_cast<const unsigned short*>(wimg));
+        uint32_t* bits = (relu && y && p.N == 32 && relu_bits_on()) ? relu_bits : nullptr;
+        const int rc = obs_conv_patch_launch(p, ws, ws_floats, stream, reinterpret_cast<const unsigned short*>(wimg), bits);
+        if (rc == HAB_OK && bits && bits_made) *bits_made = 1;
         if (rc != 1) return rc;
     }
     if ((bf3_mode() & 32) && (bf3_mode() & 2) && p.quad && p.M > 64) {
@@ -159,9 +166,11 @@
 }
 
 int conv_dgrad(const ConvDesc& d, const float* dy, const float* wd, const float* mask, const float* add, float* dx,
-               float* ws, size_t ws_floats, hipStream_t stream) {
+               float* ws, size_t ws_floats, hipStream_t stream, const uint32_t* mask_bits) {
+    if (mask_bits && (!mask || (reinterpret_cast<uintptr_t>(mask_bits) & 3))) return HAB_ERR_ARG;
+    if (!relu_bits_on() || d.C % 32) mask_bits = nullptr;
     if ((bf3_mode() & 512) && (bf3_mode() & 1)) {
-        const int rc = conv2_dgrad_strip(d, dy, wd, mask, add, dx, stream);
+        const int rc = conv2_dgrad_strip(d, dy, wd, mask, mask_bits, add, dx, stream);
         if (rc != 1) return rc;
     }
     if (d.stride > 1 && !no_dma() && !no_merged_dgrad()) {
@@ -187,6 +196,7 @@
         for (int pw = 0; pw < d.stride; ++pw) {
             ConvDgradProb p;
             HAB_TRY(build(p, d, dy, wd, mask, add, dx, ph, pw));
+            p.mask_bits = mask_bits;
             if (p.Hc <= 0 || p.Wc <= 0) continue;
             if ((bf3_mode() & 16) && d.stride == 1 && d.KH == 3 && d.KW == 3 && p.M > 64 && p.K > 0) {
                 PatchGeom gq{};
@@ -489,6 +499,25 @@
     if (!dy || !w_dgrad || !dx) return HAB_ERR_ARG;
     return conv_dgrad(mk(B, H, W, C, Cout, KH, KW, stride, pad), dy, w_dgrad, relu_mask, add, dx, ws, ws_floats, stream);
 }
+extern "C" int hab_conv2d_fwd_bits(const float* x, const float* w_fwd, const float* bias, float* y, uint32_t* relu_bits, int* bits_made,
+                                   int B, int H, int W, int C, int Cout, int KH, int KW, int stride, int pad, float* ws, size_t ws_floats,
+                                   hipStream_t stream) {
+    if (!x || !w_fwd || !y || !relu_bits || !bits_made) return HAB_ERR_ARG;
+    return conv_fwd(mk(B, H, W, C, Cout, KH, KW, stride, pad), x, w_fwd, bias, y, 1, ws, ws_floats, stream, relu_bits, bits_made);
+}
+extern "C" int hab_obs_conv2d_fwd_bits(const uint8_t* rgb, const float* depth, const int* rows, const float* w_fwd, const float* bias,
+                                       float* y, uint32_t* relu_bits, int* bits_made, int B, int H, int W, int Cout, int KH, int KW,
+                                       int stride, int pad, float* ws, size_t ws_floats, hipStream_t stream) {
+    if ((!rgb && !depth) || !w_fwd || !y || !relu_bits || !bits_made) return HAB_ERR_ARG;
+    ObsView o = mkobs(rgb, depth, rows, H, W);
+    return obs_conv_fwd(mk(B, H, W, o.C, Cout, KH, KW, stride, pad), o, w_fwd, bias, y, 1, ws, ws_floats, stream, nullptr, relu_bits, bits_made);
+}
+extern "C" int hab_conv2d_dgrad_bits(const float* dy, const float* w_dgrad, const float* relu_mask, const uint32_t* mask_bits, const float* add,
+                                     float* dx, int B, int H, int W, int C, int Cout, int KH, int KW, int stride, int pad, float* ws,
+                                     size_t ws_floats, hipStream_t stream) {
+    if (!dy || !w_dgrad || !dx || !relu_mask || !mask_bits) return HAB_ERR_ARG;
+    return conv_dgrad(mk(B, H, W, C, Cout, KH, KW, stride, pad), dy, w_dgrad, relu_mask, add, dx, ws, ws_floats, stream, mask_bits);
+}
 extern "C" int hab_conv2d_wgrad(const float* x, const float* dy, float* dw_oihw, float* dbias, int B, int H, int W, int C, int Cout,
                                 int KH, int KW, int stride, int pad, float* ws, size_t ws_floats, hipStream_t stream) {
     if (!x || !dy || !dw_oihw) return HAB_ERR_ARG;
diff --git a/habitat-lab_amd/csrc/obs_conv_patch.h b/habitat-lab_amd/csrc/obs_conv_patch.h
--- a/habitat-lab_amd/csrc/obs_conv_patch.h
+++ b/habitat-lab_amd/csrc/obs_conv_patch.h
@@ -2,6 +2,7 @@
 #include <utility>
 
 #include "igemm_bf3.h"
+#include "relu_bits.h"
 
 namespace hab {
 
@@ -46,9 +47,9 @@
     int patch_elems;
 };
 
-template <int UPT>
+template <int UPT, bool BITS>
 __global__ void __launch_bounds__(512) obs_conv_patch_kernel(const ObsConvFwdProb p, const ObsPatchGeom gq, const unsigned short* __restrict__ wimg,
-                                                              const int sign_schedule, const int ablate) {
+                                                              const int sign_schedule, const int ablate, uint32_t* __restrict__ relu_bits) {
     using P = ObsConvFwdProb;
     static_assert(EpiV4<P>::value, "transposed-accumulator epilogue");
     extern __shared__ __attribute__((aligned(16))) unsigned short smem16[];
@@ -229,6 +230,7 @@
             const int wo = 32 * i + li;
             if (wo >= gq.Wo) continue;
             const size_t base = ((size_t)(img * gq.Ho + ho) * gq.Wo + wo) * p.N;
+            unsigned wbits = 0;
 #pragma unroll
             for (int g = 0; g < 4; ++g) {
                 const int n = 8 * g + 4 * hi;
@@ -239,6 +241,11 @@
                 v += *reinterpret_cast<const f32x4*>(biasL + n);
                 if (p.relu) { v[0] = fmaxf(v[0], 0.f); v[1] = fmaxf(v[1], 0.f); v[2] = fmaxf(v[2], 0.f); v[3] = fmaxf(v[3], 0.f); }
                 if (p.y) *reinterpret_cast<f32x4*>(p.y + base + n) = v;
+                if constexpr (BITS) wbits |= relu_bits4(v) << n;
+            }
+            if constexpr (BITS) {
+                wbits |= __shfl_xor(wbits, 32);
+                if (hi == 0) relu_bits[(size_t)(img * gq.Ho + ho) * gq.Wo + wo] = wbits;
             }
         }
     };
@@ -282,13 +289,15 @@
     return HAB_OK;
 }
 
-inline int obs_conv_patch_launch(const ObsConvFwdProb& p, float* ws, size_t ws_floats, hipStream_t stream, const unsigned short* wimg_cached = nullptr) {
+inline int obs_conv_patch_launch(const ObsConvFwdProb& p, float* ws, size_t ws_floats, hipStream_t stream, const unsigned short* wimg_cached = nullptr,
+                                 uint32_t* relu_bits = nullptr) {
     const ConvGeom& g = p.g;
     if (!p.quad || g.KH != 8 || g.KW != 8 || g.stride != 4 || g.pad != 0 || p.N > 32 || (p.N & 3) || p.K != 256 || g.W > 256 || (g.W & 3) || g.Wo > 64 ||
         g.Wo < 1 || p.M <= 0)
         return 1;
     if (!wimg_cached && (!ws || ws_floats * 4 < (size_t)OCP_W_ELEMS * 2 || (reinterpret_cast<uintptr_t>(ws) & 15))) return 1;
     if (reinterpret_cast<uintptr_t>(wimg_cached) & 15) return 1;
+    if (relu_bits && (!p.relu || p.N != 32 || !p.y || (reinterpret_cast<uintptr_t>(relu_bits) & 3))) return HAB_ERR_ARG;
     ObsPatchGeom gq;
     gq.W = g.W; gq.H = g.H; gq.Ho = g.Ho; gq.Wo = g.Wo;
     gq.tiles_per_img = cdiv(g.Ho, OCP_TH);
@@ -305,14 +314,18 @@
         HAB_LAUNCH_CHECK();
         wimg = built;
     }
-    auto kern = obs_conv_patch_kernel<5>;
-    static const hipError_t attr_err = hipFuncSetAttribute(reinterpret_cast<const void*>(kern), hipFuncAttributeMaxDynamicSharedMemorySize, 160 * 1024);
+    static const hipError_t attr_err = [] {
+        const hipError_t e0 = hipFuncSetAttribute(reinterpret_cast<const void*>(obs_conv_patch_kernel<5, false>), hipFuncAttributeMaxDynamicSharedMemorySize, 160 * 1024);
+        const hipError_t e1 = hipFuncSetAttribute(reinterpret_cast<const void*>(obs_conv_patch_kernel<5, true>), hipFuncAttributeMaxDynamicSharedMemorySize, 160 * 1024);
+        return e0 != hipSuccess ? e0 : e1;
+    }();
     if (attr_err != hipSuccess) return (int)attr_err;
     static const int sign_schedule = !hab_env_flag("HAB_BF3_NOSIGN");
     static const int ablate = hab_env_int("HAB_OCP_ABLATE", 0);
     const int pairs = (gq.ntiles + 1) / 2;
     const int grid = pairs < 256 ? (pairs + 7) / 8 * 8 : 256;
-    kern<<<grid, 512, lds, stream>>>(p, gq, wimg, sign_schedule, ablate);
+    if (relu_bits) obs_conv_patch_kernel<5, true><<<grid, 512, lds, stream>>>(p, gq, wimg, sign_schedule, ablate, relu_bits);
+    else obs_conv_patch_kernel<5, false><<<grid, 512, lds, stream>>>(p, gq, wimg, sign_schedule, ablate, nullptr);
     HAB_LAUNCH_CHECK();
     return HAB_OK;
 }
diff --git a/habitat-lab_amd/csrc/ops.h b/habitat-lab_amd/csrc/ops.h
--- a/habitat-lab_amd/csrc/ops.h
+++ b/habitat-lab_amd/csrc/ops.h
@@ -12,13 +12,13 @@
 struct ObsView;
 
 int conv_fwd(const ConvDesc& d, const float* x, const float* wf, const float* bias, float* y, int relu, float* ws,
-             size_t ws_floats, hipStream_t stream);
+             size_t ws_floats, hipStream_t stream, uint32_t* relu_bits = nullptr, int* bits_made = nullptr);
 int obs_conv_fwd(const ConvDesc& d, const ObsView& obs, const float* wf, const float* bias, float* y, int relu, float* ws,
-                 size_t ws_floats, hipStream_t stream, const void* wimg = nullptr);
+                 size_t ws_floats, hipStream_t stream, const void* wimg = nullptr, uint32_t* relu_bits = nullptr, int* bits_made = nullptr);
 int64_t obs_conv_weight_image_floats();
 int obs_conv_weight_image(const float* wf, int Cout, int KH, int KW, int C, void* img, hipStream_t stream);
 int conv_dgrad(const ConvDesc& d, const float* dy, const float* wd, const float* mask, const float* add, float* dx,
-               float* ws, size_t ws_floats, hipStream_t stream);
+               float* ws, size_t ws_floats, hipStream_t stream, const uint32_t* mask_bits = nullptr);
 int conv_wgrad(const ConvDesc& d, const float* x, const float* dy, float* dw_oihw, float* dbias, float* ws, size_t ws_floats,
                hipStream_t stream);
 int obs_conv_wgrad(const ConvDesc& d, const ObsView& obs, const float* dy, float* dw_oihw, float* dbias, float* ws,
diff --git a/habitat-lab_amd/csrc/problems.h b/habitat-lab_amd/csrc/problems.h
--- a/habitat-lab_amd/csrc/problems.h
+++ b/habitat-lab_amd/csrc/problems.h
@@ -371,6 +371,7 @@
     const float* mask;
     const float* add;
     float* dx;
+    const uint32_t* mask_bits = nullptr;
     HAB_HD const float* dma_a_origin() const { return dy; }
     HAB_HD const float* dma_b_origin() const { return w; }
     void set_class(int ph_, int pw_) {
@@ -492,7 +493,8 @@
         EpiAux a;
         const size_t i = (r.ok & c.ok) ? r.base + c.n : 0;
         a.add = add ? add[i] : 0.f;
-        a.mask = mask ? mask[i] : 1.f;
+        if (mask_bits) a.mask = (float)((mask_bits[i >> 5] >> (i & 31)) & 1u);
+        else a.mask = mask ? mask[i] : 1.f;
         return a;
     }
     HAB_HD void epi_store(const EpiRow& r, const EpiCol& c, const EpiAux& a, float v) const {
@@ -509,7 +511,12 @@
         EpiAux4 a;
         const size_t i = (r.ok & c.ok) ? r.base + c.n : 0;
         a.add = add ? ld4(add + i) : zero4();
-        a.mask = mask ? ld4(mask + i) : splat4(1.f);
+        if (mask_bits) {
+            const uint32_t w = mask_bits[i >> 5] >> (i & 31);
+            for (int e = 0; e < 4; ++e) a.mask[e] = (float)((w >> e) & 1u);
+        } else {
+            a.mask = mask ? ld4(mask + i) : splat4(1.f);
+        }
         return a;
     }
     HAB_HD void epi_store4(const EpiRow& r, const EpiCol4& c, const EpiAux4& a, f32x4 v) const {
diff --git a/habitat-lab_amd/csrc/relu_bits.h b/habitat-lab_amd/csrc/relu_bits.h
--- /dev/null
+++ b/habitat-lab_amd/csrc/relu_bits.h
@@ -0,0 +1,19 @@
+#pragma once
+#include "hab_common.h"
+
+namespace hab {
+
+constexpr int MATRIX_PATH_RELU_BITS = 1 << 14;
+
+__device__ __forceinline__ unsigned relu_bits4(const f32x4 v) {
+    return (v[0] > 0.f ? 1u : 0u) | (v[1] > 0.f ? 2u : 0u) | (v[2] > 0.f ? 4u : 0u) | (v[3] > 0.f ? 8u : 0u);
+}
+
+__device__ __forceinline__ unsigned or_over_8_lanes(unsigned w) {
+    w |= (unsigned)__builtin_amdgcn_update_dpp(0, (int)w, 0xB1, 0xF, 0xF, true);
+    w |= (unsigned)__builtin_amdgcn_update_dpp(0, (int)w, 0x4E, 0xF, 0xF, true);
+    w |= (unsigned)__builtin_amdgcn_update_dpp(0, (int)w, 0x141, 0xF, 0xF, true);
+    return w;
+}
+
+}
diff --git a/habitat-lab_amd/habitat_amd/_lib.py b/habitat-lab_amd/habitat_amd/_lib.py
--- a/habitat-lab_amd/habitat_amd/_lib.py
+++ b/habitat-lab_amd/habitat_amd/_lib.py
@@ -79,6 +79,9 @@
     "hab_conv2d_fwd": (c_int, [vp, vp, vp, vp] + [c_int] * 10 + [vp, c_size_t, vp]),
     "hab_obs_conv2d_fwd": (c_int, [vp, vp, vp, vp, vp, vp] + [c_int] * 9 + [vp, c_size_t, vp]),
     "hab_conv2d_dgrad": (c_int, [vp, vp, vp, vp, vp] + [c_int] * 9 + [vp, c_size_t, vp]),
+    "hab_conv2d_fwd_bits": (c_int, [vp, vp, vp, vp, vp, POINTER(c_int)] + [c_int] * 9 + [vp, c_size_t, vp]),
+    "hab_obs_conv2d_fwd_bits": (c_int, [vp, vp, vp, vp, vp, vp, vp, POINTER(c_int)] + [c_int] * 8 + [vp, c_size_t, vp]),
+    "hab_conv2d_dgrad_bits": (c_int, [vp, vp, vp, vp, vp, vp] + [c_int] * 9 + [vp, c_size_t, vp]),
     "hab_conv2d_wgrad": (c_int, [vp, vp, vp, vp] + [c_int] * 9 + [vp, c_size_t, vp]),
     "hab_obs_conv2d_wgrad": (c_int, [vp, vp, vp, vp, vp, vp] + [c_int] * 8 + [vp, c_size_t, vp]),
     "hab_linear_fwd": (c_int, [vp, c_int, vp, c_int, vp, vp, c_int, c_int, c_int, c_int, c_int, c_int, vp, c_size_t, vp]),
diff --git a/include/habitat_amd.h b/include/habitat_amd.h
--- a/include/habitat_amd.h
+++ b/include/habitat_amd.h
@@ -112,6 +112,15 @@
 int hab_conv2d_dgrad(const float* dy, const float* w_dgrad, const float* relu_mask, const float* add, float* dx, int B,
                      int H, int W, int C, int Cout, int KH, int KW, int stride, int pad, float* ws, size_t ws_floats,
                      hipStream_t stream);
+int hab_conv2d_fwd_bits(const float* x, const float* w_fwd, const float* bias, float* y, uint32_t* relu_bits, int* bits_made, int B,
+                        int H, int W, int C, int Cout, int KH, int KW, int stride, int pad, float* ws, size_t ws_floats,
+                        hipStream_t stream);
+int hab_obs_conv2d_fwd_bits(const uint8_t* rgb, const float* depth, const int* rows, const float* w_fwd, const float* bias, float* y,
+                            uint32_t* relu_bits, int* bits_made, int B, int H, int W, int Cout, int KH, int KW, int stride, int pad,
+                            float* ws, size_t ws_floats, hipStream_t stream);
+int hab_conv2d_dgrad_bits(const float* dy, const float* w_dgrad, const float* relu_mask, const uint32_t* mask_bits, const float* add,
+                          float* dx, int B, int H, int W, int C, int Cout, int KH, int KW, int stride, int pad, float* ws,
+                          size_t ws_floats, hipStream_t stream);
 int hab_conv2d_wgrad(const float* x, const float* dy, float* dw_oihw, float* dbias, int B, int H, int W, int C, int Cout,
                      int KH, int KW, int stride, int pad, float* ws, size_t ws_floats, hipStream_t stream);
 int hab_obs_conv2d_wgrad(const uint8_t* rgb, const float* depth, const int* rows, const float* dy, float* dw_oihw,
@@ -344,6 +353,8 @@
 #define HAB_TAP_COMPRESSION 8
 #define HAB_TAP_LAYER1 9
 #define HAB_TAP_POOL_IDX 13
+#define HAB_TAP_CONV1_BITS 14
+#define HAB_TAP_CONV2_BITS 15
 #define HAB_TAP_CONV_OUT 100
 int hab_policy_tap(hab_policy* p, int which, const float** ptr, int64_t* floats);
 
```

Result: no change. 62700 env-steps/s, median of 4 (+0.1%).
